# D-Robotics/hobot_stereonet

Measured on AMD Instinct MI355X. Metric: stereo pairs/s at 1280x720 D=192 (ms/frame alongside), higher is better.
Workload: dtype f16 (refinement-tower MFMA operands fp16 — 3x3 weights rounded per kernel so that every kernel's tap sum survives —, LeakyReLU applied after the fp16 rounding; low-resolution branch on 22-bit hi/lo split fp16 operands, 3 fp16 MFMAs per product in every 32-channel layer — profiles/r04_lowres_ablation

## Files before the change

### hobot_stereonet_amd/csrc/sn_dbg_hooks.hpp

```cpp
#pragma once

namespace {

void host_to_slots(const float* src, int nimg, int H, int W, std::vector<_Float16>& dst) {
  const size_t plane = (size_t)H * W;
  dst.assign((size_t)nimg * 8 * plane * 8, (_Float16)0.f);
  for (int img = 0; img < nimg; ++img)
    for (int c = 0; c < kC; ++c)
      for (size_t i = 0; i < plane; ++i) {
        const float v = src[((size_t)img * kC + c) * plane + i];
        const _Float16 hi = (_Float16)v;
        const size_t base = (((size_t)img * 4 + (c >> 3)) * 2) * plane;
        dst[(base + i) * 8 + (c & 7)] = hi;
        dst[(base + plane + i) * 8 + (c & 7)] = (_Float16)((v - (float)hi) * kSplitScale);
      }
}
void host_from_slots(const std::vector<_Float16>& src, int nimg, int H, int W, float* dst) {
  const size_t plane = (size_t)H * W;
  for (int img = 0; img < nimg; ++img)
    for (int c = 0; c < kC; ++c)
      for (size_t i = 0; i < plane; ++i) {
        const size_t base = (((size_t)img * 4 + (c >> 3)) * 2) * plane;
        dst[((size_t)img * kC + c) * plane + i] =
            (float)src[(base + i) * 8 + (c & 7)] + (float)src[(base + plane + i) * 8 + (c & 7)] * kSplitInv;
      }
}

template <class V>
hipError_t to_dev(void* dev, const V& v) {
  return hipMemcpy(dev, v.data(), v.size() * sizeof(v[0]), hipMemcpyHostToDevice);
}
template <class V>
hipError_t from_dev(V& v, const void* dev) {
  return hipMemcpy(v.data(), dev, v.size() * sizeof(v[0]), hipMemcpyDeviceToHost);
}

struct PaddedSlots {
  SlotGeom g;
  int H, W;
  size_t nplanes, lead;
  std::vector<_Float16> v;
  PaddedSlots(const SlotGeom& g_, int H_, int W_, size_t nplanes_, size_t lead_ = 0)
      : g(g_), H(H_), W(W_), nplanes(nplanes_), lead(lead_), v((nplanes_ + 2 * lead_) * g_.PH * g_.PW * 8, (_Float16)0.f) {}
  size_t row(size_t plane, int y) const { return (((plane + lead) * g.PH + y + g.py) * g.PW + g.px) * 8; }
  void put(const std::vector<_Float16>& plain) {
    for (size_t p = 0; p < nplanes; ++p)
      for (int y = 0; y < H; ++y) memcpy(&v[row(p, y)], &plain[((p * H + y) * W) * 8], (size_t)W * 16);
  }
  void get(std::vector<_Float16>& plain) const {
    for (size_t p = 0; p < nplanes; ++p)
      for (int y = 0; y < H; ++y) memcpy(&plain[((p * H + y) * W) * 8], &v[row(p, y)], (size_t)W * 16);
  }
  bool outside_is_zero() const {
    const size_t phw = (size_t)g.PH * g.PW;
    for (size_t i = 0; i < v.size(); ++i) {
      const size_t sl = i / 8, p = sl / phw, y = (sl % phw) / g.PW, x = sl % g.PW;
      const bool inside = p >= lead && p < lead + nplanes && y >= (size_t)g.py && y < (size_t)H + g.py && x >= (size_t)g.px &&
                          x < (size_t)W + g.px;
      if (!inside && (float)v[i] != 0.f) return false;
    }
    return true;
  }
};

struct RefHost {
  RefGeom g;
  int n, h, w;
  size_t lo_slots;
  std::vector<_Float16> v;
  RefHost(const RefGeom& g_, int n_, int h_, int w_, bool split, bool slack)
      : g(g_), n(n_), h(h_), w(w_), lo_slots(ref16_slots(g_, n_) + (slack ? ref_slack(g_) : 0)), v((split ? 2 : 1) * lo_slots * 8) {}
  size_t slots() const { return v.size() / 8; }
  size_t at(int i, int c, int y, int x) const {
    return ((((size_t)i * 4 + (c >> 3)) * g.Hs + y + kRefPad) * g.Ws + x + kRefPad) * 8 + (c & 7);
  }
  void pack(const float* src, bool split) {
    v.assign(v.size(), (_Float16)0.f);
    for (int i = 0; i < n; ++i)
      for (int c = 0; c < kC; ++c)
        for (int y = 0; y < h; ++y)
          for (int x = 0; x < w; ++x) {
            const float f = src[(((size_t)i * kC + c) * h + y) * w + x];
            const _Float16 hi = (_Float16)f;
            v[at(i, c, y, x)] = hi;
            if (split) v[lo_slots * 8 + at(i, c, y, x)] = (_Float16)((f - (float)hi) * kSplitScale);
          }
  }
  void unpack(float* dst, bool split) const {
    for (int i = 0; i < n; ++i)
      for (int c = 0; c < kC; ++c)
        for (int y = 0; y < h; ++y)
          for (int x = 0; x < w; ++x) {
            float f = (float)v[at(i, c, y, x)];
            if (split) f += (float)v[lo_slots * 8 + at(i, c, y, x)] * kSplitInv;
            dst[(((size_t)i * kC + c) * h + y) * w + x] = f;
          }
  }
  bool border_is_zero(int parts) const {
    for (int part = 0; part < parts; ++part)
      for (int plane = 0; plane < 4 * n; ++plane)
        for (int y = 0; y < g.Hs; ++y)
          for (int x = 0; x < g.Ws; ++x) {
            if (y >= kRefPad && y < kRefPad + h && x >= kRefPad && x < kRefPad + w) continue;
            for (int e = 0; e < 8; ++e)
              if ((float)v[part * lo_slots * 8 + (((size_t)plane * g.Hs + y) * g.Ws + x) * 8 + e] != 0.f) return false;
          }
    return true;
  }
};

hipError_t alloc_ref16(DevScope& ds, const RefGeom& g, size_t tensor_and_slack_slots, uint4** base) {
  uint4* raw = nullptr;
  const hipError_t e = alloc_ref16(g, tensor_and_slack_slots, &raw, base);
  ds.track(raw);
  return e;
}

}

extern "C" {

int sn_dbg_conv2d(sn_handle* h, const float* in, int cin, int h_px, int w, const float* wt, const float* bias,
                  int k, int stride, int dil, int lrelu, const float* residual, float* out) {
  DevScope ds;
  if (!h || !in || !wt || !bias || !out || cin <= 0 || cin > kC) return SN_ERR_ARG;
  if (!((k == 3 && stride == 1) || (k == 5 && stride == 2 && dil == 1))) return SN_ERR_ARG;
  int rc = check_device(h);
  if (rc) return rc;
  const int taps = k * k;
  const int Ho = stride == 1 ? h_px : h_px / 2, Wo = stride == 1 ? w : w / 2;
  if (stride == 2 && ((h_px & 1) || (w & 1))) return SN_ERR_ARG;
  const bool x3 = (lrelu & 2) != 0, slots = (lrelu & 4) != 0;
  const bool tower32 = (lrelu & 8) != 0;
  const bool dma = (lrelu & 16) != 0;
  lrelu &= 1;
  if (x3 != slots || (x3 && !(cin == kC && dil == 1))) return SN_ERR_ARG;
  if (dma && !(slots && (k == 3 || !residual))) return SN_ERR_ARG;
  ConvLayer L;
  rc = upload_conv2d(h, HostLayer{wt, bias, kC, cin, taps}, slots ? 8 : (k == 5 || cin <= 4) ? 4 : 8, &L);
  if (!rc && slots)
    rc = upload_x3(h, kC, [&](int co, int c, int tap) { return wt[((size_t)co * kC + c) * taps + tap]; }, &L, taps);
  ds.adopt(L);
  if (rc) return rc;
  hipStream_t st = h->stream;
  if (slots) {
    std::vector<_Float16> hin, hres, hout((size_t)8 * Ho * Wo * 8);
    host_to_slots(in, 1, h_px, w, hin);
    if (residual) host_to_slots(residual, 1, Ho, Wo, hres);
    if (dma) {
      const FeatPad fp = feat_pad(h_px, w);
      PaddedSlots pin(k == 3 ? SlotGeom{fp.PH, fp.PW, 1, 1} : down_in_geom(Ho, Wo), h_px, w, 8);
      PaddedSlots pout(k == 3 ? pin.g : SlotGeom{Ho + 5, Wo + 7, 2, 3}, Ho, Wo, 8);
      pin.put(hin);
      if (residual) pout.put(hres);
      uint4 *pdin = nullptr, *pdout = nullptr;
      HIP_TRY(h, ds.alloc(&pdin, pin.v.size() / 8));
      HIP_TRY(h, ds.alloc(&pdout, pout.v.size() / 8));
      HIP_TRY(h, to_dev(pdin, pin.v));
      HIP_TRY(h, to_dev(pdout, pout.v));
      HIP_TRY(h, hipDeviceSynchronize());
      if (k == 5)
        HIP_TRY(h, launch_down_dma(st, L, pdin, 1, Ho, Wo, pdout, pout.g, lrelu != 0, h->num_cu));
      else if (residual)
        HIP_TRY(h, (launch_feat_dma<true, true>(st, L, pdin, fp, 1, pdout, pdout, lrelu != 0, h->num_cu)));
      else
        HIP_TRY(h, (launch_feat_dma<true, false>(st, L, pdin, fp, 1, pdout, nullptr, lrelu != 0, h->num_cu)));
      HIP_TRY(h, hipStreamSynchronize(st));
      HIP_TRY(h, from_dev(pout.v, pdout));
      pout.get(hout);
      if (!pout.outside_is_zero()) {
        set_err(h, k == 3 ? "k_feat_x3s_dma wrote outside the image" : "k_down_x3s_dma wrote outside the image");
        return SN_ERR_DEVICE;
      }
    } else {
      uint4 *din = nullptr, *dout = nullptr;
      HIP_TRY(h, ds.alloc(&din, hin.size() / 8));
      HIP_TRY(h, ds.alloc(&dout, hout.size() / 8));
      HIP_TRY(h, to_dev(din, hin));
      if (residual) HIP_TRY(h, to_dev(dout, hres));
      const float* dres = residual ? reinterpret_cast<const float*>(dout) : nullptr;
      SlotIn ls{din, 0, h_px, w};
      HIP_TRY(h, k == 5 ? (launch_conv_x3s<5, 2, 32, 4, 32, 32, 1, true, SlotIn>(st, L, ls, 1, Ho, Wo, reinterpret_cast<float*>(dout), dres, lrelu != 0, h->num_cu))
                        : (launch_conv_x3s<3, 1, 32, 8, 16, 16, 2, true, SlotIn>(st, L, ls, 1, Ho, Wo, reinterpret_cast<float*>(dout), dres, lrelu != 0, h->num_cu)));
      HIP_TRY(h, hipStreamSynchronize(st));
      HIP_TRY(h, from_dev(hout, dout));
    }
    host_from_slots(hout, 1, Ho, Wo, out);
    return SN_OK;
  }
  float *din = nullptr, *dout = nullptr;
  const size_t nin = (size_t)cin * h_px * w, nout = (size_t)kC * Ho * Wo;
  HIP_TRY(h, ds.alloc(&din, nin));
  HIP_TRY(h, ds.alloc(&dout, nout));
  HIP_TRY(h, hipMemcpy(din, in, nin * 4, hipMemcpyHostToDevice));
  const float* dres = nullptr;
  if (residual) {
    HIP_TRY(h, hipMemcpy(dout, residual, nout * 4, hipMemcpyHostToDevice));
    dres = dout;
  }
  LoadF32 ld{din, cin, h_px, w};
  hipError_t e;
  if (k == 5) {
    e = (Ho * Wo <= 64 * 128) ? launch_conv<5, 2, 1, 4, 4, 32>(st, L, ld, 1, Ho, Wo, dout, dres, lrelu != 0)
                              : launch_conv<5, 2, 1, 4, 8, 64>(st, L, ld, 1, Ho, Wo, dout, dres, lrelu != 0);
  } else if (cin <= 4) {
    if (dil != 1) return SN_ERR_ARG;
    e = (Ho * Wo <= 64 * 128) ? launch_conv<3, 1, 1, 4, 4, 32>(st, L, ld, 1, Ho, Wo, dout, dres, lrelu != 0)
                              : launch_conv<3, 1, 1, 4, 8, 64>(st, L, ld, 1, Ho, Wo, dout, dres, lrelu != 0);
  } else {
    if (tower32 && ((w & 3) != 0 || cin != kC)) return SN_ERR_ARG;
    e = conv3x3(st, L, din, 1, h_px, w, dil, dout, dres, lrelu != 0, tower32 ? h->num_cu : 0);
  }
  HIP_TRY(h, e);
  HIP_TRY(h, hipStreamSynchronize(st));
  HIP_TRY(h, hipMemcpy(out, dout, nout * 4, hipMemcpyDeviceToHost));
  return SN_OK;
}

int sn_dbg_down0(sn_handle* h, const int8_t* in6, int h_px, int w, const float* wt, const float* bias, int tc,
                 float* out) {
  DevScope ds;
  if (!h || !in6 || !wt || !bias || !out || h_px <= 0 || w <= 0 || tc != 32) return SN_ERR_ARG;
  int rc = check_device(h);
  if (rc) return rc;
  const int Hp = (h_px + 15) / 16 * 16, Wp = (w + 15) / 16 * 16, Ho = Hp / 2, Wo = Wp / 2;
  Down0F16 L;
  rc = upload_down0_f16(h, HostLayer{wt, bias, kC, 3, 25}, &L);
  ds.adopt(L);
  if (rc) return rc;
  int8_t* din = nullptr;
  float *dout = nullptr, *dbias = nullptr;
  const size_t nin = (size_t)6 * h_px * w, nout = (size_t)2 * kC * Ho * Wo;
  HIP_TRY(h, ds.alloc(&din, nin));
  HIP_TRY(h, ds.alloc(&dout, nout));
  HIP_TRY(h, ds.alloc(&dbias, kC));
  HIP_TRY(h, hipMemcpy(din, in6, nin, hipMemcpyHostToDevice));
  HIP_TRY(h, hipMemcpy(dbias, bias, kC * 4, hipMemcpyHostToDevice));
  HIP_TRY(h, launch_down0_f16(h->stream, L, dbias, din, h_px, w, 2, Ho, Wo, dout, h->num_cu));
  HIP_TRY(h, hipStreamSynchronize(h->stream));
  std::vector<_Float16> hs(nout * 2);
  HIP_TRY(h, from_dev(hs, dout));
  host_from_slots(hs, 2, Ho, Wo, out);
  return SN_OK;
}

int sn_dbg_round_kernels_f16(const float* w, int nkernels, float* out) {
  if (!w || !out || nkernels < 0) return SN_ERR_ARG;
  for (int k = 0; k < nkernels; ++k) {
    _Float16 q[9];
    round_kernel_sum_preserving(w + (size_t)k * 9, q);
    for (int t = 0; t < 9; ++t) out[(size_t)k * 9 + t] = (float)q[t];
  }
  return SN_OK;
}

int sn_dbg_compose_down01(const float* w0, const float* b0, const float* w1, const float* b1, float* weff, float* beff) {
  if (!w0 || !b0 || !w1 || !b1 || !weff || !beff) return SN_ERR_ARG;
  std::vector<double> we, be;
  compose_down01(w0, b0, w1, b1, we, be);
  for (size_t i = 0; i < we.size(); ++i) weff[i] = (float)we[i];
  for (size_t i = 0; i < be.size(); ++i) beff[i] = (float)be[i];
  return SN_OK;
}

int sn_dbg_down01(sn_handle* h, const int8_t* in6, int h_px, int w, const float* w0, const float* b0, const float* w1,
                  const float* b1, float* out) {
  DevScope ds;
  if (!h || !in6 || !w0 || !b0 || !w1 || !b1 || !out || h_px <= 0 || w <= 0) return SN_ERR_ARG;
  int rc = check_device(h);
  if (rc) return rc;
  const int Hp = (h_px + 15) / 16 * 16, Wp = (w + 15) / 16 * 16, Ho = Hp / 4, Wo = Wp / 4;
  Down01W L;
  rc = upload_down01(h, HostLayer{w0, b0, kC, 3, 25}, HostLayer{w1, b1, kC, kC, 25}, &L);
  ds.adopt(L);
  if (rc) return rc;
  int8_t* din = nullptr;
  uint4* dout = nullptr;
  const size_t nin = (size_t)6 * h_px * w, nout = (size_t)2 * kC * Ho * Wo;
  HIP_TRY(h, ds.alloc(&din, nin));
  HIP_TRY(h, ds.alloc(&dout, nout / 4));
  HIP_TRY(h, hipMemcpy(din, in6, nin, hipMemcpyHostToDevice));
  HIP_TRY(h, launch_down01(h->stream, L, din, h_px, w, 2, Ho, Wo, dout, SlotGeom{Ho, Wo, 0, 0}, h->num_cu));
  HIP_TRY(h, hipStreamSynchronize(h->stream));
  std::vector<_Float16> hs(nout * 2);
  HIP_TRY(h, from_dev(hs, dout));
  host_from_slots(hs, 2, Ho, Wo, out);
  return SN_OK;
}

int sn_dbg_refin(sn_handle* h, const float* disp_low, const int8_t* in6, int h_px, int w, int dmax, const float* wt,
                 const float* bias, int split, float* out) {
  DevScope ds;
  if (!h || !disp_low || !in6 || !wt || !bias || !out || h_px <= 0 || w <= 0 || dmax <= 0) return SN_ERR_ARG;
  int rc = check_device(h);
  if (rc) return rc;
  const int Hp = (h_px + 15) / 16 * 16, Wp = (w + 15) / 16 * 16, hl = Hp / 16, wl = Wp / 16;
  RefHost t(make_ref_geom(Hp, Wp), 1, Hp, Wp, true, true);
  Down0F16 L;
  rc = upload_refin_f16(h, HostLayer{wt, bias, kC, 4, 9}, &L);
  ds.adopt(L);
  if (rc) return rc;
  float *ddl = nullptr, *dbias = nullptr;
  int8_t* din = nullptr;
  uint4* dout = nullptr;
  HIP_TRY(h, ds.alloc(&ddl, (size_t)hl * wl));
  HIP_TRY(h, ds.alloc(&dbias, kC));
  HIP_TRY(h, ds.alloc(&din, (size_t)6 * h_px * w));
  HIP_TRY(h, ds.alloc(&dout, t.slots()));
  HIP_TRY(h, hipMemcpy(ddl, disp_low, (size_t)hl * wl * 4, hipMemcpyHostToDevice));
  HIP_TRY(h, hipMemcpy(dbias, bias, kC * 4, hipMemcpyHostToDevice));
  HIP_TRY(h, hipMemcpy(din, in6, (size_t)6 * h_px * w, hipMemcpyHostToDevice));
  HIP_TRY(h, memset_now(dout, 0, t.slots() * 16));
  HIP_TRY(h, launch_refin_f16(h->stream, L, dbias, ddl, din, false, hl, wl, h_px, w, 1.0f / (float)dmax,
                              UpScale{1.0f / 16.0f, 16.0f}, t.g, 1, dout, split != 0, t.lo_slots * 16, h->num_cu));
  HIP_TRY(h, hipStreamSynchronize(h->stream));
  HIP_TRY(h, from_dev(t.v, dout));
  t.unpack(out, split != 0);
  if (!t.border_is_zero(1)) {
    set_err(h, "ref.in wrote into the zero border");
    return SN_ERR_DEVICE;
  }
  return SN_OK;
}

int sn_dbg_conv3d(sn_handle* h, const float* in, int d, int h_px, int w, const float* wt, const float* bias,
                  int lrelu, float* out) {
  DevScope ds;
  if (!h || !in || !wt || !bias || !out || d <= 0) return SN_ERR_ARG;
  int rc = check_device(h);
  if (rc) return rc;
  const bool x3 = (lrelu & 2) != 0, slots = (lrelu & 4) != 0, dma = (lrelu & 8) != 0;
  lrelu &= 1;
  if (slots != x3 || (dma && !slots)) return SN_ERR_ARG;
  ConvLayer L;
  rc = upload_conv3d(h, HostLayer{wt, bias, kC, kC, 27}, &L);
  if (!rc && x3)
    rc = upload_x3(h, 96, [&](int co, int c, int tap) { return wt[(((size_t)co * kC + (c & 31)) * 3 + (c >> 5)) * 9 + tap]; }, &L);
  ds.adopt(L);
  if (rc) return rc;
  const size_t plane = (size_t)h_px * w, n = (size_t)kC * d * plane;
  std::vector<float> tmp(n);
  for (int ci = 0; ci < kC; ++ci)
    for (int z = 0; z < d; ++z)
      memcpy(&tmp[((size_t)z * kC + ci) * plane], &in[((size_t)ci * d + z) * plane], plane * 4);
  float *din = nullptr, *dout = nullptr;
  HIP_TRY(h, ds.alloc(&din, n));
  HIP_TRY(h, ds.alloc(&dout, n));
  if (slots) {
    std::vector<_Float16> hs, ho(n * 2);
    host_to_slots(tmp.data(), d, h_px, w, hs);
    if (dma) {
      const VolPad g = vol_pad(d, h_px, w);
      PaddedSlots pin(SlotGeom{g.PH, g.PW, 1, 1}, h_px, w, (size_t)d * 8, 8), pout = pin;
      pin.put(hs);
      uint4 *pdin = nullptr, *pdout = nullptr;
      HIP_TRY(h, ds.alloc(&pdin, pin.v.size() / 8));
      HIP_TRY(h, ds.alloc(&pdout, pout.v.size() / 8));
      HIP_TRY(h, to_dev(pdin, pin.v));
      HIP_TRY(h, memset_now(pdout, 0, pout.v.size() * 2));
      HIP_TRY(h, launch_agg_dma<true>(h->stream, L, pdin, g, 1, pdout, lrelu != 0, h->num_cu));
      HIP_TRY(h, hipStreamSynchronize(h->stream));
      HIP_TRY(h, from_dev(pout.v, pdout));
      pout.get(ho);
      if (!pout.outside_is_zero()) {
        set_err(h, "k_agg_x3s_dma wrote outside the image");
        return SN_ERR_DEVICE;
      }
    } else {
      HIP_TRY(h, to_dev(din, hs));
      SlotIn ls{reinterpret_cast<const uint4*>(din), d, h_px, w};
      HIP_TRY(h, (launch_conv_x3s<3, 1, 96, 8, 16, 16, 1, true, SlotIn>(h->stream, L, ls, d, h_px, w, dout, nullptr, lrelu != 0, h->num_cu)));
      HIP_TRY(h, hipStreamSynchronize(h->stream));
      HIP_TRY(h, from_dev(ho, dout));
    }
    host_from_slots(ho, d, h_px, w, tmp.data());
  } else {
    HIP_TRY(h, to_dev(din, tmp));
    LoadVol3D lv{din, d, h_px, w};
    HIP_TRY(h, (launch_conv<3, 1, 1, 8, 4, 32>(h->stream, L, lv, d, h_px, w, dout, nullptr, lrelu != 0)));
    HIP_TRY(h, hipStreamSynchronize(h->stream));
    HIP_TRY(h, from_dev(tmp, dout));
  }
  for (int co = 0; co < kC; ++co)
    for (int z = 0; z < d; ++z)
      memcpy(&out[((size_t)co * d + z) * plane], &tmp[((size_t)z * kC + co) * plane], plane * 4);
  return SN_OK;
}

int sn_dbg_ref_conv_f16(sn_handle* h, const float* in, int h_px, int w, const float* wt, const float* bias, int dil,
                        int lrelu, const float* residual, float* out) {
  DevScope ds;
  if (!h || !in || !wt || !bias || !out || h_px <= 0 || w <= 0) return SN_ERR_ARG;
  if (dil != 1 && dil != 2 && dil != 4 && dil != 8) return SN_ERR_ARG;
  int rc = check_device(h);
  if (rc) return rc;
  RefHost t(make_ref_geom(h_px, w), 1, h_px, w, false, false);
  RefLayerF16 L;
  rc = upload_ref_f16(h, HostLayer{wt, bias, kC, kC, 9}, switches_at_create().w_round_sum_preserving, &L);
  ds.adopt(L);
  if (rc) return rc;
  uint4 *din = nullptr, *dout = nullptr;
  HIP_TRY(h, ds.alloc(&din, t.slots()));
  HIP_TRY(h, ds.alloc(&dout, t.slots()));
  t.pack(in, false);
  HIP_TRY(h, to_dev(din, t.v));
  if (residual) {
    t.pack(residual, false);
    HIP_TRY(h, to_dev(dout, t.v));
  } else {
    HIP_TRY(h, memset_now(dout, 0, t.slots() * 16));
  }
  unsigned* ctr = h->ws.tile_ctr;
  if (!ctr) {
    set_err(h, "sn_dbg_ref_conv_f16 needs an engine created in an fp16 mode");
    return SN_ERR_ARG;
  }
  HIP_TRY(h, hipMemsetAsync(ctr, 0, kTileCtrBytes, h->stream));
  HIP_TRY(h, ref_conv_f16(h->stream, L, t.g, h->num_cu, dil, din, dout, residual ? dout : nullptr, 1, (lrelu & 1) != 0, ctr,
                          (lrelu & 2) ? 64 : (lrelu & 4) ? 32 : 0));
  HIP_TRY(h, hipStreamSynchronize(h->stream));
  HIP_TRY(h, from_dev(t.v, dout));
  t.unpack(out, false);
  if (!t.border_is_zero(1)) {
    set_err(h, "fp16 conv wrote into the zero border");
    return SN_ERR_DEVICE;
  }
  return SN_OK;
}

int sn_dbg_ref_conv_f16x3(sn_handle* h, const float* in, int h_px, int w, const float* wt, const float* bias, int dil,
                          int lrelu, const float* residual, float* out) {
  DevScope ds;
  if (!h || !in || !wt || !bias || !out || h_px <= 0 || w <= 0) return SN_ERR_ARG;
  if (dil != 1 && dil != 2 && dil != 4 && dil != 8) return SN_ERR_ARG;
  int rc = check_device(h);
  if (rc) return rc;
  RefHost t(make_ref_geom(h_px, w), 1, h_px, w, true, true);
  RefLayerF16 L;
  rc = upload_ref_f16x3(h, HostLayer{wt, bias, kC, kC, 9}, &L);
  ds.adopt(L);
  if (rc) return rc;
  uint4 *din = nullptr, *dout = nullptr;
  HIP_TRY(h, ds.alloc(&din, t.slots()));
  HIP_TRY(h, ds.alloc(&dout, t.slots()));
  t.pack(in, true);
  HIP_TRY(h, to_dev(din, t.v));
  if (residual) {
    t.pack(residual, true);
    HIP_TRY(h, to_dev(dout, t.v));
  } else {
    HIP_TRY(h, memset_now(dout, 0, t.slots() * 16));
  }
  HIP_TRY(h, ref_conv_f16x3(h->stream, L, t.g, h->num_cu, dil, din, dout, residual ? dout : nullptr, t.lo_slots, 1, lrelu != 0));
  HIP_TRY(h, hipStreamSynchronize(h->stream));
  HIP_TRY(h, from_dev(t.v, dout));
  t.unpack(out, true);
  if (!t.border_is_zero(2)) {
    set_err(h, "f16x3 conv wrote into the zero border");
    return SN_ERR_DEVICE;
  }
  return SN_OK;
}

int sn_dbg_ref_block_f16x3(sn_handle* h, const float* in, int h_px, int w, const float* w1, const float* b1, const float* w2,
                           const float* b2, int dil, int form, float* out) {
  DevScope ds;
  if (!h || !in || !w1 || !b1 || !w2 || !b2 || !out || h_px <= 0 || w <= 0) return SN_ERR_ARG;
  if (dil != 1 && dil != 2 && dil != 4 && dil != 8) return SN_ERR_ARG;
  if (form != 0 && form != 1) return SN_ERR_ARG;
  if (form == 1 && !stream_x3_supports(dil)) return SN_ERR_ARG;
  int rc = check_device(h);
  if (rc) return rc;
  RefHost t(make_ref_geom(h_px, w), 1, h_px, w, true, true);
  RefLayerF16 L1, L2;
  rc = upload_ref_f16x3(h, HostLayer{w1, b1, kC, kC, 9}, &L1);
  if (!rc) rc = upload_ref_f16x3(h, HostLayer{w2, b2, kC, kC, 9}, &L2);
  ds.adopt(L1);
  ds.adopt(L2);
  if (rc) return rc;
  uint4 *cur = nullptr, *oth = nullptr;
  HIP_TRY(h, alloc_ref16(ds, t.g, t.slots(), &cur));
  HIP_TRY(h, alloc_ref16(ds, t.g, t.slots(), &oth));
  t.pack(in, true);
  HIP_TRY(h, to_dev(cur, t.v));
  HIP_TRY(h, ref_block_f16x3(h->stream, L1, L2, t.g, h->num_cu, dil, &cur, &oth, t.lo_slots, 1, form == 1));
  HIP_TRY(h, hipStreamSynchronize(h->stream));
  HIP_TRY(h, from_dev(t.v, cur));
  t.unpack(out, true);
  if (!t.border_is_zero(2)) {
    set_err(h, "f16x3 residual block wrote into the zero border");
    return SN_ERR_DEVICE;
  }
  return SN_OK;
}

int sn_dbg_ref_block_f16(sn_handle* h, const float* in, int h_px, int w, const float* w1, const float* b1,
                         const float* w2, const float* b2, int dil, float* out) {
  DevScope ds;
  if (!h || !in || !w1 || !b1 || !w2 || !b2 || !out || h_px <= 0 || w <= 0) return SN_ERR_ARG;
  const int form = dil >> 8;
  if (form != 0 && form != 2) return SN_ERR_ARG;
  const int fuse_mode = form == 2 ? 4 : 0;
  dil &= 0xff;
  if (dil != 1 && dil != 2 && dil != 4 && dil != 8) return SN_ERR_ARG;
  if (fuse_mode == 4 && !stream_block_supports(dil)) return SN_ERR_ARG;
  int rc = check_device(h);
  if (rc) return rc;
  RefHost t(make_ref_geom(h_px, w), 1, h_px, w, false, false);
  const bool sp = switches_at_create().w_round_sum_preserving;
  RefLayerF16 L1, L2;
  rc = upload_ref_f16(h, HostLayer{w1, b1, kC, kC, 9}, sp, &L1);
  if (!rc) rc = upload_ref_f16(h, HostLayer{w2, b2, kC, kC, 9}, sp, &L2);
  ds.adopt(L1);
  ds.adopt(L2);
  if (rc) return rc;
  uint4 *cur = nullptr, *oth = nullptr;
  HIP_TRY(h, alloc_ref16(ds, t.g, t.slots() + ref_slack(t.g), &cur));
  HIP_TRY(h, alloc_ref16(ds, t.g, t.slots() + ref_slack(t.g), &oth));
  t.pack(in, false);
  HIP_TRY(h, to_dev(cur, t.v));
  if (!h->ws.tile_ctr) {
    set_err(h, "sn_dbg_ref_block_f16 needs an engine created in an fp16 mode");
    return SN_ERR_ARG;
  }
  HIP_TRY(h, hipMemsetAsync(h->ws.tile_ctr, 0, kTileCtrBytes, h->stream));
  HIP_TRY(h, ref_block_f16(h->stream, L1, L2, t.g, h->num_cu, dil, &cur, &oth, 1, h->ws.tile_ctr, fuse_mode, h->dump));
  HIP_TRY(h, hipStreamSynchronize(h->stream));
  HIP_TRY(h, from_dev(t.v, cur));
  t.unpack(out, false);
  if (!t.border_is_zero(1)) {
    set_err(h, "fp16 residual block wrote into the zero border");
    return SN_ERR_DEVICE;
  }
  return SN_OK;
}

int sn_dbg_ref_tail_f16(sn_handle* h, int n, const float* in, int hk, int wk, const float* w1, const float* b1, const float* w2,
                        const float* b2, const float* head_w, float head_b, const float* low, int ups, float dnorm, int h_out,
                        int w_out, int form, float* out_disp, int32_t* out_raw) {
  DevScope ds;
  if (!h || !in || !w1 || !b1 || !w2 || !b2 || !head_w || !low || !out_disp || !out_raw) return SN_ERR_ARG;
  if (n <= 0 || hk <= 0 || wk <= 0 || h_out <= 0 || w_out <= 0 || h_out > hk || w_out > wk || (ups != 16 && ups != 2) ||
      hk % ups || wk % ups || (form != 0 && form != 1) || !(dnorm > 0.f))
    return SN_ERR_ARG;
  if (h->precision != SN_PREC_F16 && h->precision != SN_PREC_AUTO) {
    set_err(h, "sn_dbg_ref_tail_f16 needs an engine created with SN_PREC_F16 or SN_PREC_AUTO");
    return SN_ERR_ARG;
  }
  int rc = check_device(h);
  if (rc) return rc;
  const RefGeom g = make_ref_geom(hk, wk);
  if ((ref16_slots(g, n) + ref_slack(g) + ref_front(g)) * 16 >= ((size_t)1 << 32)) return SN_ERR_ARG;
  RefHost t(g, n, hk, wk, false, false);
  t.pack(in, false);
  const bool sp = switches_at_create().w_round_sum_preserving;
  RefLayerF16 L1, L2;
  HeadLayer hd;
  rc = upload_ref_f16(h, HostLayer{w1, b1, kC, kC, 9}, sp, &L1);
  if (!rc) rc = upload_ref_f16(h, HostLayer{w2, b2, kC, kC, 9}, sp, &L2);
  if (!rc) rc = upload_head(h, HostLayer{head_w, &head_b, 1, kC, 9}, &hd);
  ds.adopt(L1);
  ds.adopt(L2);
  ds.adopt(hd);
  if (rc) return rc;
  uint4 *da = nullptr, *db = nullptr;
  HIP_TRY(h, alloc_ref16(ds, g, t.slots() + ref_slack(g), &da));
  HIP_TRY(h, alloc_ref16(ds, g, t.slots() + ref_slack(g), &db));
  HIP_TRY(h, to_dev(da, t.v));
  const int sh = hk / ups, sw = wk / ups;
  const size_t nlow = (size_t)n * sh * sw, nout = (size_t)n * h_out * w_out;
  float *dlow = nullptr, *dd = nullptr;
  int32_t* dr = nullptr;
  HIP_TRY(h, ds.alloc(&dlow, nlow));
  HIP_TRY(h, ds.alloc(&dd, nout));
  HIP_TRY(h, ds.alloc(&dr, nout));
  HIP_TRY(h, hipMemcpy(dlow, low, nlow * 4, hipMemcpyHostToDevice));
  HIP_TRY(h, memset_now(dd, 0xff, nout * 4));
  HIP_TRY(h, memset_now(dr, 0xff, nout * 4));
  const float inv_q = (float)(1.0 / (kWireFactor * (double)kOutScale));
  const UpScale us{1.0f / (float)ups, (float)ups};
  const HeadArgs ha{hd.w, dlow, dd, dr, hd.bias, dnorm, inv_q, sh, sw, h_out, w_out, us};
  if (form == 1) {
    HIP_TRY(h, ref_block_stream_tail(h->stream, L1, L2, g, h->num_cu, da, n, h->dump, ha));
  } else {
    HIP_TRY(h, ref_block_stream(h->stream, L1, L2, g, h->num_cu, 1, da, db, n, h->dump));
    HIP_TRY(h, launch_head_final_f16(h->stream, false, db, 0, g, n, ha));
  }
  HIP_TRY(h, hipStreamSynchronize(h->stream));
  HIP_TRY(h, hipMemcpy(out_disp, dd, nout * 4, hipMemcpyDeviceToHost));
  HIP_TRY(h, hipMemcpy(out_raw, dr, nout * 4, hipMemcpyDeviceToHost));
  return SN_OK;
}

int sn_dbg_jpeg_dct(sn_handle* h, const uint8_t* nv12, int w, int h_px, int pitch, float* out) {
  DevScope ds;
  if (!h || !nv12 || !out || !jpg_size_ok(w, h_px) || pitch < w) return SN_ERR_ARG;
  int rc = check_device(h);
  if (rc) return rc;
  const size_t span = (size_t)(h_px + h_px / 2 - 1) * pitch + w;
  const size_t blocks = (size_t)((w + 15) / 16) * jpg_mcu_rows(h_px) * 6;
  JpgPlan plan;
  jpg_make_plan(w, h_px, 50, 0, &plan);
  uint8_t* din = nullptr;
  int16_t* dcoef = nullptr;
  float* ddct = nullptr;
  HIP_TRY(h, ds.alloc(&din, span));
  HIP_TRY(h, ds.alloc(&dcoef, blocks * 64));
  HIP_TRY(h, ds.alloc(&ddct, blocks * 64));
  HIP_TRY(h, hipMemcpy(din, nv12, span, hipMemcpyHostToDevice));
  if ((rc = jpeg_launch(h, h->stream, plan, 1, din, pitch, 0, 0, dcoef, nullptr, nullptr, nullptr, 0, nullptr, ddct))) return rc;
  HIP_TRY(h, hipStreamSynchronize(h->stream));
  HIP_TRY(h, hipMemcpy(out, ddct, blocks * 64 * 4, hipMemcpyDeviceToHost));
  return SN_OK;
}

__global__ __launch_bounds__(256) void k_copy_limited(uint4* __restrict__ dst, const uint4* __restrict__ src, size_t n16) {
  for (size_t i = (size_t)blockIdx.x * 256 + threadIdx.x; i < n16; i += (size_t)gridDim.x * 256) dst[i] = src[i];
}

int sn_dbg_copy_limited(void* dst, const void* src, size_t bytes, int workgroups, void* stream) {
  if (!dst || !src || (bytes & 15) || workgroups <= 0 || workgroups > 65535 || ((uintptr_t)dst & 15) || ((uintptr_t)src & 15)) return SN_ERR_ARG;
  hipLaunchKernelGGL(k_copy_limited, dim3((unsigned)workgroups), dim3(256), 0, static_cast<hipStream_t>(stream),
                     static_cast<uint4*>(dst), static_cast<const uint4*>(src), bytes / 16);
  return hipGetLastError() == hipSuccess ? SN_OK : SN_ERR_DEVICE;
}

int sn_dbg_read(sn_handle* h, const char* what, float* dst, size_t cap, size_t* n) {
  if (!h || !what || !n) return SN_ERR_ARG;
  int rc = check_device(h);
  if (rc) return rc;
  const size_t hw = (size_t)h->hl * h->wl;
  const float* src = nullptr;
  size_t cnt = 0;
  if (!strcmp(what, "stream_prio")) {
    *n = 1;
    if (dst && cap >= 1) dst[0] = h->stream_prio ? 1.f : 0.f;
    return (dst && cap < 1) ? SN_ERR_ARG : SN_OK;
  }
  if (!strcmp(what, "feat_l")) { src = h->ws.feat; cnt = kC * hw; }
  else if (!strcmp(what, "feat_r")) { src = h->ws.feat + kC * hw; cnt = kC * hw; }
  else if (!strcmp(what, "cost")) { src = h->ws.cost; cnt = h->Dl * hw; }
  else if (!strcmp(what, "disp_low")) { src = h->ws.disp_low; cnt = hw; }
  else if (!strcmp(what, "conf_low")) { src = h->ws.conf_low; cnt = hw; }
  else if (!strcmp(what, "tile_ctr") && h->ws.tile_ctr) { src = reinterpret_cast<const float*>(h->ws.tile_ctr); cnt = kTileCtrBytes / 4 * h->ws.n_chunks; }
  else if (!strcmp(what, "refine_x") && h->precision == SN_PREC_FP32) { src = h->ws.ref[0]; cnt = (size_t)kC * h->Hp * h->Wp; }
  else if (!strncmp(what, "level", 5) && what[5] >= '1' && what[5] < '0' + h->levels && what[6] == 0) {
    const int k = what[5] - '0';
    src = h->ws.lvl_disp[k];
    cnt = (size_t)h->tw[k].Hk * h->tw[k].Wk;
  }
  else return SN_ERR_ARG;
  *n = cnt;
  if (!dst) return SN_OK;
  if (cap < cnt) return SN_ERR_ARG;
  HIP_TRY(h, hipStreamSynchronize(h->stream));
  HIP_TRY(h, hipMemcpy(dst, src, cnt * 4, hipMemcpyDeviceToHost));
  return SN_OK;
}

}
```

### hobot_stereonet_amd/csrc/sn_engine.hpp

```cpp
#pragma once

namespace {

using namespace sn;

constexpr int kNDown = 4, kNFeatRes = 6, kNAgg = 4, kNRefRes = 6;
constexpr int kRefDil[kNRefRes] = {1, 2, 4, 8, 1, 1};
constexpr float kOutScale = 2.60443857769133e-6f;
constexpr double kWireFactor = 16.0 * 12.0;
constexpr double kAutoEnvelopeSingle = 1.0, kAutoEnvelopeMulti = 2.9;
constexpr double kAutoResidualCap = 1e30;
constexpr int kMaxPieceEvents = 64;
constexpr int kMaxTowerStreams = 2;

#define HIP_TRY(h, expr)                                                              \
  do {                                                                                \
    hipError_t e_ = (expr);                                                           \
    if (e_ != hipSuccess) {                                                           \
      set_err(h, std::string(#expr) + ": " + hipGetErrorString(e_));                  \
      return SN_ERR_DEVICE;                                                           \
    }                                                                                 \
  } while (0)

inline hipError_t memset_now(void* p, int v, size_t bytes) {
  hipError_t e = hipMemset(p, v, bytes);
  if (e != hipSuccess) return e;
  return hipStreamSynchronize(nullptr);
}

struct GrowBuf {
  void* p = nullptr;
  size_t cap = 0;
  bool pinned = false;
  hipError_t reserve(size_t bytes) {
    if (bytes <= cap) return hipSuccess;
    release();
    const hipError_t e = pinned ? hipHostMalloc(&p, bytes, hipHostMallocDefault) : hipMalloc(&p, bytes);
    if (e == hipSuccess) cap = bytes;
    else p = nullptr;
    return e;
  }
  void release() {
    if (p) (void)(pinned ? hipHostFree(p) : hipFree(p));
    p = nullptr;
    cap = 0;
  }
};

template <class Slots>
struct Lane : Slots {
  std::mutex mu;
  hipStream_t stream = nullptr;
  hipEvent_t ev = nullptr;
  GrowBuf buf[Slots::kCount];
  void destroy() {
    if (stream) (void)hipStreamSynchronize(stream);
    if (ev) {
      (void)hipEventSynchronize(ev);
      (void)hipEventDestroy(ev);
    }
    if (stream) (void)hipStreamDestroy(stream);
    for (GrowBuf& b : buf) b.release();
    stream = nullptr, ev = nullptr;
  }
};

struct ConvLayer {
  uint4* wx3 = nullptr;
  float* wpk = nullptr;
  float* bias = nullptr;
  int cin = 0, cin_pad = 0, taps = 0;
};

struct Down0F16 {
  uint4* wfrag = nullptr;
};

struct Down01W {
  uint4* wfrag = nullptr;
  float* bias = nullptr;
};

struct RefLayerF16 {
  uint4* wfrag = nullptr;
  float* bias = nullptr;
};

struct HeadLayer {
  float* w = nullptr;
  float bias = 0.f;
  float* wsplit = nullptr;
  float biassplit = 0.f, unscale = 1.f;
  uint4* pfrag = nullptr;
};

constexpr int kMaxLevels = 4, kMultiLevels = 4;
constexpr int kStatWords = 8;
constexpr size_t kStatU64 = (size_t)kStatWords * kStatWordStride;
constexpr int kTileCtrStride = 8 * 16;
constexpr size_t kTileCtrBytes = (size_t)2 * 6 * kTileCtrStride * sizeof(unsigned);

struct Workspace {
  int nb = 0, rb = 0, pb = 0;
  int rb_x3 = 0;
  int tower_cu = 0;
  int rbk_x3[4] = {};
  unsigned long long* stats = nullptr;
  unsigned long long* stats_host = nullptr;
  int8_t* in6 = nullptr;
  float* down[3] = {nullptr, nullptr, nullptr};
  float* low[3] = {nullptr, nullptr, nullptr};
  float* feat = nullptr;
  float* vol[2] = {nullptr, nullptr};
  uint4* volp[2] = {nullptr, nullptr};
  uint4* lowp[2] = {nullptr, nullptr};
  uint4* downp[3] = {nullptr, nullptr, nullptr};
  float* cost = nullptr;
  float* disp_low = nullptr;
  float* conf_low = nullptr;
  int ns = 1;
  float* ref[2 * kMaxTowerStreams] = {};
  uint4* ref16[2 * kMaxTowerStreams] = {};
  uint4* ref16_raw[2 * kMaxTowerStreams] = {};
  int rbk[kMaxLevels] = {};
  float* ref_lv[kMaxLevels][2] = {};
  uint4* ref16_lv[kMaxLevels][2] = {};
  uint4* ref16_lv_raw[kMaxLevels][2] = {};
  float* pyr[kMaxLevels] = {};
  float* lvl_disp[kMaxLevels] = {};
  int n_chunks = 0;
  unsigned* tile_ctr = nullptr;
  float* out_disp = nullptr;
  int32_t* out_raw = nullptr;
  uint8_t* nv12 = nullptr;
};

struct Tower {
  ConvLayer rin, rres[kNRefRes][2];
  Down0F16 refin;
  RefLayerF16 rres16[kNRefRes][2];
  RefLayerF16 rres16x3[kNRefRes][2];
  HeadLayer rout;
  RefGeom rg{};
  int Hk = 0, Wk = 0;
};

struct Slot {
  hipStream_t stream = nullptr;
  hipEvent_t ev0 = nullptr, ev1 = nullptr;
  Workspace ws;
  int8_t* pin_in = nullptr;
  int32_t* pin_raw = nullptr;
  float* pin_disp = nullptr;
  int32_t* user_raw = nullptr;
  float* user_disp = nullptr;
  uint64_t ticket = 0;
  hipGraphExec_t gexec[2][4][4] = {};
  int uses[2][4][4] = {};
  int mode_run = 0;
};

struct RangeCount {
  unsigned long long level[4] = {}, low = 0;
  bool any() const { return (level[0] | level[1] | level[2] | level[3] | low) != 0; }
};

struct AutoCtl {
  sn_auto_state st{};
  bool calibrated = false;
  bool pending = false;
  int pending_mode = 0, pending_n = 0;
  double selfcheck_epe = -1.0, selfcheck_res = -1.0;
  double last_level[4] = {}, last_res = 0.0;
  RangeCount last_range;
  int last_mode = 0;
  uint64_t calls = 0, pairs = 0, reruns = 0;
};

}

struct sn_handle {
  int device = 0;
  int W = 0, H = 0, D = 0, Wp = 0, Hp = 0, wl = 0, hl = 0, Dl = 0;
  int max_batch = 1, precision = SN_PREC_F16, task_num = 4, refine_chunk = 1, piece = 16;
  AutoCtl actl;
  std::mutex mu_cal;
  float* chk[2] = {nullptr, nullptr};
  hipEvent_t ev_stats = nullptr;
  int refine_chunk_x3 = 1;
  hipStream_t stream = nullptr;
  hipStream_t s_low = nullptr, s_tow[kMaxTowerStreams] = {};
  hipEvent_t ev_fork = nullptr, ev_join = nullptr, ev_tow_join[kMaxTowerStreams] = {}, ev_piece[kMaxPieceEvents] = {};
  bool overlap = true;
  int tower_streams = kMaxTowerStreams;
#if SN_DIAGNOSTICS
  unsigned ablate_x = 0;
#else
  static constexpr unsigned ablate_x = 0;
#endif
  bool tail_fuse = true;
  int fuse_mode = 4;
  unsigned* dump = nullptr;
  bool use_graphs = true;
  bool stream_prio = false;
  ConvLayer down[kNDown], fres[kNFeatRes][2], fout, agg[kNAgg];
  Down0F16 down0;
  Down01W down01;
  bool fold_down01 = false;
  HeadLayer aout;
  int levels = 1;
  Tower tw[kMaxLevels];
  int num_cu = 256;
  Workspace ws;
  std::vector<Slot> slots;
  std::mutex mu;
  std::condition_variable cv;
  uint64_t next_ticket = 1;
  bool profiling = false;
  hipEvent_t ev[8] = {};
  hipEvent_t ev_dom[2 * 6] = {};
  int dom_pairs = 0;
  float stage_ms[SN_STAGE_COUNT] = {};
  mutable std::string err;
  mutable std::mutex err_mu;
  struct PointCloudSlots {
    enum { kScratch = 0, kRaw, kNv12, kPoints, kCounts, kPinRaw, kPinNv12, kCount };
  };
  struct PointCloud : Lane<PointCloudSlots> {
    PointCloud() { buf[kPinRaw].pinned = buf[kPinNv12].pinned = true; }
  } pc;
  struct FilterSlots {
    enum { kScratch = 0, kRaw, kDisp, kMask, kCounts, kCount };
  };
  using Filter = Lane<FilterSlots>;
  Filter flt;
  struct SmoothSlots {
    enum { kScratch = 0, kRaw, kGuide, kOut, kDisp, kMask, kCounts, kCount };
  };
  using Smooth = Lane<SmoothSlots>;
  Smooth smo;
  struct JpegSlots {
    enum { kCoef = 0, kBytes, kLens, kIn, kOut, kSizes, kCount };
  };
  struct Jpeg : Lane<JpegSlots> {
    sn::JpgPlan plan;
  } jpg;
  struct InferStaging {
    enum { kIn = 0, kMirror, kLeft, kRight, kDisp, kRightOut, kMask, kKept, kConf, kCount };
    GrowBuf buf[kCount];
  } stage;
  std::atomic<int> temporal_live{0};
  std::atomic<int> rectify_live{0};
};

struct sn_temporal_slots {
  enum { kRaw = 0, kGuide, kDisp, kMask, kCounts, kCount };
};
struct sn_temporal : Lane<sn_temporal_slots> {
  sn_handle* h = nullptr;
  int streams = 0;
  sn_temporal_params p{};
  long long q = 0;
  void* state = nullptr;
  std::vector<uint8_t> fresh;
};

struct sn_rectify_slots {
  enum { kLeft = 0, kRight, kSbs, kTensor, kCount };
};
struct sn_rectify : Lane<sn_rectify_slots> {
  sn_handle* h = nullptr;
  sn_stereo_calib c{};
  uint32_t valid[2] = {0, 0};
  int32_t* map = nullptr;
};

namespace {

void set_err(const sn_handle* h, const std::string& s) {
  if (h) {
    std::lock_guard<std::mutex> lk(h->err_mu);
    h->err = s;
  }
}
void set_err(std::nullptr_t, const std::string&) {}

template <class T>
hipError_t dalloc(T** p, size_t count) {
  return hipMalloc(reinterpret_cast<void**>(p), count * sizeof(T) + 256);
}

struct DevScope {
  std::vector<void*> ptrs;
  void track(const void* p) {
    void* q = const_cast<void*>(p);
    if (q && std::find(ptrs.begin(), ptrs.end(), q) == ptrs.end()) ptrs.push_back(q);
  }
  template <class T>
  hipError_t alloc(T** p, size_t count) {
    const hipError_t e = dalloc(p, count);
    track(*p);
    return e;
  }
  void adopt(const ConvLayer& l) { track(l.wx3); track(l.wpk); track(l.bias); }
  void adopt(const Down0F16& l) { track(l.wfrag); }
  void adopt(const Down01W& l) { track(l.wfrag); track(l.bias); }
  void adopt(const RefLayerF16& l) { track(l.wfrag); track(l.bias); }
  void adopt(const HeadLayer& l) { track(l.w); track(l.pfrag); if (l.wsplit != l.w) track(l.wsplit); }
  ~DevScope() {
    for (void* q : ptrs) (void)hipFree(q);
  }
};

int check_device(sn_handle* h) {
  HIP_TRY(h, hipSetDevice(h->device));
  return SN_OK;
}

}
```

### hobot_stereonet_amd/csrc/sn_forward.hpp

```cpp
#pragma once

namespace {

inline int piece_pairs(const sn_handle* h, int nb, int rb) {
  int pb = h->piece > 0 ? h->piece : 16;
  if (pb > nb) pb = nb;
  if (pb < rb) pb = rb;
  return pb;
}
inline int level_chunk_pairs(int rb, int pb, int lv) {
  const long r = (long)rb << (2 * lv);
  return lv == 0 ? rb : (r < pb ? (int)r : pb);
}

int alloc_ws(sn_handle* h, Workspace* ws, int nb, int rb, int ns, int rb_x3 = 0) {
  const bool is_auto = h->precision == SN_PREC_AUTO;
  if (rb_x3 <= 0 || rb_x3 > rb) rb_x3 = rb;
  ws->nb = nb;
  ws->rb = rb;
  ws->rb_x3 = rb_x3;
  ws->ns = (ns > 1 && nb > rb) ? (ns < kMaxTowerStreams ? ns : kMaxTowerStreams) : 1;
  if (h->levels > 1) ws->ns = 1;
  ws->pb = piece_pairs(h, nb, rb);
  const int pb = ws->pb;
  const size_t HW = (size_t)h->H * h->W, HWp = (size_t)h->Hp * h->Wp, hw = (size_t)h->hl * h->wl;
  HIP_TRY(h, dalloc(&ws->in6, (size_t)nb * 6 * HW));
  bool padded_down = h->precision != SN_PREC_FP32 && switches().down_dma;
  size_t downp_bytes[3] = {0, 0, 0};
  for (int k = h->fold_down01 ? 1 : 0; k < 3 && padded_down; ++k) {
    const SlotGeom g = down_in_geom(h->Hp >> (k + 2), h->Wp >> (k + 2));
    downp_bytes[k] = (size_t)2 * pb * 8 * g.PH * g.PW * sizeof(uint4);
    padded_down = downp_bytes[k] < ((size_t)1 << 32);
  }
  const int k_first = h->fold_down01 ? 1 : 0;
  for (int k = k_first; k < 3 && !padded_down; ++k)
    HIP_TRY(h, dalloc(&ws->down[k], (size_t)2 * pb * kC * (HWp >> (2 * (k + 1)))));
  for (int k = 0; k < 3; ++k) HIP_TRY(h, dalloc(&ws->low[k], (size_t)2 * pb * kC * hw));
  HIP_TRY(h, dalloc(&ws->feat, (size_t)2 * pb * kC * hw));
  for (int k = 0; k < 2; ++k) HIP_TRY(h, dalloc(&ws->vol[k], (size_t)pb * h->Dl * kC * hw));
  for (int k = k_first; k < 3 && padded_down; ++k) {
    HIP_TRY(h, hipMalloc(reinterpret_cast<void**>(&ws->downp[k]), downp_bytes[k]));
    HIP_TRY(h, memset_now(ws->downp[k], 0, downp_bytes[k]));
  }
  if (padded_down && switches().feat_dma) {
    const FeatPad g = feat_pad(h->hl, h->wl);
    const size_t bytes = (size_t)2 * pb * g.img_slots() * sizeof(uint4);
    for (int k = 0; k < 2 && bytes < ((size_t)1 << 32); ++k) {
      HIP_TRY(h, hipMalloc(reinterpret_cast<void**>(&ws->lowp[k]), bytes));
      HIP_TRY(h, memset_now(ws->lowp[k], 0, bytes));
    }
  }
  if (h->precision != SN_PREC_FP32 && switches().agg_dma) {
    const VolPad g = vol_pad(h->Dl, h->hl, h->wl);
    const size_t bytes = g.planes(pb) * g.plane_slots() * sizeof(uint4);
    for (int k = 0; k < 2 && bytes < ((size_t)1 << 32); ++k) {
      HIP_TRY(h, hipMalloc(reinterpret_cast<void**>(&ws->volp[k]), bytes));
      HIP_TRY(h, memset_now(ws->volp[k], 0, bytes));
    }
  }
  HIP_TRY(h, dalloc(&ws->cost, (size_t)nb * h->Dl * hw));
  HIP_TRY(h, dalloc(&ws->disp_low, (size_t)nb * hw));
  HIP_TRY(h, dalloc(&ws->conf_low, (size_t)nb * hw));
  HIP_TRY(h, memset_now(ws->conf_low, 0, (size_t)nb * hw * sizeof(float)));
  auto tensor_slots = [&](const RefGeom& rg, int pairs, int pairs_x3) {
    const size_t one = ref16_slots(rg, pairs) + ref_slack(rg), lo = ref16_slots(rg, pairs_x3) + ref_slack(rg);
    return h->precision == SN_PREC_F16X3 ? 2 * one : (is_auto ? one + lo : one);
  };
  if (h->precision == SN_PREC_FP32) {
    for (int k = 0; k < 2 * ws->ns; ++k) HIP_TRY(h, dalloc(&ws->ref[k], (size_t)rb * kC * HWp));
  } else {
    for (int k = 0; k < 2 * ws->ns; ++k)
      HIP_TRY(h, alloc_ref16(h->tw[0].rg, tensor_slots(h->tw[0].rg, rb, rb_x3), &ws->ref16_raw[k], &ws->ref16[k]));
    ws->n_chunks = (nb + rb_x3 - 1) / rb_x3 + (nb + pb - 1) / pb + 2;
    for (int lv = 1; lv < h->levels; ++lv) {
      const int rbk = level_chunk_pairs(rb_x3, pb, lv);
      ws->n_chunks += ((nb + pb - 1) / pb + 2) * ((pb + rbk - 1) / rbk + 1);
    }
    HIP_TRY(h, hipExtMallocWithFlags(reinterpret_cast<void**>(&ws->tile_ctr), kTileCtrBytes * ws->n_chunks, hipDeviceMallocFinegrained));
  }
  ws->rbk[0] = rb;
  ws->rbk_x3[0] = rb_x3;
  for (int lv = 1; lv < h->levels; ++lv) {
    const Tower& T = h->tw[lv];
    const size_t HWk = (size_t)T.Hk * T.Wk;
    ws->rbk[lv] = level_chunk_pairs(rb, pb, lv);
    ws->rbk_x3[lv] = level_chunk_pairs(rb_x3, pb, lv);
    for (int k = 0; k < 2; ++k) {
      if (h->precision == SN_PREC_FP32) {
        HIP_TRY(h, dalloc(&ws->ref_lv[lv][k], (size_t)ws->rbk[lv] * kC * HWk));
      } else {
        HIP_TRY(h, alloc_ref16(T.rg, tensor_slots(T.rg, ws->rbk[lv], ws->rbk_x3[lv]), &ws->ref16_lv_raw[lv][k], &ws->ref16_lv[lv][k]));
      }
    }
    HIP_TRY(h, dalloc(&ws->pyr[lv], (size_t)pb * 3 * HWk));
    HIP_TRY(h, dalloc(&ws->lvl_disp[lv], (size_t)pb * HWk));
  }
  HIP_TRY(h, dalloc(&ws->out_disp, (size_t)nb * HW));
  HIP_TRY(h, dalloc(&ws->out_raw, (size_t)nb * HW));
  HIP_TRY(h, dalloc(&ws->nv12, (size_t)HW * 3));
  HIP_TRY(h, dalloc(&ws->stats, kStatU64));
  HIP_TRY(h, memset_now(ws->stats, 0, kStatU64 * sizeof(unsigned long long)));
  HIP_TRY(h, hipHostMalloc(reinterpret_cast<void**>(&ws->stats_host), kStatU64 * sizeof(unsigned long long), hipHostMallocDefault));
  memset(ws->stats_host, 0, kStatU64 * sizeof(unsigned long long));
  return SN_OK;
}

void free_ws(Workspace* ws) {
  hipFree(ws->in6);
  hipFree(ws->tile_ctr);
  for (auto p : ws->down) hipFree(p);
  for (auto p : ws->low) hipFree(p);
  hipFree(ws->feat);
  for (auto p : ws->vol) hipFree(p);
  for (auto p : ws->volp) hipFree(p);
  for (auto p : ws->downp) hipFree(p);
  for (auto p : ws->lowp) hipFree(p);
  hipFree(ws->cost);
  hipFree(ws->disp_low);
  hipFree(ws->conf_low);
  for (auto p : ws->ref) hipFree(p);
  for (auto p : ws->ref16_raw) hipFree(p);
  for (auto& lv : ws->ref_lv)
    for (auto p : lv) hipFree(p);
  for (auto& lv : ws->ref16_lv_raw)
    for (auto p : lv) hipFree(p);
  for (auto p : ws->pyr) hipFree(p);
  for (auto p : ws->lvl_disp) hipFree(p);
  hipFree(ws->out_disp);
  hipFree(ws->out_raw);
  hipFree(ws->nv12);
  hipFree(ws->stats);
  if (ws->stats_host) hipHostFree(ws->stats_host);
  *ws = Workspace();
}

int launch_softargmin(sn_handle* h, Workspace& ws, hipStream_t st, const float* v, bool folded, int p0, int m, bool want_cost,
                      bool want_conf) {
  const int hl = h->hl, wl = h->wl, Dl = h->Dl, npix = m * hl * wl;
  float* const disp_low = ws.disp_low + (size_t)p0 * hl * wl;
  float* const cost_out = want_cost ? ws.cost + (size_t)p0 * Dl * hl * wl : nullptr;
  float* const conf_low = want_conf ? ws.conf_low + (size_t)p0 * hl * wl : nullptr;
  unsigned long long* const nf = ws.stats + kStatNonfiniteLow;
  const dim3 grid((npix + 63) / 64);
  if (folded) {
    const auto kern = want_conf ? k_softargmin_p<16, true> : k_softargmin_p<16, false>;
    hipLaunchKernelGGL(kern, grid, dim3(64 * Dl), 0, st, v, h->aout.bias, Dl, hl, wl, npix, disp_low, cost_out, conf_low, nf);
  } else {
    const auto kern = want_conf ? k_head_softargmin<16, true> : k_head_softargmin<16, false>;
    hipLaunchKernelGGL(kern, grid, dim3(64 * kSamWaves), 0, st, v, h->aout.w, h->aout.bias, Dl, hl, wl, npix, disp_low, cost_out,
                       conf_low, nf);
  }
  HIP_TRY(h, hipGetLastError());
  return SN_OK;
}

inline const uint4* as_slots(const float* p) { return reinterpret_cast<const uint4*>(p); }

int lowres_down_slots(sn_handle* h, Workspace& ws, hipStream_t st, const int8_t* in, int ni) {
  const int Hp = h->Hp, Wp = h->Wp, ncu = h->num_cu;
  const int k_first = h->fold_down01 ? 1 : 0;
  if (ws.downp[1] != nullptr) {
    SlotGeom gin[3];
    for (int i = 0; i < 3; ++i) gin[i] = down_in_geom(Hp >> (i + 2), Wp >> (i + 2));
    if (h->fold_down01)
      HIP_TRY(h, launch_down01(st, h->down01, in, h->H, h->W, ni, Hp / 4, Wp / 4, ws.downp[1], gin[1], ncu));
    else
      HIP_TRY(h, launch_down0_f16(st, h->down0, h->down[0].bias, in, h->H, h->W, ni, Hp / 2, Wp / 2,
                                  reinterpret_cast<float*>(ws.downp[0]), ncu, &gin[0]));
    for (int i = k_first; i < 3; ++i) {
      const int Ho = Hp >> (i + 2), Wo = Wp >> (i + 2);
      const SlotGeom plain{Ho, Wo, 0, 0};
      const FeatPad fp = feat_pad(h->hl, h->wl);
      const SlotGeom bordered{fp.PH, fp.PW, 1, 1};
      void* const last = ws.lowp[0] ? (void*)ws.lowp[0] : (void*)ws.low[0];
      HIP_TRY(h, launch_down_dma(st, h->down[i + 1], ws.downp[i], ni, Ho, Wo, i < 2 ? (void*)ws.downp[i + 1] : last,
                                 i < 2 ? gin[i + 1] : (ws.lowp[0] ? bordered : plain), false, ncu));
    }
    return SN_OK;
  }
  if (h->fold_down01)
    HIP_TRY(h, launch_down01(st, h->down01, in, h->H, h->W, ni, Hp / 4, Wp / 4, reinterpret_cast<uint4*>(ws.down[1]),
                             SlotGeom{Hp / 4, Wp / 4, 0, 0}, ncu));
  else
    HIP_TRY(h, launch_down0_f16(st, h->down0, h->down[0].bias, in, h->H, h->W, ni, Hp / 2, Wp / 2, ws.down[0], ncu));
  float* const src[3] = {ws.down[0], ws.down[1], ws.down[2]};
  float* const dst[3] = {ws.down[1], ws.down[2], ws.low[0]};
  for (int i = k_first; i < 3; ++i) {
    const int Hi = Hp >> (i + 1), Wi = Wp >> (i + 1);
    if ((h->ablate_x >> (kAblDown + i)) & 1u) HIP_TRY(h, zero_lo_slots(st, src[i], ni, (size_t)Hi * Wi));
    SlotIn ld{as_slots(src[i]), 0, Hi, Wi};
    HIP_TRY(h, (launch_conv_x3s<5, 2, 32, 4, 32, 32, 1, true, SlotIn>(st, h->down[i + 1], ld, ni, Hi / 2, Wi / 2, dst[i],
                                                                     nullptr, false, ncu)));
  }
  return SN_OK;
}

int lowres_features_slots(sn_handle* h, Workspace& ws, hipStream_t st, int ni) {
  const int hl = h->hl, wl = h->wl, ncu = h->num_cu;
  if (ws.lowp[0] != nullptr && ws.downp[1] != nullptr) {
    const FeatPad fp = feat_pad(hl, wl);
    uint4 *x = ws.lowp[0], *t = ws.lowp[1];
    for (int i = 0; i < kNFeatRes; ++i) {
      HIP_TRY(h, (launch_feat_dma<true, false>(st, h->fres[i][0], x, fp, ni, t, nullptr, true, ncu)));
      HIP_TRY(h, (launch_feat_dma<true, true>(st, h->fres[i][1], t, fp, ni, x, x, true, ncu)));
    }
    HIP_TRY(h, (launch_feat_dma<false, false>(st, h->fout, x, fp, ni, ws.feat, nullptr, false, ncu)));
    return SN_OK;
  }
  float *const x = ws.low[0], *const t = ws.low[1];
  const SlotIn lx{as_slots(x), 0, hl, wl}, lt{as_slots(t), 0, hl, wl};
  for (int i = 0; i < kNFeatRes; ++i) {
    if ((h->ablate_x >> (kAblFeat + 2 * i)) & 1u) HIP_TRY(h, zero_lo_slots(st, x, ni, (size_t)hl * wl));
    HIP_TRY(h, (launch_conv_x3s<3, 1, 32, 8, 16, 16, 2, true, SlotIn>(st, h->fres[i][0], lx, ni, hl, wl, t, nullptr, true, ncu)));
    if ((h->ablate_x >> (kAblFeat + 2 * i + 1)) & 1u) HIP_TRY(h, zero_lo_slots(st, t, ni, (size_t)hl * wl));
    HIP_TRY(h, (launch_conv_x3s<3, 1, 32, 8, 16, 16, 2, true, SlotIn>(st, h->fres[i][1], lt, ni, hl, wl, x, x, true, ncu)));
  }
  if ((h->ablate_x >> (kAblFeat + 12)) & 1u) HIP_TRY(h, zero_lo_slots(st, x, ni, (size_t)hl * wl));
  HIP_TRY(h, (launch_conv_x3s<3, 1, 32, 8, 16, 16, 1, false, SlotIn>(st, h->fout, lx, ni, hl, wl, ws.feat, nullptr, false, ncu)));
  return SN_OK;
}

int lowres_aggregate_slots(sn_handle* h, Workspace& ws, hipStream_t st, int m, bool* folded) {
  const int hl = h->hl, wl = h->wl, Dl = h->Dl, ncu = h->num_cu;
  const long total = (long)m * Dl * 4 * hl * wl;
  *folded = false;
  if (ws.volp[0] != nullptr) {
    const VolPad g = vol_pad(Dl, hl, wl);
    hipLaunchKernelGGL(k_cost_slots_pad, dim3((unsigned)((total + 255) / 256)), dim3(256), 0, st, ws.feat, ws.volp[1], g, m);
    for (int i = 0; i + 1 < kNAgg; ++i)
      HIP_TRY(h, launch_agg_dma<true>(st, h->agg[i], ws.volp[(i + 1) & 1], g, m, ws.volp[i & 1], true, ncu));
    const int i = kNAgg - 1;
    *folded = switches().head_fold && h->aout.pfrag;
    if (*folded)
      HIP_TRY(h, (launch_agg_dma<false, true>(st, h->agg[i], ws.volp[(i + 1) & 1], g, m, ws.vol[i & 1], true, ncu, h->aout.pfrag)));
    else
      HIP_TRY(h, launch_agg_dma<false>(st, h->agg[i], ws.volp[(i + 1) & 1], g, m, ws.vol[i & 1], true, ncu));
    return SN_OK;
  }
  hipLaunchKernelGGL(k_cost_slots, dim3((unsigned)((total + 255) / 256)), dim3(256), 0, st, ws.feat,
                     reinterpret_cast<uint4*>(ws.vol[1]), Dl, hl, wl, m);
  for (int i = 0; i < kNAgg; ++i) {
    float* const src = ws.vol[(i + 1) & 1];
    if ((h->ablate_x >> (kAblAgg + i)) & 1u) HIP_TRY(h, zero_lo_slots(st, src, m * Dl, (size_t)hl * wl));
    SlotIn lv{as_slots(src), Dl, hl, wl};
    if (i + 1 < kNAgg)
      HIP_TRY(h, (launch_conv_x3s<3, 1, 96, 8, 16, 16, 1, true, SlotIn>(st, h->agg[i], lv, m * Dl, hl, wl, ws.vol[i & 1], nullptr, true, ncu)));
    else
      HIP_TRY(h, (launch_conv_x3s<3, 1, 96, 8, 16, 16, 1, false, SlotIn>(st, h->agg[i], lv, m * Dl, hl, wl, ws.vol[i & 1], nullptr, true, ncu)));
  }
  return SN_OK;
}

int lowres(sn_handle* h, Workspace& ws, hipStream_t st, int p0, int m, const int8_t* in6, bool want_cost, bool want_conf,
           bool prof) {
  const int Hp = h->Hp, Wp = h->Wp, hl = h->hl, wl = h->wl, Dl = h->Dl;
  const size_t HW = (size_t)h->H * h->W;
  const int8_t* in = in6 + (size_t)p0 * 6 * HW;
  bool folded = false;
  if (h->precision != SN_PREC_FP32) {
    int rc;
    if ((rc = lowres_down_slots(h, ws, st, in, 2 * m))) return rc;
    if ((rc = lowres_features_slots(h, ws, st, 2 * m))) return rc;
    if (prof) HIP_TRY(h, hipEventRecord(h->ev[1], st));
    if ((rc = lowres_aggregate_slots(h, ws, st, m, &folded))) return rc;
    return launch_softargmin(h, ws, st, ws.vol[(kNAgg - 1) & 1], folded, p0, m, want_cost, want_conf);
  }
  {
    LoadI8Eye ld{in, h->H, h->W};
    const int Ho = Hp / 2, Wo = Wp / 2;
    if (Ho * Wo <= 64 * 128)
      HIP_TRY(h, (launch_conv<5, 2, 1, 4, 4, 32>(st, h->down[0], ld, 2 * m, Ho, Wo, ws.down[0], nullptr, false)));
    else
      HIP_TRY(h, (launch_conv<5, 2, 1, 4, 8, 64>(st, h->down[0], ld, 2 * m, Ho, Wo, ws.down[0], nullptr, false)));
  }
  HIP_TRY(h, conv5x5s2(st, h->down[1], ws.down[0], 2 * m, Hp / 2, Wp / 2, ws.down[1]));
  HIP_TRY(h, conv5x5s2(st, h->down[2], ws.down[1], 2 * m, Hp / 4, Wp / 4, ws.down[2]));
  HIP_TRY(h, conv5x5s2(st, h->down[3], ws.down[2], 2 * m, Hp / 8, Wp / 8, ws.low[0]));
  float* x = ws.low[0];
  float* t = ws.low[1];
  for (int i = 0; i < kNFeatRes; ++i) {
    HIP_TRY(h, conv3x3(st, h->fres[i][0], x, 2 * m, hl, wl, 1, t, nullptr, true));
    HIP_TRY(h, conv3x3(st, h->fres[i][1], t, 2 * m, hl, wl, 1, x, x, true));
  }
  HIP_TRY(h, conv3x3(st, h->fout, x, 2 * m, hl, wl, 1, ws.feat, nullptr, false));
  if (prof) HIP_TRY(h, hipEventRecord(h->ev[1], st));

  LoadCostVol ld{ws.feat, Dl, hl, wl};
  HIP_TRY(h, (launch_conv<3, 1, 1, 8, 4, 32>(st, h->agg[0], ld, m * Dl, hl, wl, ws.vol[0], nullptr, true)));
  for (int i = 1; i < kNAgg; ++i) {
    LoadVol3D lv{ws.vol[(i - 1) & 1], Dl, hl, wl};
    HIP_TRY(h, (launch_conv<3, 1, 1, 8, 4, 32>(st, h->agg[i], lv, m * Dl, hl, wl, ws.vol[i & 1], nullptr, true)));
  }
  return launch_softargmin(h, ws, st, ws.vol[(kNAgg - 1) & 1], folded, p0, m, want_cost, want_conf);
}

inline int first_piece(const sn_handle* h, const Workspace& ws, int n) {
  const int forced = switches().first_piece;
  int m = ws.pb;
  if (h->precision == SN_PREC_FP32) m = ws.rb * ws.ns > 2 ? ws.rb * ws.ns : 2;
  if (forced > 0) m = forced;
  if (m > ws.pb) m = ws.pb;
  return m < n ? m : n;
}

struct RefineCall {
  const Tower* T;
  float* const* ref;
  uint4* const* ref16;
  const float* src;
  int sh, sw;
  UpScale ups;
  const void* img_src;
  bool pyr;
  int H, W;
  float dnorm;
  float* od;
  int32_t* orw;
  unsigned* chunk_ctr;
  int c;
  int cap;
  bool pe;
  int mode;
  unsigned long long* stat;
};

int refine_level(sn_handle* h, Workspace& ws, hipStream_t st, const RefineCall& a) {
  const Tower& T = *a.T;
  const int ncu = h->num_cu, c = a.c;
  const int tcu = ws.tower_cu > 0 ? ws.tower_cu : ncu;
  const int Hk = T.Hk, Wk = T.Wk;
  const bool pe = a.pe;
  const float inv_q = (float)(1.0 / (kWireFactor * (double)kOutScale));
  if (a.mode == SN_PREC_FP32) {
    LoadRefineIn ld{a.src, reinterpret_cast<const int8_t*>(a.img_src), a.sh, a.sw, a.H, a.W, Hk, Wk, 1.0f / a.dnorm, a.ups,
                    a.pyr ? reinterpret_cast<const float*>(a.img_src) : nullptr};
    if (Hk * Wk <= 64 * 128)
      HIP_TRY(h, (launch_conv<3, 1, 1, 4, 4, 32>(st, T.rin, ld, c, Hk, Wk, a.ref[0], nullptr, true)));
    else
      HIP_TRY(h, (launch_conv<3, 1, 1, 4, 8, 64>(st, T.rin, ld, c, Hk, Wk, a.ref[0], nullptr, true)));
    if (pe) HIP_TRY(h, hipEventRecord(h->ev[4], st));
    for (int i = 0; i < kNRefRes; ++i) {
      HIP_TRY(h, conv3x3(st, T.rres[i][0], a.ref[0], c, Hk, Wk, kRefDil[i], a.ref[1], nullptr, true, ncu));
      HIP_TRY(h, conv3x3(st, T.rres[i][1], a.ref[1], c, Hk, Wk, kRefDil[i], a.ref[0], a.ref[0], true, ncu));
    }
    if (pe) HIP_TRY(h, hipEventRecord(h->ev[5], st));
    const HeadArgs ha{T.rout.w, a.src, a.od, a.orw, T.rout.bias, a.dnorm, inv_q, a.sh, a.sw, a.H, a.W, a.ups, a.stat};
    if (switches().head_mfma32) {
      constexpr int TH = 14;
      using HT = HeadTile<TH>;
      const int tiles_x = (a.W + HT::TWO - 1) / HT::TWO, tiles_y = (a.H + TH - 1) / TH;
      hipLaunchKernelGGL(k_head_final_mfma32<TH>, dim3((unsigned)(tiles_x * tiles_y * c)), dim3(256), HT::LDS_BYTES, st, a.ref[0],
                         Hk, Wk, tiles_x, tiles_y, ha);
    } else {
      dim3 grid((a.W + 63) / 64, (a.H + 3) / 4, c);
      hipLaunchKernelGGL(k_head_final, grid, dim3(256), 0, st, a.ref[0], Hk, Wk, ha);
    }
  } else {
    uint4 *x16 = a.ref16[0], *t16 = a.ref16[1];
    if (pe) h->dom_pairs = 0;
    const bool rev_env = switches().rev;
    RefGeom g = T.rg;
    int launch_no = 0;
    auto flip = [&]() { g.rev = rev_env ? (launch_no++ & 1) : 0; };
    flip();
    const bool x3 = a.mode == SN_PREC_F16X3;
    const size_t lo_slots = ref16_slots(g, a.cap) + ref_slack(g);
    HIP_TRY(h, launch_refin_f16(st, T.refin, T.rin.bias, a.src, a.img_src, a.pyr, a.sh, a.sw, a.H, a.W, 1.0f / a.dnorm, a.ups, g,
                                c, x16, x3, lo_slots * 16, ncu));
    if (pe) HIP_TRY(h, hipEventRecord(h->ev[4], st));
    flip();
    const HeadArgs ha{T.rout.wsplit, a.src, a.od, a.orw, T.rout.biassplit, a.dnorm * T.rout.unscale, inv_q, a.sh, a.sw,
                      a.H, a.W, a.ups, a.stat};
    const bool last_streamed = h->fuse_mode == 4 && stream_block_supports(kRefDil[kNRefRes - 1]);
    const bool tail = !x3 && last_streamed && h->tail_fuse && kRefDil[kNRefRes - 1] == 1 && a.ups.rs <= 0.5f;
    for (int i = 0; i < kNRefRes; ++i) {
      if (x3) {
        const bool dom = pe && stream_x3_supports(kRefDil[i]) && h->dom_pairs < 6;
        if (dom) HIP_TRY(h, hipEventRecord(h->ev_dom[2 * h->dom_pairs], st));
        HIP_TRY(h, ref_block_f16x3(st, T.rres16x3[i][0], T.rres16x3[i][1], g, tcu, kRefDil[i], &x16, &t16, lo_slots, c));
        if (dom) HIP_TRY(h, hipEventRecord(h->ev_dom[2 * h->dom_pairs++ + 1], st));
      } else if (tail && i == kNRefRes - 1) {
        if (pe) HIP_TRY(h, hipEventRecord(h->ev[5], st));
        HIP_TRY(h, ref_block_stream_tail(st, T.rres16[i][0], T.rres16[i][1], g, tcu, x16, c, h->dump, ha));
      } else {
        const bool dom = pe && h->fuse_mode == 4 && stream_block_supports(kRefDil[i]) && h->dom_pairs < 6;
        if (dom) HIP_TRY(h, hipEventRecord(h->ev_dom[2 * h->dom_pairs], st));
        HIP_TRY(h, ref_block_f16(st, T.rres16[i][0], T.rres16[i][1], g, tcu, kRefDil[i], &x16, &t16, c,
                                 a.chunk_ctr + 2 * i * kTileCtrStride, h->fuse_mode, h->dump, rev_env));
        if (dom) HIP_TRY(h, hipEventRecord(h->ev_dom[2 * h->dom_pairs++ + 1], st));
      }
    }
    if (!tail) {
      if (pe) HIP_TRY(h, hipEventRecord(h->ev[5], st));
      HIP_TRY(h, launch_head_final_f16(st, x3, x16, lo_slots, g, c, ha));
    }
  }
  HIP_TRY(h, hipGetLastError());
  return SN_OK;
}

inline int chunk_pairs(const sn_handle* h, const Workspace& ws, int mode, int lv = 0) {
  return (h->precision == SN_PREC_AUTO && mode == SN_PREC_F16X3) ? ws.rbk_x3[lv] : ws.rbk[lv];
}

inline int take_ctr_block(sn_handle* h, Workspace& ws, int* ctr_block, unsigned** out) {
  *out = nullptr;
  if (!ws.tile_ctr) return SN_OK;
  if (*ctr_block >= ws.n_chunks) {
    set_err(h, "internal: tile-queue pool exhausted");
    return SN_ERR_DEVICE;
  }
  *out = ws.tile_ctr + (size_t)(*ctr_block)++ * (kTileCtrBytes / sizeof(unsigned));
  return SN_OK;
}

int refine_coarse(sn_handle* h, Workspace& ws, hipStream_t st, int p0, int m, const int8_t* in6, int* ctr_block, int mode) {
  const size_t HW = (size_t)h->H * h->W;
  const int8_t* in_piece = in6 + (size_t)p0 * 6 * HW;
  for (int lv = 1; lv < h->levels; ++lv) {
    const Tower& T = h->tw[lv];
    const long total = (long)m * 3 * T.Hk * T.Wk;
    const dim3 grid((unsigned)((total + 255) / 256));
    if (lv == 1)
      hipLaunchKernelGGL(k_img_pool2<true>, grid, dim3(256), 0, st, (const void*)in_piece, h->H, h->W, T.Hk, T.Wk,
                         ws.pyr[lv], total);
    else
      hipLaunchKernelGGL(k_img_pool2<false>, grid, dim3(256), 0, st, (const void*)ws.pyr[lv - 1], 0, 0, T.Hk, T.Wk,
                         ws.pyr[lv], total);
  }
  HIP_TRY(h, hipGetLastError());
  const float* src = ws.disp_low + (size_t)p0 * h->hl * h->wl;
  int sh = h->hl, sw = h->wl;
  for (int lv = h->levels - 1; lv >= 1; --lv) {
    const Tower& T = h->tw[lv];
    const size_t HWk = (size_t)T.Hk * T.Wk;
    const float dnorm = (float)h->D / (float)(1 << lv);
    const int rbk = chunk_pairs(h, ws, mode, lv);
    for (int q = 0; q < m; q += rbk) {
      const int c = (m - q) < rbk ? (m - q) : rbk;
      RefineCall a{};
      int rc = take_ctr_block(h, ws, ctr_block, &a.chunk_ctr);
      if (rc) return rc;
      a.T = &T;
      a.ref = ws.ref_lv[lv], a.ref16 = ws.ref16_lv[lv];
      a.src = src + (size_t)q * sh * sw, a.sh = sh, a.sw = sw, a.ups = UpScale{0.5f, 2.0f};
      a.img_src = ws.pyr[lv] + (size_t)q * 3 * HWk, a.pyr = true;
      a.H = T.Hk, a.W = T.Wk, a.dnorm = dnorm;
      a.od = ws.lvl_disp[lv] + (size_t)q * HWk;
      a.c = c, a.cap = ws.rbk[lv], a.mode = mode;
      a.stat = ws.stats + (size_t)lv * kStatWordStride;
      if ((rc = refine_level(h, ws, st, a))) return rc;
    }
    src = ws.lvl_disp[lv];
    sh = T.Hk;
    sw = T.Wk;
  }
  return SN_OK;
}

int refine_chunk(sn_handle* h, Workspace& ws, hipStream_t st, int sidx, int* ctr_block, int p0, int q0, int c,
                 const int8_t* in6, float* out_disp, int32_t* out_raw, bool pe, int mode) {
  const int hl = h->hl, wl = h->wl;
  const size_t HW = (size_t)h->H * h->W;
  RefineCall a{};
  if (const int rc = take_ctr_block(h, ws, ctr_block, &a.chunk_ctr)) return rc;
  a.T = &h->tw[0];
  a.ref = &ws.ref[2 * sidx], a.ref16 = &ws.ref16[2 * sidx];
  if (h->levels > 1) {
    a.sh = h->tw[1].Hk, a.sw = h->tw[1].Wk;
    a.src = ws.lvl_disp[1] + (size_t)(q0 - p0) * a.sh * a.sw;
    a.ups = UpScale{0.5f, 2.0f};
  } else {
    a.sh = hl, a.sw = wl;
    a.src = ws.disp_low + (size_t)q0 * hl * wl;
    a.ups = UpScale{1.0f / 16.0f, 16.0f};
  }
  a.img_src = in6 + (size_t)q0 * 6 * HW, a.pyr = false;
  a.H = h->H, a.W = h->W, a.dnorm = (float)h->D;
  a.od = out_disp ? out_disp + (size_t)q0 * HW : nullptr;
  a.orw = out_raw ? out_raw + (size_t)q0 * HW : nullptr;
  a.c = c, a.cap = ws.rb, a.pe = pe, a.mode = mode, a.stat = ws.stats;
  return refine_level(h, ws, st, a);
}

int forward(sn_handle* h, Workspace& ws, hipStream_t st, int n, const int8_t* in6, float* out_disp,
            int32_t* out_raw, bool want_cost, int mode = 0, bool want_conf = false) {
  if (mode == 0) mode = h->precision == SN_PREC_AUTO ? h->actl.st.mode : h->precision;
  const int rb = chunk_pairs(h, ws, mode);
  const bool prof = h->profiling && (&ws == &h->ws);
  const bool piped = !prof && (&ws == &h->ws) && h->overlap && n > rb;
  int rc;
  int ctr_block = 0;
  bool need_queues = ws.tile_ctr != nullptr && mode == SN_PREC_F16;
  if (need_queues && h->fuse_mode == 4) {
    need_queues = false;
    for (int i = 0; i < kNRefRes; ++i) need_queues = need_queues || !stream_block_supports(kRefDil[i]);
  }
  if (need_queues) HIP_TRY(h, hipMemsetAsync(ws.tile_ctr, 0, kTileCtrBytes * ws.n_chunks, st));
  HIP_TRY(h, hipMemsetAsync(ws.stats, 0, kMaxLevels * kStatWordStride * sizeof(unsigned long long), st));
  auto finish = [&]() -> int {
    HIP_TRY(h, hipMemcpyAsync(ws.stats_host, ws.stats, (size_t)h->levels * kStatWordStride * sizeof(unsigned long long),
                              hipMemcpyDeviceToHost, st));
    return SN_OK;
  };
  if (!piped) {
    if (prof) HIP_TRY(h, hipEventRecord(h->ev[0], st));
    for (int p0 = 0, m = 0; p0 < n; p0 += m) {
      m = (n - p0) < ws.pb ? (n - p0) : ws.pb;
      if ((rc = lowres(h, ws, st, p0, m, in6, want_cost, want_conf, prof && p0 == 0))) return rc;
      if (prof && p0 == 0) HIP_TRY(h, hipEventRecord(h->ev[2], st));
      if (h->levels > 1 && (rc = refine_coarse(h, ws, st, p0, m, in6, &ctr_block, mode))) return rc;
      for (int q0 = p0; q0 < p0 + m; q0 += rb) {
        const int c = (p0 + m - q0) < rb ? (p0 + m - q0) : rb;
        if ((rc = refine_chunk(h, ws, st, 0, &ctr_block, p0, q0, c, in6, out_disp, out_raw, prof && q0 == 0, mode))) return rc;
      }
    }
    if (prof) HIP_TRY(h, hipEventRecord(h->ev[3], st));
    return finish();
  }
  const int ns = ws.ns;
  HIP_TRY(h, hipEventRecord(h->ev_fork, st));
  HIP_TRY(h, hipStreamWaitEvent(h->s_low, h->ev_fork, 0));
  for (int s = 0; s < ns; ++s) HIP_TRY(h, hipStreamWaitEvent(h->s_tow[s], h->ev_fork, 0));
  int k = 0, chunk = 0;
  for (int p0 = 0, m = 0; p0 < n; p0 += m, ++k) {
    m = p0 == 0 ? first_piece(h, ws, n) : ((n - p0) < ws.pb ? (n - p0) : ws.pb);
    if ((rc = lowres(h, ws, h->s_low, p0, m, in6, want_cost, want_conf, false))) return rc;
    hipEvent_t e = h->ev_piece[k % kMaxPieceEvents];
    HIP_TRY(h, hipEventRecord(e, h->s_low));
    bool waited[kMaxTowerStreams] = {};
    if (h->levels > 1) {
      HIP_TRY(h, hipStreamWaitEvent(h->s_tow[0], e, 0));
      waited[0] = true;
      if ((rc = refine_coarse(h, ws, h->s_tow[0], p0, m, in6, &ctr_block, mode))) return rc;
    }
    for (int q0 = p0; q0 < p0 + m; q0 += rb, ++chunk) {
      const int c = (p0 + m - q0) < rb ? (p0 + m - q0) : rb;
      const int s = chunk % ns;
      if (!waited[s]) {
        HIP_TRY(h, hipStreamWaitEvent(h->s_tow[s], e, 0));
        waited[s] = true;
      }
      if ((rc = refine_chunk(h, ws, h->s_tow[s], s, &ctr_block, p0, q0, c, in6, out_disp, out_raw, false, mode))) return rc;
    }
  }
  HIP_TRY(h, hipEventRecord(h->ev_join, h->s_low));
  HIP_TRY(h, hipStreamWaitEvent(st, h->ev_join, 0));
  for (int s = 0; s < ns; ++s) {
    HIP_TRY(h, hipEventRecord(h->ev_tow_join[s], h->s_tow[s]));
    HIP_TRY(h, hipStreamWaitEvent(st, h->ev_tow_join[s], 0));
  }
  return finish();
}

int collect_profile(sn_handle* h) {
  if (!h->profiling) return SN_OK;
  HIP_TRY(h, hipEventSynchronize(h->ev[3]));
  float ms = 0.f;
  HIP_TRY(h, hipEventElapsedTime(&ms, h->ev[0], h->ev[1]));
  h->stage_ms[SN_STAGE_FEATURES] = ms;
  HIP_TRY(h, hipEventElapsedTime(&ms, h->ev[1], h->ev[2]));
  h->stage_ms[SN_STAGE_AGGREGATE] = ms;
  HIP_TRY(h, hipEventElapsedTime(&ms, h->ev[2], h->ev[3]));
  h->stage_ms[SN_STAGE_REFINE] = ms;
  HIP_TRY(h, hipEventElapsedTime(&ms, h->ev[4], h->ev[5]));
  h->stage_ms[SN_STAGE_REFINE_CONV] = ms;
  HIP_TRY(h, hipEventElapsedTime(&ms, h->ev[0], h->ev[3]));
  h->stage_ms[SN_STAGE_TOTAL] = ms;
  if (h->dom_pairs > 0) {
    float sum = 0.f;
    for (int i = 0; i < h->dom_pairs; ++i) {
      HIP_TRY(h, hipEventElapsedTime(&ms, h->ev_dom[2 * i], h->ev_dom[2 * i + 1]));
      sum += ms;
    }
    h->stage_ms[SN_STAGE_DOMINANT] = sum;
  } else {
    h->stage_ms[SN_STAGE_DOMINANT] = h->stage_ms[SN_STAGE_REFINE_CONV];
  }
  return SN_OK;
}

__global__ __launch_bounds__(256) void k_abs_diff_sum(const float* __restrict__ a, const float* __restrict__ b, size_t n,
                                                      unsigned long long* __restrict__ out) {
  float sum = 0.f;
  for (size_t i = (size_t)blockIdx.x * 256 + threadIdx.x; i < n; i += (size_t)gridDim.x * 256) sum += fabsf(a[i] - b[i]);
  refine_stat_commit_block(out, sum);
}

inline unsigned long long stat_word(const Workspace& ws, int word, int at = 0) {
  unsigned long long sum = 0;
  for (int s = 0; s < kStatSlots; ++s) sum += ws.stats_host[(size_t)word * kStatWordStride + (size_t)s * kStatLine + at];
  return sum;
}
void read_stats(const sn_handle* h, const Workspace& ws, int n, double* level_px, double* residual_px, RangeCount* range) {
  double res = 0.0;
  *range = RangeCount{};
  for (int lv = 0; lv < kMaxLevels; ++lv) {
    level_px[lv] = 0.0;
    if (lv >= h->levels || n <= 0) continue;
    const double px = lv == 0 ? (double)h->H * h->W : (double)h->tw[lv].Hk * h->tw[lv].Wk;
    level_px[lv] = (double)stat_word(ws, lv) / (double)kStatScale / (px * n);
    res += level_px[lv] * (double)(1 << lv);
    range->level[lv] = stat_word(ws, lv, kStatNonfinite);
  }
  if (n > 0) range->low = stat_word(ws, 0, kStatNonfiniteLow);
  *residual_px = range->any() ? (double)INFINITY : res;
}
int range_result(sn_handle* h, const RangeCount& r) {
  if (!r.any()) return SN_OK;
  char msg[256];
  snprintf(msg, sizeof msg, "activations left the range of fp16 (65504): non-finite pixels per level %llu/%llu/%llu/%llu, low-resolution "
           "%llu; the maps are not valid — use SN_PREC_FP32 for this model", r.level[0], r.level[1], r.level[2], r.level[3], r.low);
  set_err(h, msg);
  return SN_ERR_RANGE;
}

void count_call(sn_handle* h, int n) {
  std::lock_guard<std::mutex> lk(h->mu);
  ++h->actl.calls;
  h->actl.pairs += (uint64_t)n;
}

int fold_stats(sn_handle* h, const double* level_px, double residual_px, const RangeCount& range, int n, int mode,
               bool observe = true) {
  std::lock_guard<std::mutex> lk(h->mu);
  AutoCtl& a = h->actl;
  for (int lv = 0; lv < kMaxLevels; ++lv) a.last_level[lv] = level_px[lv];
  a.last_res = residual_px;
  a.last_range = range;
  a.last_mode = mode;
  if (!observe) {
    ++a.reruns;
    return a.st.mode;
  }
  if (h->precision != SN_PREC_AUTO) {
    const double r = residual_px <= kAutoResidualCap ? residual_px : kAutoResidualCap;
    a.st.running_px = a.st.running_px < 0.0 ? r : 0.75 * a.st.running_px + 0.25 * r;
    return h->precision;
  }
  const int before = a.st.mode;
  const int after = sn_auto_observe(&a.st, residual_px);
  if (before == SN_PREC_F16X3 && after == SN_PREC_F16) a.calibrated = false;
  return after;
}

int auto_selfcheck(sn_handle* h, Workspace& ws, hipStream_t st, const int8_t* in6_pair) {
  std::lock_guard<std::mutex> cal(h->mu_cal);
  {
    std::lock_guard<std::mutex> lk(h->mu);
    if (h->actl.calibrated) return SN_OK;
  }
  const bool prof = h->profiling;
  h->profiling = false;
  double lvl[kMaxLevels], res = 0.0;
  RangeCount range_x3, range;
  int rc = forward(h, ws, st, 1, in6_pair, h->chk[1], nullptr, false, SN_PREC_F16X3);
  if (!rc && hipStreamSynchronize(st) == hipSuccess) read_stats(h, ws, 1, lvl, &res, &range_x3);
  if (!rc) rc = forward(h, ws, st, 1, in6_pair, h->chk[0], nullptr, false, SN_PREC_F16);
  h->profiling = prof;
  if (rc) return rc;
  const size_t HW = (size_t)h->H * h->W;
  HIP_TRY(h, hipMemsetAsync(ws.stats + 4 * kStatWordStride, 0, kStatWordStride * sizeof(unsigned long long), st));
  hipLaunchKernelGGL(k_abs_diff_sum, dim3(512), dim3(256), 0, st, h->chk[0], h->chk[1], HW, ws.stats + 4 * kStatWordStride);
  HIP_TRY(h, hipGetLastError());
  HIP_TRY(h, hipMemcpyAsync(ws.stats_host, ws.stats, kStatU64 * sizeof(unsigned long long), hipMemcpyDeviceToHost, st));
  HIP_TRY(h, hipStreamSynchronize(st));
  read_stats(h, ws, 1, lvl, &res, &range);
  if (range.any() || range_x3.any() || stat_word(ws, 4, kStatNonfinite) != 0) return SN_OK;
  const double epe = (double)stat_word(ws, 4) / (double)kStatScale / (double)HW;
  std::lock_guard<std::mutex> lk(h->mu);
  AutoCtl& a = h->actl;
  a.selfcheck_epe = epe;
  a.selfcheck_res = res;
  a.st.epe_per_px = res > 1e-6 ? epe / res : 0.0;
  a.calibrated = true;
  return SN_OK;
}

int fold_pending(sn_handle* h, bool wait) {
  AutoCtl& a = h->actl;
  {
    std::lock_guard<std::mutex> lk(h->mu);
    if (!a.pending) return SN_OK;
  }
  if (wait) {
    HIP_TRY(h, hipEventSynchronize(h->ev_stats));
  } else if (hipEventQuery(h->ev_stats) != hipSuccess) {
    (void)hipGetLastError();
    return SN_OK;
  }
  int n, mode;
  {
    std::lock_guard<std::mutex> lk(h->mu);
    if (!a.pending) return SN_OK;
    a.pending = false;
    n = a.pending_n;
    mode = a.pending_mode;
  }
  double lvl[kMaxLevels], res = 0.0;
  RangeCount range;
  read_stats(h, h->ws, n, lvl, &res, &range);
  fold_stats(h, lvl, res, range, n, mode);
  return SN_OK;
}

template <class Rerun>
int settle(sn_handle* h, Workspace& ws, hipStream_t st, int n, const int8_t* in6, int mode, bool check, bool count,
           Rerun rerun, RangeCount* range) {
  double lvl[kMaxLevels], res = 0.0;
  int rc;
  read_stats(h, ws, n, lvl, &res, range);
  if (check && !range->any() && (rc = auto_selfcheck(h, ws, st, in6))) return rc;
  if (count) count_call(h, n);
  const int next = fold_stats(h, lvl, res, *range, n, mode);
  if (h->precision == SN_PREC_AUTO && mode == SN_PREC_F16 && next == SN_PREC_F16X3) {
    if ((rc = rerun())) return rc;
    read_stats(h, ws, n, lvl, &res, range);
    fold_stats(h, lvl, res, *range, n, SN_PREC_F16X3, false);
  }
  return SN_OK;
}

template <class Post>
int run_forward(sn_handle* h, hipStream_t st, int n, const int8_t* din, float* ddisp, int32_t* draw, bool want_cost,
                bool blocking, Post post, bool want_conf = false) {
  const bool is_auto = h->precision == SN_PREC_AUTO;
  AutoCtl& a = h->actl;
  int rc = fold_pending(h, blocking);
  if (rc) return rc;
  int mode, calibrated;
  {
    std::lock_guard<std::mutex> lk(h->mu);
    mode = is_auto ? a.st.mode : h->precision;
    calibrated = a.calibrated;
  }
  const bool check = is_auto && mode == SN_PREC_F16 && !calibrated;
  if ((rc = forward(h, h->ws, st, n, din, ddisp, draw, want_cost, mode, want_conf))) return rc;
  if ((rc = post())) return rc;
  count_call(h, n);
  if (!blocking && !check) {
    HIP_TRY(h, hipEventRecord(h->ev_stats, st));
    std::lock_guard<std::mutex> lk(h->mu);
    a.pending = true;
    a.pending_n = n;
    a.pending_mode = mode;
    return SN_OK;
  }
  HIP_TRY(h, hipStreamSynchronize(st));
  RangeCount range;
  auto rerun = [&]() -> int {
    int r = forward(h, h->ws, st, n, din, ddisp, draw, want_cost, SN_PREC_F16X3, want_conf);
    if (!r) r = post();
    if (r) return r;
    HIP_TRY(h, hipStreamSynchronize(st));
    return SN_OK;
  };
  if ((rc = settle(h, h->ws, st, n, din, mode, check, false, rerun, &range))) return rc;
  if ((rc = collect_profile(h))) return rc;
  return blocking ? range_result(h, range) : SN_OK;
}

}
```

### hobot_stereonet_amd/csrc/sn_switches.hpp

```cpp
#pragma once

#include <cctype>
#include <climits>
#include <cstdlib>
#include <cstring>
#include <string>

#include "../../include/stereonet_hip.h"

#ifndef SN_DIAGNOSTICS
#define SN_DIAGNOSTICS 0
#endif

namespace sn {

constexpr int kSwitchUnset = INT_MIN;

enum { kAblDown = 0, kAblFeat = 3, kAblAgg = 16, kAblCount = 20 };

struct Switches {
  bool down01 = true;
  bool agg_dma = true;
  bool feat_dma = true;
  bool down_dma = true;
  bool head_fold = true;
  int f32_grid = 0;
  bool f32_tower = true;
  int stream_wgs = 0;
  int stream_dil = 8;
  int fuse = 4;
  bool x3_stream = true;
  int x3_nwr = 4;
  int first_piece = 0;
  bool head_mfma32 = true;
  bool rev = true;
  bool async_share = true;

  bool w_round_sum_preserving = true;
  int precision = SN_PREC_AUTO;
  int tower_streams = kSwitchUnset;
  int stream_priority = kSwitchUnset;
  bool no_overlap = false;
  bool no_graph = false;
  bool tail_fuse = true;
  int mgpu_gather = 0;
  bool mgpu_allow_dup = false;
  unsigned ablate_w = 0;
  unsigned ablate_x = 0;
};

namespace switch_parse {
inline bool on_unless_zero(const char* name) {
  const char* e = getenv(name);
  return !(e != nullptr && atoi(e) == 0);
}
inline bool present(const char* name) { return getenv(name) != nullptr; }
inline int int_or(const char* name, int dflt) {
  const char* e = getenv(name);
  return e ? atoi(e) : dflt;
}
inline bool equals(const char* name, const char* value) {
  const char* e = getenv(name);
  return e && strcmp(e, value) == 0;
}

#if !SN_DIAGNOSTICS
inline unsigned ablate_mask(const char*) { return 0u; }
#else
inline unsigned ablate_mask(const char* var) {
  const char* e = getenv(var);
  if (!e || !*e) return 0u;
  if (!strcmp(e, "all")) return (1u << kAblCount) - 1u;
  unsigned m = 0;
  std::string str(e);
  size_t pos = 0;
  while (pos <= str.size()) {
    size_t c = str.find(',', pos);
    if (c == std::string::npos) c = str.size();
    const std::string t = str.substr(pos, c - pos);
    int idx = -1;
    if (t.rfind("down", 0) == 0 && t.size() == 5 && t[4] >= '1' && t[4] <= '3') idx = kAblDown + (t[4] - '1');
    else if (t.rfind("agg", 0) == 0 && t.size() == 4 && t[3] >= '0' && t[3] <= '3') idx = kAblAgg + (t[3] - '0');
    else if (t.size() >= 2 && t[0] == 'f' && atoi(t.c_str() + 1) >= 0 && atoi(t.c_str() + 1) <= 12 && isdigit((unsigned char)t[1])) idx = kAblFeat + atoi(t.c_str() + 1);
    if (idx >= 0) m |= 1u << idx;
    pos = c + 1;
  }
  return m;
}
#endif
}

inline void read_switches(Switches* s, bool process_scope) {
  using namespace switch_parse;
  if (process_scope) {
    const bool plain = ablate_mask("SN_ABLATE_X") != 0;
    s->down01 = on_unless_zero("SN_DOWN01");
    s->agg_dma = on_unless_zero("SN_AGG_DMA") && !plain;
    s->feat_dma = on_unless_zero("SN_FEAT_DMA") && !plain;
    s->down_dma = on_unless_zero("SN_DOWN_DMA") && !plain;
    s->head_fold = on_unless_zero("SN_HEAD_FOLD");
    s->f32_grid = int_or("SN_F32_GRID", 0);
    s->f32_tower = on_unless_zero("SN_F32_TOWER");
    s->stream_wgs = int_or("SN_STREAM_WGS", 0);
    s->stream_dil = int_or("SN_STREAM_DIL", 8);
    s->fuse = int_or("SN_FUSE", 4);
    s->x3_stream = on_unless_zero("SN_X3_STREAM");
    s->x3_nwr = int_or("SN_X3_NWR", 4);
    s->first_piece = int_or("SN_FIRST_PIECE", 0);
    s->head_mfma32 = on_unless_zero("SN_HEAD_MFMA32");
    s->rev = on_unless_zero("SN_REV");
    s->async_share = on_unless_zero("SN_ASYNC_SHARE");
    return;
  }
  s->w_round_sum_preserving = !equals("SN_W_ROUND", "rne");
  s->precision = equals("SN_PRECISION", "f16") ? SN_PREC_F16 : equals("SN_PRECISION", "f16x3") ? SN_PREC_F16X3
                 : equals("SN_PRECISION", "fp32") ? SN_PREC_FP32 : SN_PREC_AUTO;
  s->tower_streams = int_or("SN_TOWER_STREAMS", kSwitchUnset);
  s->stream_priority = equals("SN_STREAM_PRIORITY", "") ? kSwitchUnset : int_or("SN_STREAM_PRIORITY", kSwitchUnset);
  s->no_overlap = present("SN_NO_OVERLAP");
  s->no_graph = present("SN_NO_GRAPH");
  s->tail_fuse = on_unless_zero("SN_TAIL_FUSE");
  s->mgpu_gather = equals("SN_MGPU_GATHER", "peer") ? 1 : equals("SN_MGPU_GATHER", "rccl") ? 2 : 0;
  s->mgpu_allow_dup = int_or("SN_MGPU_ALLOW_DUP", 0) == 1;
  s->ablate_w = ablate_mask("SN_ABLATE_W");
  s->ablate_x = ablate_mask("SN_ABLATE_X");
}

inline const Switches& switches() {
  static const Switches latched = [] {
    Switches s;
    read_switches(&s, true);
    return s;
  }();
  return latched;
}
inline Switches switches_at_create() {
  Switches s = switches();
  read_switches(&s, false);
  return s;
}

}
```

### hobot_stereonet_amd/csrc/stereonet_hip.hip

```cpp
#include <hip/hip_runtime.h>

#include <algorithm>

#include <atomic>
#include <chrono>
#include <cmath>
#include <condition_variable>
#include <cstdio>
#include <cstdlib>
#include <cstring>
#include <memory>
#include <mutex>
#include <string>
#include <unordered_map>
#include <vector>

#include "../../include/stereonet_hip.h"
#include "sn_internal.h"
#include "sn_switches.hpp"
#include "sn_kernels.hpp"
#include "sn_pointcloud.hpp"
#include "sn_lrcheck.hpp"
#include "sn_dispfilter.hpp"
#include "sn_confidence.hpp"
#include "sn_smooth.hpp"
#include "sn_temporal.hpp"
#include "sn_rectify.hpp"
#include "sn_jpeg.hpp"
#include "sn_engine.hpp"
#include "sn_weights.hpp"
#include "sn_launch.hpp"
#include "sn_forward.hpp"
#include "sn_postproc.hpp"
#include "sn_dbg_hooks.hpp"

extern "C" {

const char* sn_strerror(int code) {
  switch (code) {
    case SN_OK: return "ok";
    case SN_ERR_ARG: return "invalid argument";
    case SN_ERR_FILE: return "model file missing or unreadable";
    case SN_ERR_FORMAT: return "model file is not an SN-K4 SNW1 weight file";
    case SN_ERR_DEVICE: return "HIP device error (a gfx950 GPU is required; there is no CPU path)";
    case SN_ERR_NOMEM: return "out of memory";
    case SN_ERR_BUSY: return "no free task slot";
    case SN_ERR_TICKET: return "unknown ticket";
    case SN_ERR_RANGE: return "activations left the range of fp16 (65504): the maps are not valid; use SN_PREC_FP32 for this model";
    default: return "unknown error";
  }
}

static thread_local std::string g_create_err;
static int create_fail(int code, const char* what) {
  const hipError_t e = hipGetLastError();
  g_create_err = std::string(what) + (e != hipSuccess ? std::string(": ") + hipGetErrorString(e) : std::string());
  return code;
}

const char* sn_last_error(const sn_handle* h) {
  if (!h) return g_create_err.c_str();
  thread_local std::string copy;
  std::lock_guard<std::mutex> lk(h->err_mu);
  copy = h->err;
  return copy.c_str();
}

int sn_create(const char* model_file, const sn_config* cfg, sn_handle** out) {
  return sn_create_prio(model_file, cfg, -1, out);
}

int sn_create_prio(const char* model_file, const sn_config* cfg, int stream_prio, sn_handle** out) {
  if (!model_file || !out) return SN_ERR_ARG;
  *out = nullptr;
  FILE* f = fopen(model_file, "rb");
  if (!f) return SN_ERR_FILE;
  SnwHeader hd;
  if (fread(&hd, 1, sizeof hd, f) != sizeof hd || memcmp(hd.magic, "SNW1", 4) != 0) {
    fclose(f);
    return SN_ERR_FORMAT;
  }
  const uint32_t dil_ok[6] = {1, 2, 4, 8, 1, 1};
  if (hd.version != 1 || hd.channels != kC || hd.n_down != kNDown || hd.n_fres != kNFeatRes ||
      hd.n_agg != kNAgg || hd.n_rres != kNRefRes || memcmp(hd.dil, dil_ok, sizeof dil_ok) != 0 ||
      (hd.reserved != 0 && hd.reserved != 1 && hd.reserved != (uint64_t)kMultiLevels)) {
    fclose(f);
    return SN_ERR_FORMAT;
  }
  const int levels = hd.reserved > 1 ? (int)hd.reserved : 1;
  if (hd.n_params != param_count(levels)) {
    fclose(f);
    return SN_ERR_FORMAT;
  }
  std::vector<float> blob(hd.n_params);
  const size_t got = fread(blob.data(), sizeof(float), blob.size(), f);
  fclose(f);
  if (got != blob.size()) return SN_ERR_FORMAT;

  const Switches sw = switches_at_create();
  sn_config c{};
  if (cfg) c = *cfg; else c.device = -1;
  const int W = c.width > 0 ? c.width : (int)hd.width;
  const int H = c.height > 0 ? c.height : (int)hd.height;
  const int D = c.dmax > 0 ? c.dmax : (int)hd.dmax;
  if (W <= 0 || H <= 0 || D < 16 || D % 16 || D > 256) return SN_ERR_ARG;
  if (c.precision == SN_PREC_DEFAULT) {
    c.precision = sw.precision;
  }
  if (c.precision != SN_PREC_FP32 && c.precision != SN_PREC_F16 && c.precision != SN_PREC_F16X3 && c.precision != SN_PREC_AUTO)
    return SN_ERR_ARG;

  int ndev = 0;
  g_create_err.clear();
  if (hipGetDeviceCount(&ndev) != hipSuccess || ndev <= 0) return create_fail(SN_ERR_DEVICE, "hipGetDeviceCount");
  int dev = c.device;
  if (dev < 0 && hipGetDevice(&dev) != hipSuccess) return create_fail(SN_ERR_DEVICE, "hipGetDevice");
  if (dev >= ndev) return SN_ERR_ARG;
  hipDeviceProp_t prop;
  if (hipGetDeviceProperties(&prop, dev) != hipSuccess) return create_fail(SN_ERR_DEVICE, "hipGetDeviceProperties");
  if (strncmp(prop.gcnArchName, "gfx950", 6) != 0) {
    fprintf(stderr, "stereonet_hip: device %d is %s, this library is built for gfx950 only\n", dev,
            prop.gcnArchName);
    return SN_ERR_DEVICE;
  }

  sn_handle* h = new sn_handle();
  h->device = dev;
  h->W = W;
  h->H = H;
  h->D = D;
  h->Wp = (W + 15) / 16 * 16;
  h->Hp = (H + 15) / 16 * 16;
  h->wl = h->Wp / 16;
  h->hl = h->Hp / 16;
  h->Dl = D / 16;
  h->max_batch = c.max_batch > 0 ? c.max_batch : 1;
  h->precision = c.precision;
  h->task_num = c.task_num > 0 ? c.task_num : 4;
  h->refine_chunk = c.refine_chunk;
  h->piece = c.piece > 0 ? c.piece : 16;
  h->levels = levels;
  sn_auto_init(&h->actl.st, levels);
  if (c.precision != SN_PREC_AUTO) h->actl.st.mode = c.precision;
  h->actl.last_mode = h->actl.st.mode;
  for (int k = 0; k < levels; ++k) {
    h->tw[k].Hk = h->Hp >> k;
    h->tw[k].Wk = h->Wp >> k;
    h->tw[k].rg = make_ref_geom(h->tw[k].Hk, h->tw[k].Wk);
  }
  {
    h->tower_streams = sw.tower_streams != kSwitchUnset ? sw.tower_streams : (h->precision == SN_PREC_FP32 ? 2 : 1);
    if (h->tower_streams < 1) h->tower_streams = 1;
    if (h->tower_streams > kMaxTowerStreams) h->tower_streams = kMaxTowerStreams;
  }
  const bool want_f16 = c.precision == SN_PREC_F16 || c.precision == SN_PREC_AUTO;
  const bool want_x3 = c.precision == SN_PREC_F16X3 || c.precision == SN_PREC_AUTO;
  {
    const double tensor_mb = 4.0 * h->tw[0].rg.Hs * h->tw[0].rg.Ws * 16.0 / 1048576.0 * 2.0;
    int r = (int)(256.0 / (2.0 * tensor_mb * h->tower_streams) + 0.5);
    if (stream_x3_supports(8)) {
      const int by_px = (int)(5.5e6 / ((double)h->Hp * h->Wp) + 0.5);
      if (by_px > r) r = by_px;
    }
    h->refine_chunk_x3 = r < 1 ? 1 : (r > 8 ? 8 : r);
  }
  if (h->refine_chunk <= 0) {
    const double tensor_mb = 4.0 * h->tw[0].rg.Hs * h->tw[0].rg.Ws * 16.0 / 1048576.0 * (c.precision == SN_PREC_F16X3 ? 2.0 : c.precision == SN_PREC_FP32 ? 2.0 : 1.0);
    int rc_auto = (int)(256.0 / (2.0 * tensor_mb * h->tower_streams) + 0.5);
    if ((want_f16 && sw.fuse == 4 && stream_block_supports(8)) || (c.precision == SN_PREC_F16X3 && stream_x3_supports(8))) {
      const int by_px = (int)(5.5e6 / ((double)h->Hp * h->Wp) + 0.5);
      if (by_px > rc_auto) rc_auto = by_px;
    }
    h->refine_chunk = rc_auto < 1 ? 1 : (rc_auto > 8 ? 8 : rc_auto);
  }
  h->num_cu = prop.multiProcessorCount > 0 ? prop.multiProcessorCount : 256;
  if (h->refine_chunk > h->max_batch) h->refine_chunk = h->max_batch;
  if (h->refine_chunk_x3 > h->refine_chunk) h->refine_chunk_x3 = h->refine_chunk;

  {
    const int pb = piece_pairs(h, h->max_batch, h->refine_chunk);
    const double low_elems = 2.0 * pb * kC * (h->Hp / 2.0) * (h->Wp / 2.0);
    const double vol_elems = (double)pb * h->Dl * kC * h->hl * h->wl;
    double ref_bytes = 0;
    for (int lv = 0; lv < h->levels; ++lv) {
      const RefGeom& rg = h->tw[lv].rg;
      const double b = ((double)level_chunk_pairs(h->refine_chunk, pb, lv) * 4.0 * rg.Hs * rg.Ws + (double)ref_slack(rg) + (double)ref_front(rg)) * 16.0;
      if (b > ref_bytes) ref_bytes = b;
    }
    if (low_elems >= 4.0e9 || ref_bytes >= 4.0e9 || vol_elems >= 4.0e9) {
      delete h;
      return SN_ERR_ARG;
    }
  }
  int rc = check_device(h);
  auto fail = [&](int code) {
    create_fail(code, h->err.empty() ? "engine set-up" : h->err.c_str());
    sn_destroy(h);
    return code;
  };
  if (rc) return fail(rc);
  if (hipStreamCreateWithFlags(&h->stream, hipStreamNonBlocking) != hipSuccess) return fail(SN_ERR_DEVICE);
  for (auto& e : h->ev)
    if (hipEventCreate(&e) != hipSuccess) return fail(SN_ERR_DEVICE);
  for (auto& e : h->ev_dom)
    if (hipEventCreate(&e) != hipSuccess) return fail(SN_ERR_DEVICE);
  if (hipEventCreateWithFlags(&h->ev_stats, hipEventDisableTiming) != hipSuccess) return fail(SN_ERR_DEVICE);
  if (c.precision == SN_PREC_AUTO)
    for (auto& p : h->chk)
      if (dalloc(&p, (size_t)H * W) != hipSuccess) return fail(SN_ERR_NOMEM);
  int prio = 0;
  {
    int least = 0, greatest = 0;
    const bool want = sw.stream_priority != kSwitchUnset ? sw.stream_priority == 1 : stream_prio == 1;
    if (want && hipDeviceGetStreamPriorityRange(&least, &greatest) == hipSuccess) prio = greatest;
  }
  h->stream_prio = prio != 0;
  auto mk_stream = [&](hipStream_t* st) {
    return prio != 0 ? hipStreamCreateWithPriority(st, hipStreamNonBlocking, prio) : hipStreamCreateWithFlags(st, hipStreamNonBlocking);
  };
  if (mk_stream(&h->s_low) != hipSuccess ||
      hipEventCreateWithFlags(&h->ev_fork, hipEventDisableTiming) != hipSuccess ||
      hipEventCreateWithFlags(&h->ev_join, hipEventDisableTiming) != hipSuccess)
    return fail(SN_ERR_DEVICE);
  for (int i = 0; i < kMaxTowerStreams; ++i)
    if (mk_stream(&h->s_tow[i]) != hipSuccess ||
        hipEventCreateWithFlags(&h->ev_tow_join[i], hipEventDisableTiming) != hipSuccess)
      return fail(SN_ERR_DEVICE);
  for (auto& e : h->ev_piece)
    if (hipEventCreateWithFlags(&e, hipEventDisableTiming) != hipSuccess) return fail(SN_ERR_DEVICE);
  h->overlap = !sw.no_overlap;
  h->use_graphs = !sw.no_graph;
  h->fuse_mode = sw.fuse;
  h->tail_fuse = sw.tail_fuse;
  if (hipMalloc(reinterpret_cast<void**>(&h->dump), 4096) != hipSuccess) return fail(SN_ERR_NOMEM);

  BlobWalker bw{blob.data()};
  const bool low_x3 = h->precision != SN_PREC_FP32;
  const unsigned abl_w = sw.ablate_w;
#if SN_DIAGNOSTICS
  h->ablate_x = sw.ablate_x;
#endif
  int feat_idx = 0;
  h->fold_down01 = low_x3 && sw.down01;
  HostLayer hl_down0{};
  for (int i = 0; i < kNDown; ++i) {
    const HostLayer hl_ = bw.next(kC, i == 0 ? 3 : kC, 25);
    if ((rc = upload_conv2d(h, hl_, 4, &h->down[i]))) return fail(rc);
    if (low_x3 && i == 0 && (rc = upload_down0_f16(h, hl_, &h->down0))) return fail(rc);
    if (i == 0) hl_down0 = hl_;
    if (h->fold_down01 && i == 1 && (rc = upload_down01(h, hl_down0, hl_, &h->down01))) return fail(rc);
    if (low_x3 && i > 0 &&
        (rc = upload_x3(h, kC, [&](int co, int c, int tap) { return hl_.w[((size_t)co * kC + c) * 25 + tap]; },
                        &h->down[i], 25, (abl_w >> (kAblDown + i - 1)) & 1u)))
      return fail(rc);
  }
  auto up2d = [&](ConvLayer* L) -> int {
    const HostLayer hl_ = bw.next(kC, kC, 9);
    int r = upload_conv2d(h, hl_, 8, L);
    if (r || !low_x3) return r;
    const bool z = (abl_w >> (kAblFeat + feat_idx)) & 1u;
    ++feat_idx;
    return upload_x3(h, kC, [&](int co, int c, int tap) { return hl_.w[((size_t)co * kC + c) * 9 + tap]; }, L, 9, z);
  };
  for (int i = 0; i < kNFeatRes; ++i)
    for (int j = 0; j < 2; ++j)
      if ((rc = up2d(&h->fres[i][j]))) return fail(rc);
  if ((rc = up2d(&h->fout))) return fail(rc);
  for (int i = 0; i < kNAgg; ++i) {
    const HostLayer hl_ = bw.next(kC, kC, 27);
    if ((rc = upload_conv3d(h, hl_, &h->agg[i]))) return fail(rc);
    if (low_x3 && (rc = upload_x3(h, 96, [&](int co, int c, int tap) {
          return hl_.w[(((size_t)co * kC + (c & 31)) * 3 + (c >> 5)) * 9 + tap];
        }, &h->agg[i], 9, (abl_w >> (kAblAgg + i)) & 1u)))
      return fail(rc);
  }
  {
    const HostLayer hl_ = bw.next(1, kC, 27);
    if ((rc = upload_head(h, hl_, &h->aout))) return fail(rc);
    if (low_x3 && (rc = upload_agg_head_frag(h, hl_, &h->aout))) return fail(rc);
  }
  for (int lv = 0; lv < h->levels; ++lv) {
    Tower& T = h->tw[lv];
    {
      const HostLayer hl_ = bw.next(kC, 4, 9);
      if ((rc = upload_conv2d(h, hl_, 4, &T.rin))) return fail(rc);
      if (h->precision != SN_PREC_FP32 && (rc = upload_refin_f16(h, hl_, &T.refin))) return fail(rc);
    }
    for (int i = 0; i < kNRefRes; ++i)
      for (int j = 0; j < 2; ++j) {
        const HostLayer hl_ = bw.next(kC, kC, 9);
        if (h->precision == SN_PREC_FP32 && (rc = upload_conv2d(h, hl_, 8, &T.rres[i][j]))) return fail(rc);
        if (want_x3 && (rc = upload_ref_f16x3(h, hl_, &T.rres16x3[i][j]))) return fail(rc);
        if (want_f16 && (rc = upload_ref_f16(h, hl_, sw.w_round_sum_preserving, &T.rres16[i][j]))) return fail(rc);
      }
    if ((rc = upload_head_split(h, bw.next(1, kC, 9), &T.rout))) return fail(rc);
  }
  if (bw.off != blob.size()) return fail(SN_ERR_FORMAT);

  if ((rc = alloc_ws(h, &h->ws, h->max_batch, h->refine_chunk, h->tower_streams, h->refine_chunk_x3)))
    return fail(rc == SN_ERR_DEVICE ? SN_ERR_NOMEM : rc);
  *out = h;
  return SN_OK;
}

int sn_destroy(sn_handle* h) {
  if (!h) return SN_ERR_ARG;
  if (h->temporal_live.load() > 0) {
    set_err(h, "sn_destroy: the handle still has temporal filters (sn_temporal_destroy them first)");
    return SN_ERR_BUSY;
  }
  if (h->rectify_live.load() > 0) {
    set_err(h, "sn_destroy: the handle still has rectifiers (sn_rectify_destroy them first)");
    return SN_ERR_BUSY;
  }
  hipSetDevice(h->device);
  hipDeviceSynchronize();
  auto free_conv = [](ConvLayer& l) {
    hipFree(l.wx3);
    hipFree(l.wpk);
    hipFree(l.bias);
  };
  for (auto& l : h->down) free_conv(l);
  hipFree(h->down0.wfrag);
  hipFree(h->down01.wfrag);
  hipFree(h->down01.bias);
  for (auto& b : h->fres)
    for (auto& l : b) free_conv(l);
  free_conv(h->fout);
  for (auto& l : h->agg) free_conv(l);
  for (auto& T : h->tw) {
    hipFree(T.refin.wfrag);
    free_conv(T.rin);
    for (auto& b : T.rres)
      for (auto& l : b) free_conv(l);
    for (auto& b : T.rres16)
      for (auto& l : b) {
        hipFree(l.wfrag);
        hipFree(l.bias);
      }
    for (auto& b : T.rres16x3)
      for (auto& l : b) {
        hipFree(l.wfrag);
        hipFree(l.bias);
      }
    if (T.rout.wsplit != T.rout.w) hipFree(T.rout.wsplit);
    hipFree(T.rout.w);
  }
  hipFree(h->dump);
  h->pc.destroy();
  h->flt.destroy();
  h->smo.destroy();
  h->jpg.destroy();
  for (GrowBuf& b : h->stage.buf) b.release();
  hipFree(h->aout.w);
  hipFree(h->aout.pfrag);
  for (auto p : h->chk) hipFree(p);
  if (h->ev_stats) hipEventDestroy(h->ev_stats);
  free_ws(&h->ws);
  for (auto& s : h->slots) {
    free_ws(&s.ws);
    if (s.pin_in) hipHostFree(s.pin_in);
    if (s.pin_raw) hipHostFree(s.pin_raw);
    if (s.pin_disp) hipHostFree(s.pin_disp);
    for (auto& gk : s.gexec)
      for (auto& gm : gk)
        for (auto& g : gm)
          if (g) hipGraphExecDestroy(g);
    if (s.ev0) hipEventDestroy(s.ev0);
    if (s.ev1) hipEventDestroy(s.ev1);
    if (s.stream) hipStreamDestroy(s.stream);
  }
  for (auto& e : h->ev)
    if (e) hipEventDestroy(e);
  for (auto& e : h->ev_dom)
    if (e) hipEventDestroy(e);
  for (auto& e : h->ev_piece)
    if (e) hipEventDestroy(e);
  if (h->ev_fork) hipEventDestroy(h->ev_fork);
  if (h->ev_join) hipEventDestroy(h->ev_join);
  if (h->s_low) hipStreamDestroy(h->s_low);
  for (auto& st : h->s_tow)
    if (st) hipStreamDestroy(st);
  for (auto& e : h->ev_tow_join)
    if (e) hipEventDestroy(e);
  if (h->stream) hipStreamDestroy(h->stream);
  delete h;
  return SN_OK;
}

int sn_get_io_info(const sn_handle* h, sn_io_info* info) {
  if (!h || !info) return SN_ERR_ARG;
  memset(info, 0, sizeof *info);
  info->width = h->W;
  info->height = h->H;
  info->dmax = h->D;
  info->in_channels = 6;
  info->max_batch = h->max_batch;
  info->precision = h->precision;
  info->task_num = h->task_num;
  info->device = h->device;
  info->out_scale = kOutScale;
  info->in_bytes = (size_t)6 * h->H * h->W;
  info->out_bytes = (size_t)4 * h->H * h->W;
  double mac = 0;
  const double wp = h->Wp, hp = h->Hp, wl = h->wl, hl = h->hl, dl = h->Dl;
  for (int k = 1; k <= kNDown; ++k) mac += 2.0 * (wp * hp / (double)(1 << (2 * k))) * kC * (k == 1 ? 3 : kC) * 25;
  mac += 2.0 * (2 * kNFeatRes + 1) * wl * hl * kC * kC * 9;
  mac += kNAgg * dl * hl * wl * kC * kC * 27 + dl * hl * wl * kC * 27;
  for (int k = 0; k < h->levels; ++k)
    mac += (wp * hp / (double)(1 << (2 * k))) * (4.0 * kC * 9 + 2.0 * kNRefRes * kC * kC * 9 + kC * 9);
  info->flops_per_pair = 2.0 * mac;
  info->refine_levels = h->levels;
  info->precision_selected = h->precision == SN_PREC_AUTO ? h->actl.st.mode : h->precision;
  info->refine_chunk = chunk_pairs(h, h->ws, info->precision_selected);
  info->piece = h->ws.pb;
  info->tower_streams = h->ws.ns;
  return SN_OK;
}

int sn_abi_version(void) { return SN_ABI_VERSION; }

double sn_auto_envelope_px(int refine_levels) { return refine_levels > 1 ? kAutoEnvelopeMulti : kAutoEnvelopeSingle; }

int sn_auto_init(sn_auto_state* s, int refine_levels) {
  if (!s) return SN_ERR_ARG;
  s->mode = SN_PREC_F16;
  s->calm = 0;
  s->envelope_px = sn_auto_envelope_px(refine_levels);
  s->epe_per_px = 0.0;
  s->running_px = -1.0;
  s->switches = 0;
  return SN_OK;
}

double sn_auto_limit_px(const sn_auto_state* s) {
  if (!s) return 0.0;
  if (!(s->epe_per_px > 0.0)) return s->envelope_px;
  const double own = SN_AUTO_BUDGET_PX / s->epe_per_px;
  return own < s->envelope_px ? own : s->envelope_px;
}

int sn_auto_observe(sn_auto_state* s, double residual_px) {
  if (!s) return SN_ERR_ARG;
  if (!(residual_px >= 0.0) || residual_px > kAutoResidualCap) residual_px = kAutoResidualCap;
  s->running_px = s->running_px < 0.0 ? residual_px : 0.75 * s->running_px + 0.25 * residual_px;
  const double lim = sn_auto_limit_px(s);
  if (s->mode == SN_PREC_F16) {
    if (residual_px > lim) {
      s->mode = SN_PREC_F16X3;
      s->calm = 0;
      ++s->switches;
    }
  } else {
    if (residual_px < SN_AUTO_REENTRY * lim) {
      if (++s->calm >= SN_AUTO_CALM_CALLS) {
        s->mode = SN_PREC_F16;
        s->calm = 0;
        ++s->switches;
      }
    } else {
      s->calm = 0;
    }
  }
  return s->mode;
}

int sn_get_refine_stats(sn_handle* h, sn_refine_stats* out) {
  if (!h || !out) return SN_ERR_ARG;
  int rc = check_device(h);
  if (rc) return rc;
  if ((rc = fold_pending(h, true))) return rc;
  std::lock_guard<std::mutex> lk(h->mu);
  const AutoCtl& a = h->actl;
  memset(out, 0, sizeof *out);
  out->levels = h->levels;
  out->precision = h->precision;
  out->precision_selected = h->precision == SN_PREC_AUTO ? a.st.mode : h->precision;
  out->precision_last = a.last_mode;
  out->calls = a.calls;
  out->pairs = a.pairs;
  out->switches = a.st.switches;
  out->reruns = a.reruns;
  for (int lv = 0; lv < kMaxLevels; ++lv) out->level_px[lv] = a.last_level[lv];
  out->residual_px = a.last_res;
  out->running_px = a.st.running_px < 0.0 ? 0.0 : a.st.running_px;
  out->envelope_px = a.st.envelope_px;
  out->limit_px = sn_auto_limit_px(&a.st);
  out->selfcheck_epe_px = a.selfcheck_epe;
  out->selfcheck_residual_px = a.selfcheck_res;
  for (int lv = 0; lv < kMaxLevels; ++lv) out->nonfinite_px[lv] = a.last_range.level[lv];
  out->nonfinite_low_px = a.last_range.low;
  return SN_OK;
}

int sn_infer_batch(sn_handle* h, int n, const int8_t* in, int32_t* out_i32, float* out_disp, int mem,
                   void* stream) {
  if (!h) return SN_ERR_ARG;
  if (!in || (!out_i32 && !out_disp) || n <= 0 || n > h->max_batch) {
    set_err(h, "sn_infer_batch: bad arguments");
    return SN_ERR_ARG;
  }
  Call c;
  const int rc = enter(h, "sn_infer_batch", mem, stream, &h->stream, &c);
  if (rc) return rc;
  hipStream_t st = c.st;
  const size_t HW = (size_t)h->H * h->W;
  const int8_t* din = in;
  int32_t* draw = out_i32;
  float* ddisp = out_disp;
  if (c.host) {
    HIP_TRY(h, hipMemcpyAsync(h->ws.in6, in, (size_t)n * 6 * HW, hipMemcpyHostToDevice, st));
    din = h->ws.in6;
    draw = out_i32 ? h->ws.out_raw : nullptr;
    ddisp = out_disp ? h->ws.out_disp : nullptr;
  }
  auto post = [&]() -> int {
    if (c.host) {
      if (out_i32) HIP_TRY(h, hipMemcpyAsync(out_i32, draw, (size_t)n * HW * 4, hipMemcpyDeviceToHost, st));
      if (out_disp) HIP_TRY(h, hipMemcpyAsync(out_disp, ddisp, (size_t)n * HW * 4, hipMemcpyDeviceToHost, st));
    }
    return SN_OK;
  };
  return run_forward(h, st, n, din, ddisp, draw, n == 1, c.blocking, post);
}

int sn_infer_i8(sn_handle* h, const int8_t* in, int32_t* out_i32, float* out_disp, int mem, void* stream) {
  return sn_infer_batch(h, 1, in, out_i32, out_disp, mem, stream);
}

int sn_preprocess_nv12(sn_handle* h, const uint8_t* left, const uint8_t* right, int w, int h_px,
                       int8_t* out6, int mem, void* stream) {
  if (!h) return SN_ERR_ARG;
  if (!left || !right || !out6 || w <= 0 || h_px <= 0 || (w & 3) || (h_px & 1) ||
      (size_t)w * h_px > (size_t)h->W * h->H) {
    set_err(h, "sn_preprocess_nv12: bad arguments");
    return SN_ERR_ARG;
  }
  Call c;
  const int rc = enter(h, "sn_preprocess_nv12", mem, stream, &h->stream, &c);
  if (rc) return rc;
  hipStream_t st = c.st;
  const size_t eye = (size_t)w * h_px * 3 / 2;
  const uint8_t *dl = left, *dr = right;
  int8_t* dout = out6;
  if (c.host) {
    HIP_TRY(h, hipMemcpyAsync(h->ws.nv12, left, eye, hipMemcpyHostToDevice, st));
    HIP_TRY(h, hipMemcpyAsync(h->ws.nv12 + eye, right, eye, hipMemcpyHostToDevice, st));
    dl = h->ws.nv12;
    dr = h->ws.nv12 + eye;
    dout = h->ws.in6;
  } else if (((uintptr_t)left | (uintptr_t)right | (uintptr_t)out6) & 3) {
    return SN_ERR_ARG;
  }
  launch_pre_nv12(st, dl, dr, w, w, h_px, dout);
  HIP_TRY(h, hipGetLastError());
  if (c.host) HIP_TRY(h, hipMemcpyAsync(out6, dout, (size_t)6 * w * h_px, hipMemcpyDeviceToHost, st));
  if (c.blocking) HIP_TRY(h, hipStreamSynchronize(st));
  return SN_OK;
}

int sn_infer_sbs_nv12(sn_handle* h, const uint8_t* sbs, int w2, int h_px, int32_t* out_i32, float* out_disp,
                      int8_t* out_tensor, int mem, void* stream) {
  if (!h) return SN_ERR_ARG;
  if (!sbs || (!out_i32 && !out_disp) || !sbs_frame_ok(h, w2, h_px)) {
    set_err(h, "sn_infer_sbs_nv12: image size does not match the model input");
    return SN_ERR_ARG;
  }
  Call c;
  const int rc = enter(h, "sn_infer_sbs_nv12", mem, stream, &h->stream, &c);
  if (rc) return rc;
  hipStream_t st = c.st;
  const size_t HW = (size_t)h->H * h->W;
  const uint8_t* dsrc = sbs;
  if (c.host) {
    HIP_TRY(h, hipMemcpyAsync(h->ws.nv12, sbs, HW * 3, hipMemcpyHostToDevice, st));
    dsrc = h->ws.nv12;
  } else if ((uintptr_t)sbs & 3) {
    return SN_ERR_ARG;
  }
  int8_t* din = (!c.host && out_tensor) ? out_tensor : h->ws.in6;
  launch_pre_nv12(st, dsrc, dsrc + w2 / 2, w2, w2 / 2, h_px, din);
  HIP_TRY(h, hipGetLastError());
  int32_t* draw = out_i32;
  float* ddisp = out_disp;
  if (c.host) {
    draw = out_i32 ? h->ws.out_raw : nullptr;
    ddisp = out_disp ? h->ws.out_disp : nullptr;
  }
  auto post = [&]() -> int {
    if (c.host) {
      if (out_i32) HIP_TRY(h, hipMemcpyAsync(out_i32, draw, HW * 4, hipMemcpyDeviceToHost, st));
      if (out_disp) HIP_TRY(h, hipMemcpyAsync(out_disp, ddisp, HW * 4, hipMemcpyDeviceToHost, st));
      if (out_tensor) HIP_TRY(h, hipMemcpyAsync(out_tensor, din, HW * 6, hipMemcpyDeviceToHost, st));
    }
    return SN_OK;
  };
  return run_forward(h, st, 1, din, ddisp, draw, true, c.blocking, post);
}

int sn_preprocess_sbs_nv12_batch(sn_handle* h, int n, const uint8_t* sbs, int w2, int h_px, int8_t* out6, int mem,
                                 void* stream) {
  if (!h) return SN_ERR_ARG;
  if (!sbs || !out6 || n <= 0 || !sbs_frame_ok(h, w2, h_px) || (mem == SN_MEM_HOST && n > h->max_batch)) {
    set_err(h, "sn_preprocess_sbs_nv12_batch: bad arguments");
    return SN_ERR_ARG;
  }
  if (mem == SN_MEM_DEVICE && (((uintptr_t)sbs | (uintptr_t)out6) & 3)) return SN_ERR_ARG;
  Call c;
  int rc = enter(h, "sn_preprocess_sbs_nv12_batch", mem, stream, &h->stream, &c);
  if (rc) return rc;
  const size_t HW = (size_t)h->H * h->W;
  if ((rc = sbs_to_tensors(h, c.st, n, sbs, w2, h_px, c.host, c.host ? h->ws.in6 : out6))) return rc;
  if (c.host) HIP_TRY(h, hipMemcpyAsync(out6, h->ws.in6, (size_t)n * 6 * HW, hipMemcpyDeviceToHost, c.st));
  if (c.blocking) HIP_TRY(h, hipStreamSynchronize(c.st));
  return SN_OK;
}

static int ensure_slots(sn_handle* h) {
  if (!h->slots.empty()) return SN_OK;
  const size_t HW = (size_t)h->H * h->W;
  h->slots.resize(h->task_num);
  for (auto& s : h->slots) {
    HIP_TRY(h, hipStreamCreateWithFlags(&s.stream, hipStreamNonBlocking));
    HIP_TRY(h, hipEventCreate(&s.ev0));
    HIP_TRY(h, hipEventCreate(&s.ev1));
    int rc = alloc_ws(h, &s.ws, 1, 1, 1, 1);
    if (rc) return rc;
    HIP_TRY(h, hipHostMalloc(reinterpret_cast<void**>(&s.pin_in), 6 * HW, hipHostMallocDefault));
    HIP_TRY(h, hipHostMalloc(reinterpret_cast<void**>(&s.pin_raw), 4 * HW, hipHostMallocDefault));
    HIP_TRY(h, hipHostMalloc(reinterpret_cast<void**>(&s.pin_disp), 4 * HW, hipHostMallocDefault));
  }
  return SN_OK;
}

struct SlotGuard {
  sn_handle* h;
  Slot* s;
  bool take_mu;
  bool armed = true;
  ~SlotGuard() {
    if (!armed) return;
    if (take_mu) h->mu.lock();
    s->ticket = 0;
    if (take_mu) h->mu.unlock();
    h->cv.notify_one();
  }
};

static int submit_common(sn_handle* h, const void* in, int kind, int32_t* out_i32, float* out_disp, int timeout_ms,
                         uint64_t* ticket) {
  if (!h || !in || (!out_i32 && !out_disp) || !ticket) return SN_ERR_ARG;
  std::unique_lock<std::mutex> lk(h->mu);
  int rc = check_device(h);
  if (rc) return rc;
  if ((rc = ensure_slots(h))) return rc;
  Slot* s = nullptr;
  auto find_free = [&]() {
    for (auto& c : h->slots)
      if (c.ticket == 0) {
        s = &c;
        return true;
      }
    return false;
  };
  if (timeout_ms < 0) {
    h->cv.wait(lk, find_free);
  } else if (!h->cv.wait_for(lk, std::chrono::milliseconds(timeout_ms), find_free)) {
    return SN_ERR_BUSY;
  }
  const size_t HW = (size_t)h->H * h->W;
  s->ticket = h->next_ticket++;
  s->user_raw = out_i32;
  s->user_disp = out_disp;
  SlotGuard guard{h, s, false};
  memcpy(s->pin_in, in, (kind == 1 ? 3 : 6) * HW);
  const int mask = (out_i32 ? 1 : 0) | (out_disp ? 2 : 0);
  const int mode = h->precision == SN_PREC_AUTO ? h->actl.st.mode : h->precision;
  int others = 0;
  for (auto& c : h->slots)
    if (&c != s && c.ticket != 0) ++others;
  const int shared = (others > 0 && switches().async_share) ? 1 : 0;
  s->ws.tower_cu = shared ? h->num_cu * 7 / 8 : 0;
  const int mi = (mode == SN_PREC_F16X3 ? 0 : 2) + shared;
  s->mode_run = mode;
  auto enqueue = [&]() -> int {
    if (kind == 1) {
      HIP_TRY(h, hipMemcpyAsync(s->ws.nv12, s->pin_in, 3 * HW, hipMemcpyHostToDevice, s->stream));
      launch_pre_nv12(s->stream, s->ws.nv12, s->ws.nv12 + h->W, 2 * h->W, h->W, h->H, s->ws.in6);
      HIP_TRY(h, hipGetLastError());
    } else {
      HIP_TRY(h, hipMemcpyAsync(s->ws.in6, s->pin_in, 6 * HW, hipMemcpyHostToDevice, s->stream));
    }
    const bool prof = h->profiling;
    h->profiling = false;
    const int r = forward(h, s->ws, s->stream, 1, s->ws.in6, out_disp ? s->ws.out_disp : nullptr,
                          out_i32 ? s->ws.out_raw : nullptr, false, mode);
    h->profiling = prof;
    if (r) return r;
    if (out_i32) HIP_TRY(h, hipMemcpyAsync(s->pin_raw, s->ws.out_raw, 4 * HW, hipMemcpyDeviceToHost, s->stream));
    if (out_disp) HIP_TRY(h, hipMemcpyAsync(s->pin_disp, s->ws.out_disp, 4 * HW, hipMemcpyDeviceToHost, s->stream));
    return SN_OK;
  };
  if (h->use_graphs && !s->gexec[kind][mask][mi] && s->uses[kind][mask][mi] >= 1) {
    hipGraph_t graph = nullptr;
    if (hipStreamBeginCapture(s->stream, hipStreamCaptureModeThreadLocal) == hipSuccess) {
      const int r = enqueue();
      const hipError_t e = hipStreamEndCapture(s->stream, &graph);
      if (r == SN_OK && e == hipSuccess && graph &&
          hipGraphInstantiate(&s->gexec[kind][mask][mi], graph, nullptr, nullptr, 0) != hipSuccess)
        s->gexec[kind][mask][mi] = nullptr;
      if (graph) hipGraphDestroy(graph);
    }
    if (!s->gexec[kind][mask][mi]) {
      (void)hipGetLastError();
      h->use_graphs = false;
    }
  }
  HIP_TRY(h, hipEventRecord(s->ev0, s->stream));
  if (s->gexec[kind][mask][mi]) {
    HIP_TRY(h, hipGraphLaunch(s->gexec[kind][mask][mi], s->stream));
  } else {
    rc = enqueue();
    if (rc) return rc;
    ++s->uses[kind][mask][mi];
  }
  HIP_TRY(h, hipEventRecord(s->ev1, s->stream));
  guard.armed = false;
  *ticket = s->ticket;
  return SN_OK;
}

int sn_submit(sn_handle* h, const int8_t* in, int32_t* out_i32, float* out_disp, int timeout_ms,
              uint64_t* ticket) {
  return submit_common(h, in, 0, out_i32, out_disp, timeout_ms, ticket);
}

int sn_submit_nv12(sn_handle* h, const uint8_t* sbs, int w2, int h_px, int32_t* out_i32, float* out_disp,
                   int timeout_ms, uint64_t* ticket) {
  if (!h) return SN_ERR_ARG;
  if (!sbs_frame_ok(h, w2, h_px)) {
    set_err(h, "sn_submit_nv12: image size does not match the model input");
    return SN_ERR_ARG;
  }
  return submit_common(h, sbs, 1, out_i32, out_disp, timeout_ms, ticket);
}

int sn_wait(sn_handle* h, uint64_t ticket, float* infer_ms) {
  if (!h || ticket == 0) return SN_ERR_ARG;
  Slot* s = nullptr;
  {
    std::lock_guard<std::mutex> lk(h->mu);
    for (auto& c : h->slots)
      if (c.ticket == ticket) s = &c;
  }
  if (!s) return SN_ERR_TICKET;
  SlotGuard guard{h, s, true};
  hipSetDevice(h->device);
  HIP_TRY(h, hipEventSynchronize(s->ev1));
  const size_t HW = (size_t)h->H * h->W;
  auto rerun = [&]() -> int {
    const int r = forward(h, s->ws, s->stream, 1, s->ws.in6, s->user_disp ? s->ws.out_disp : nullptr,
                          s->user_raw ? s->ws.out_raw : nullptr, false, SN_PREC_F16X3);
    if (r) return r;
    if (s->user_raw) HIP_TRY(h, hipMemcpyAsync(s->pin_raw, s->ws.out_raw, 4 * HW, hipMemcpyDeviceToHost, s->stream));
    if (s->user_disp) HIP_TRY(h, hipMemcpyAsync(s->pin_disp, s->ws.out_disp, 4 * HW, hipMemcpyDeviceToHost, s->stream));
    HIP_TRY(h, hipEventRecord(s->ev1, s->stream));
    HIP_TRY(h, hipEventSynchronize(s->ev1));
    return SN_OK;
  };
  const bool check = h->precision == SN_PREC_AUTO && s->mode_run == SN_PREC_F16;
  RangeCount range;
  if (const int rc = settle(h, s->ws, s->stream, 1, s->ws.in6, s->mode_run, check, true, rerun, &range)) return rc;
  float ms = 0.f;
  if (infer_ms) HIP_TRY(h, hipEventElapsedTime(&ms, s->ev0, s->ev1));
  if (infer_ms) *infer_ms = ms;
  if (s->user_raw) memcpy(s->user_raw, s->pin_raw, 4 * HW);
  if (s->user_disp) memcpy(s->user_disp, s->pin_disp, 4 * HW);
  return range_result(h, range);
}

int sn_synchronize(sn_handle* h) {
  if (!h) return SN_ERR_ARG;
  int rc = check_device(h);
  if (rc) return rc;
  HIP_TRY(h, hipStreamSynchronize(h->stream));
  for (auto& s : h->slots) HIP_TRY(h, hipStreamSynchronize(s.stream));
  return SN_OK;
}

int sn_set_profiling(sn_handle* h, int enable) {
  if (!h) return SN_ERR_ARG;
  h->profiling = enable != 0;
  return SN_OK;
}

int sn_get_stage_ms(sn_handle* h, float* ms, int count) {
  if (!h || !ms || count <= 0) return SN_ERR_ARG;
  for (int i = 0; i < count && i < SN_STAGE_COUNT; ++i) ms[i] = h->stage_ms[i];
  return SN_OK;
}

int sn_get_dominant_kernel(sn_handle* h, char* name, size_t cap, int* launches, double* flops, double* bytes) {
  if (!h) return SN_ERR_ARG;
  const int cur = h->precision == SN_PREC_AUTO ? h->actl.st.mode : h->precision;
  const bool f16 = cur == SN_PREC_F16;
  const double px = (double)h->Hp * h->Wp * chunk_pairs(h, h->ws, cur);
  if (f16 && h->fuse_mode == 4) {
    int n = 0;
    for (int i = 0; i < kNRefRes; ++i) {
      const bool last = i == kNRefRes - 1;
      if (stream_block_supports(kRefDil[i]) && !(last && h->tail_fuse)) ++n;
    }
    if (n > 0) {
      if (name && cap)
        snprintf(name, cap, "%s", "k_ref_block_stream_f16<DIL> (fused residual block: two 3x3 C->C convs + residual, fp16 MFMA 32x32x16)");
      if (launches) *launches = n;
      if (flops) *flops = 2.0 * (2.0 * px * kC * kC * 9);
      if (bytes) *bytes = px * kC * 2.0 * 2.0;
      return SN_OK;
    }
  }
  if (cur == SN_PREC_F16X3) {
    int n = 0;
    for (int i = 0; i < kNRefRes; ++i)
      if (stream_x3_supports(kRefDil[i])) ++n;
    if (n > 0) {
      if (name && cap)
        snprintf(name, cap, "%s", "k_ref_block_stream_x3<DIL> (fused residual block: two 3x3 C->C convs + residual, 3 fp16 MFMAs 32x32x16 "
                                  "per product on hi/lo split operands; the FLOPs counted are the model's, not the three products')");
      if (launches) *launches = n;
      if (flops) *flops = 2.0 * (2.0 * px * kC * kC * 9);
      if (bytes) *bytes = px * kC * 4.0 * 2.0;
      return SN_OK;
    }
  }
  if (name && cap)
    snprintf(name, cap, "%s",
             cur == SN_PREC_F16     ? "k_ref_conv_f16<DIL> (refinement 3x3 C->C, fp16 MFMA 32x32x16)"
             : cur == SN_PREC_F16X3 ? "k_ref_conv_f16x3<DIL> (refinement 3x3 C->C, 3x fp16 MFMA on hi/lo split operands)"
                                             : "k_ref_conv_f32<DIL> (refinement 3x3 C->C, weights-stationary, fp32 MFMA 32x32x2)");
  const int n_plain = kNRefRes, n_res = kNRefRes;
  if (launches) *launches = n_plain + n_res;
  if (flops) *flops = 2.0 * px * kC * kC * 9;
  if (bytes) *bytes = px * kC * (f16 ? 2.0 : 4.0) * (2.0 * n_plain + 3.0 * n_res) / (double)(n_plain + n_res);
  return SN_OK;
}

}
```

### include/stereonet_hip.h

```cpp
#ifndef STEREONET_HIP_H_
#define STEREONET_HIP_H_

#include <stddef.h>
#include <stdint.h>

#ifdef __cplusplus
extern "C" {
#endif

typedef struct sn_handle sn_handle;

#define SN_ABI_VERSION 4
int sn_abi_version(void);

enum {
  SN_OK = 0,
  SN_ERR_ARG = -1,
  SN_ERR_FILE = -2,
  SN_ERR_FORMAT = -3,
  SN_ERR_DEVICE = -4,
  SN_ERR_NOMEM = -5,
  SN_ERR_BUSY = -6,
  SN_ERR_TICKET = -7,
  SN_ERR_RANGE = -8
};

enum { SN_MEM_HOST = 0, SN_MEM_DEVICE = 1 };

enum {
  SN_PREC_DEFAULT = 0,
  SN_PREC_F16X3 = 1,
  SN_PREC_F16 = 2,
  SN_PREC_FP32 = 3,
  SN_PREC_AUTO = 4
};

typedef struct sn_config {
  int device;
  int max_batch;
  int width;
  int height;
  int dmax;
  int precision;
  int task_num;
  int refine_chunk;
  int piece;
} sn_config;

typedef struct sn_io_info {
  int width, height, dmax;
  int in_channels;
  int max_batch, precision, task_num, device;
  float out_scale;
  size_t in_bytes;
  size_t out_bytes;
  double flops_per_pair;
  int refine_chunk;
  int piece;
  int tower_streams;
  int refine_levels;
  int precision_selected;
} sn_io_info;

int sn_create(const char *model_file, const sn_config *cfg, sn_handle **out);
int sn_destroy(sn_handle *h);
int sn_get_io_info(const sn_handle *h, sn_io_info *info);
const char *sn_strerror(int code);
const char *sn_last_error(const sn_handle *h);

typedef struct sn_refine_stats {
  int levels;
  int precision;
  int precision_selected;
  int precision_last;
  uint64_t calls, pairs;
  uint64_t switches;
  uint64_t reruns;
  double level_px[4];
  double residual_px;
  double running_px;
  double envelope_px;
  double limit_px;
  double selfcheck_epe_px;
  double selfcheck_residual_px;
  uint64_t nonfinite_px[4];
  uint64_t nonfinite_low_px;
} sn_refine_stats;
int sn_get_refine_stats(sn_handle *h, sn_refine_stats *out);

#define SN_AUTO_BUDGET_PX 0.85e-3
#define SN_AUTO_REENTRY 0.8
#define SN_AUTO_CALM_CALLS 8
typedef struct sn_auto_state {
  int mode;
  int calm;
  double envelope_px;
  double epe_per_px;
  double running_px;
  uint64_t switches;
} sn_auto_state;
double sn_auto_envelope_px(int refine_levels);
int sn_auto_init(sn_auto_state *s, int refine_levels);
double sn_auto_limit_px(const sn_auto_state *s);
int sn_auto_observe(sn_auto_state *s, double residual_px);

int sn_infer_i8(sn_handle *h, const int8_t *in_nchw6, int32_t *out_i32, float *out_disp,
                int mem, void *stream);
int sn_infer_batch(sn_handle *h, int n, const int8_t *in_nchw6, int32_t *out_i32, float *out_disp,
                   int mem, void *stream);

int sn_preprocess_nv12(sn_handle *h, const uint8_t *left_nv12, const uint8_t *right_nv12,
                       int w, int h_px, int8_t *out_nchw6, int mem, void *stream);
int sn_infer_sbs_nv12(sn_handle *h, const uint8_t *sbs_nv12, int w2, int h_px, int32_t *out_i32,
                      float *out_disp, int8_t *out_tensor, int mem, void *stream);

int sn_preprocess_sbs_nv12_batch(sn_handle *h, int n, const uint8_t *sbs_nv12, int w2, int h_px, int8_t *out_nchw6,
                                 int mem, void *stream);

int sn_submit(sn_handle *h, const int8_t *in_nchw6_host, int32_t *out_i32_host, float *out_disp_host,
              int timeout_ms, uint64_t *ticket);
int sn_submit_nv12(sn_handle *h, const uint8_t *sbs_nv12_host, int w2, int h_px, int32_t *out_i32_host,
                   float *out_disp_host, int timeout_ms, uint64_t *ticket);
int sn_wait(sn_handle *h, uint64_t ticket, float *infer_ms);
int sn_synchronize(sn_handle *h);

typedef struct sn_mgpu sn_mgpu;
int sn_mgpu_shard(int n, int ndev, int k, int *first, int *count);
int sn_mgpu_create(const char *model_file, const sn_config *cfg, const int *devices, int ndev, sn_mgpu **out);
int sn_mgpu_destroy(sn_mgpu *m);
int sn_mgpu_get_info(const sn_mgpu *m, int *ndev, int *per_device_batch, int *gather_kind );
int sn_mgpu_get_handle(sn_mgpu *m, int k, sn_handle **h);
int sn_mgpu_infer_batch(sn_mgpu *m, int n, const int8_t *in_nchw6_host, int32_t *out_i32_host, float *out_disp_host);
int sn_mgpu_infer_batch_device(sn_mgpu *m, int n, const int8_t *const *in_per_device, int32_t *out_i32_root,
                               float *out_disp_root);
int sn_mgpu_submit_device(sn_mgpu *m, int n, const int8_t *const *in_per_device, int32_t *out_i32_root,
                          float *out_disp_root, uint64_t *ticket);
int sn_mgpu_wait(sn_mgpu *m, uint64_t ticket);
const char *sn_mgpu_last_error(const sn_mgpu *m);
#define SN_MGPU_SLOTS 2
typedef struct sn_mgpu_ring {
  uint64_t next;
  uint64_t slot_ticket[SN_MGPU_SLOTS];
} sn_mgpu_ring;
int sn_mgpu_ring_init(sn_mgpu_ring *r);
int sn_mgpu_ring_submit(sn_mgpu_ring *r, uint64_t *ticket, int *slot);
int sn_mgpu_ring_wait(sn_mgpu_ring *r, uint64_t ticket, int *slot);

enum {
  SN_STAGE_FEATURES = 0,
  SN_STAGE_AGGREGATE = 1,
  SN_STAGE_REFINE = 2,
  SN_STAGE_REFINE_CONV = 3,
  SN_STAGE_TOTAL = 4,
  SN_STAGE_DOMINANT = 5,
  SN_STAGE_COUNT = 6
};
int sn_set_profiling(sn_handle *h, int enable);
int sn_get_stage_ms(sn_handle *h, float *ms, int count);
int sn_get_dominant_kernel(sn_handle *h, char *name, size_t name_cap, int *launches,
                           double *flops_per_launch, double *bytes_per_launch);

int sn_dbg_conv2d(sn_handle *h, const float *in, int cin, int h_px, int w, const float *wt,
                  const float *bias, int k, int stride, int dil, int lrelu, const float *residual,
                  float *out);
int sn_dbg_down0(sn_handle *h, const int8_t *in6, int h_px, int w, const float *wt, const float *bias, int tc,
                 float *out);
int sn_dbg_round_kernels_f16(const float *w, int nkernels, float *out);
int sn_dbg_compose_down01(const float *w0, const float *b0, const float *w1, const float *b1, float *weff,
                          float *beff);
int sn_dbg_down01(sn_handle *h, const int8_t *in6, int h_px, int w, const float *w0, const float *b0,
                  const float *w1, const float *b1, float *out);
int sn_dbg_refin(sn_handle *h, const float *disp_low, const int8_t *in6, int h_px, int w, int dmax,
                 const float *wt, const float *bias, int split, float *out);
int sn_dbg_conv3d(sn_handle *h, const float *in, int d, int h_px, int w, const float *wt,
                  const float *bias, int lrelu, float *out);
int sn_dbg_ref_conv_f16(sn_handle *h, const float *in, int h_px, int w, const float *wt, const float *bias,
                        int dil, int lrelu, const float *residual, float *out);
int sn_dbg_ref_conv_f16x3(sn_handle *h, const float *in, int h_px, int w, const float *wt, const float *bias,
                          int dil, int lrelu, const float *residual, float *out);
int sn_dbg_ref_block_f16(sn_handle *h, const float *in, int h_px, int w, const float *w1, const float *b1,
                         const float *w2, const float *b2, int dil, float *out);
int sn_dbg_ref_block_f16x3(sn_handle *h, const float *in, int h_px, int w, const float *w1, const float *b1,
                           const float *w2, const float *b2, int dil, int form, float *out);
int sn_dbg_ref_tail_f16(sn_handle *h, int n, const float *in, int hk, int wk, const float *w1, const float *b1,
                        const float *w2, const float *b2, const float *head_w, float head_b, const float *low, int ups,
                        float dnorm, int h_out, int w_out, int form, float *out_disp, int32_t *out_raw);
int sn_dbg_read(sn_handle *h, const char *what, float *dst, size_t cap, size_t *n);
int sn_depth_from_raw(sn_handle *h, int n, const int32_t *raw, float focal_px, float baseline_mm, float *depth_m,
                      float *disp_px, int mem, void *stream);

typedef struct sn_camera {
  float fx, fy, cx, cy;
  float baseline_mm;
  float z_min_m, z_max_m;
  int step;
} sn_camera;
enum { SN_PC_ORGANISED = 0, SN_PC_COMPACT = 1 };
int sn_pointcloud_from_raw(sn_handle *h, int n, const int32_t *raw, const uint8_t *nv12, int nv12_pitch,
                           const sn_camera *cam, int layout, float *points, uint32_t *counts, int mem, void *stream);

typedef struct sn_lrc_params {
  float tau_px;
  float tau_rel;
  int   right_mirrored;
} sn_lrc_params;
enum { SN_LRC_KEPT = 0, SN_LRC_INVALID_IN = 1, SN_LRC_OUT_OF_VIEW = 2, SN_LRC_NO_PARTNER = 4, SN_LRC_INCONSISTENT = 8 };
enum { SN_LRC_IN_TENSOR = 0, SN_LRC_IN_SBS_NV12 = 1 };
int sn_mirror_pair_i8(sn_handle *h, int n, const int8_t *in_nchw6, int8_t *out_nchw6, int mem, void *stream);
int sn_lr_check(sn_handle *h, int n, const int32_t *raw_left, const int32_t *raw_right, const sn_lrc_params *p,
                int32_t *out_raw, float *disp_inout, uint8_t *mask, uint32_t *kept, int mem, void *stream);
int sn_infer_lrc(sn_handle *h, int n, const void *in, int in_kind, int w2, int h_px, const sn_lrc_params *p,
                 int32_t *out_i32, float *out_disp, int32_t *out_right_i32, uint8_t *mask, uint32_t *kept,
                 int mem, void *stream);

typedef struct sn_conf_params { float min_conf; } sn_conf_params;
enum { SN_CONF_KEPT = 0, SN_CONF_INVALID_IN = 1, SN_CONF_LOW = 64 };
int sn_infer_conf(sn_handle *h, int n, const void *in, int in_kind, int w2, int h_px, const sn_conf_params *p,
                  int32_t *out_i32, float *out_disp, float *out_conf, uint8_t *mask, uint32_t *kept,
                  int mem, void *stream);
int sn_conf_mask(sn_handle *h, int n, const int32_t *raw, const float *conf, const sn_conf_params *p,
                 int32_t *out_raw, float *disp_inout, uint8_t *mask, uint32_t *kept, int mem, void *stream);

typedef struct sn_filter_params {
  int   speckle_max_px;
  float speckle_diff_px;
  int   fill_max_px;
} sn_filter_params;
enum { SN_FLT_INVALID_IN = 1, SN_FLT_SPECKLE = 16, SN_FLT_FILLED = 32 };
int sn_filter_raw(sn_handle *h, int n, const int32_t *raw, const sn_filter_params *p, int32_t *out_raw,
                  float *disp_inout, uint8_t *mask, uint32_t *counts, int mem, void *stream);

typedef struct sn_smooth_params {
  int radius;
  int sigma_luma;
  int min_valid;
} sn_smooth_params;
enum { SN_SMOOTH_INVALID_IN = 1, SN_SMOOTH_CHANGED = 128 };
enum { SN_GUIDE_NV12 = 0, SN_GUIDE_TENSOR = 1 };
int sn_smooth_raw(sn_handle *h, int n, const int32_t *raw, const void *guide, int guide_kind, int guide_pitch,
                  const sn_smooth_params *p, int32_t *out_raw, float *disp_inout, uint8_t *mask, uint32_t *counts,
                  int mem, void *stream);

typedef struct sn_temporal_params {
  int   alpha;
  float delta_px;
  int   persist;
  int   luma_delta;
} sn_temporal_params;
enum { SN_TMP_INVALID_IN = 1, SN_TMP_BLENDED = 2, SN_TMP_HELD = 4, SN_TMP_MOVED = 8, SN_TMP_JUMP = 16 };
typedef struct sn_temporal sn_temporal;
int  sn_temporal_create(sn_handle *h, int streams, const sn_temporal_params *p, sn_temporal **out);
int  sn_temporal_reset(sn_temporal *t, int stream);
void sn_temporal_destroy(sn_temporal *t);
int  sn_temporal_push(sn_temporal *t, int n, const int *stream_of, const int32_t *raw, const void *guide, int guide_kind,
                      int guide_pitch, int32_t *out_raw, float *disp_inout, uint8_t *mask, uint32_t *counts, int mem,
                      void *stream);

typedef struct sn_eye_calib { double fx, fy, cx, cy; double d[5]; double R[9]; } sn_eye_calib;
typedef struct sn_stereo_calib {
  int src_w, src_h;
  sn_eye_calib left, right;
  double pfx, pfy, pcx, pcy;
  double baseline_mm;
} sn_stereo_calib;
typedef struct sn_rectify sn_rectify;
typedef struct sn_rectify_info { int src_w, src_h, w, h; uint32_t valid_left, valid_right; } sn_rectify_info;
int  sn_rectify_build_map(const sn_stereo_calib *c, int eye, int w, int h, int32_t *map_xy);
int  sn_rectify_create(sn_handle *h, const sn_stereo_calib *c, sn_rectify **out);
void sn_rectify_destroy(sn_rectify *r);
int  sn_rectify_get_info(const sn_rectify *r, sn_rectify_info *info);
int  sn_rectify_get_camera(const sn_rectify *r, sn_camera *cam);
int  sn_rectify_get_map(sn_rectify *r, int eye, int32_t *map_xy_host);
int  sn_rectify_nv12(sn_rectify *r, int n, const uint8_t *left, const uint8_t *right, int src_pitch, size_t src_frame,
                     uint8_t *out_sbs_nv12, int8_t *out_nchw6, int mem, void *stream);

typedef struct sn_jpeg_params { int quality; int rows_per_slice; } sn_jpeg_params;
size_t sn_jpeg_bound(int w, int h_px);
int  sn_jpeg_encode_nv12(sn_handle *h, int n, const uint8_t *nv12, int w, int h_px, int pitch, size_t frame,
                         const sn_jpeg_params *p, uint8_t *out, size_t out_stride, uint32_t *sizes, int mem, void *stream);
int  sn_dbg_jpeg_dct(sn_handle *h, const uint8_t *nv12, int w, int h_px, int pitch, float *out);

int sn_dbg_copy_limited(void *dst, const void *src, size_t bytes, int workgroups, void *stream);

#ifdef __cplusplus
}
#endif
#endif
```

Baseline: 3068.

## Coalesce async submissions into batched group launches via dispatcher queue

Adds an async queue with a dispatcher thread that gathers ready submitted pairs and issues them as one batched forward on dedicated group lanes, with up to two groups in flight. Per-pair launches are replaced by grouped launches so per-call launch and graph overhead is amortised and larger batches fill the GPU. It also moves the AUTO-mode statistics settling to per-group records and adds a rerun lane. The price is an extra thread, more synchronisation, added latency while a group is assembled, and more complex error and ticket handling.

```diff
diff --git a/hobot_stereonet_amd/csrc/sn_async_queue.hpp b/hobot_stereonet_amd/csrc/sn_async_queue.hpp
--- /dev/null
+++ b/hobot_stereonet_amd/csrc/sn_async_queue.hpp
@@ -0,0 +1,312 @@
+#pragma once
+
+#include <algorithm>
+#include <chrono>
+#include <condition_variable>
+#include <cstdint>
+#include <mutex>
+#include <thread>
+#include <vector>
+
+namespace sn_async {
+
+constexpr int kMaxInFlight = 2;
+constexpr int kMaxGroup = 64;
+constexpr int kBusy = -1000001;
+
+enum SlotState { kFree = 0, kStaging, kReady, kIssuing, kIssued, kFailed };
+
+struct Launch {
+  uint64_t id = 0;
+  int rec = -1;
+  int k = 0;
+  int lane = -1;
+  int others = 0;
+  int slot[kMaxGroup] = {};
+};
+
+struct Backend {
+  virtual ~Backend() {}
+  virtual void thread_begin() {}
+  virtual int issue(const Launch& l) = 0;
+  virtual void wait_done(const Launch& l) = 0;
+  virtual bool done(const Launch& l) = 0;
+};
+
+class Queue {
+ public:
+  Queue(int nslots, Backend* be, int max_group)
+      : be_(be), slots_(nslots), recs_(nslots + kMaxInFlight), hist_(nslots + 1, 0),
+        max_group_(max_group < 1 ? 1 : (max_group > kMaxGroup ? kMaxGroup : max_group)) {}
+  ~Queue() { stop(); }
+  Queue(const Queue&) = delete;
+  Queue& operator=(const Queue&) = delete;
+
+  int nslots() const { return (int)slots_.size(); }
+  int nrecs() const { return (int)recs_.size(); }
+
+  void start(bool threaded) {
+    threaded_ = threaded;
+    if (threaded) thread_ = std::thread([this] { run(); });
+  }
+  void stop() {
+    {
+      std::lock_guard<std::mutex> lk(mu_);
+      stop_ = true;
+    }
+    cv_disp_.notify_all();
+    cv_user_.notify_all();
+    if (thread_.joinable()) thread_.join();
+  }
+
+  int claim(int timeout_ms, int* slot, uint64_t* ticket) {
+    std::unique_lock<std::mutex> lk(mu_);
+    int found = -1;
+    auto find_free = [&] {
+      for (int i = 0; i < (int)slots_.size(); ++i)
+        if (slots_[i].state == kFree) {
+          found = i;
+          return true;
+        }
+      return false;
+    };
+    if (timeout_ms < 0) {
+      cv_user_.wait(lk, find_free);
+    } else if (!find_free()) {
+      if (timeout_ms == 0 ||
+          !cv_user_.wait_until(lk, std::chrono::system_clock::now() + std::chrono::milliseconds(timeout_ms), find_free))
+        return kBusy;
+    }
+    S& s = slots_[found];
+    s.state = kStaging;
+    s.ticket = next_ticket_++;
+    s.rec = -1;
+    s.rc = 0;
+    *slot = found;
+    *ticket = s.ticket;
+    return 0;
+  }
+  void ready(int slot) {
+    {
+      std::lock_guard<std::mutex> lk(mu_);
+      slots_[slot].state = kReady;
+    }
+    cv_disp_.notify_one();
+  }
+  void abandon(int slot) {
+    {
+      std::lock_guard<std::mutex> lk(mu_);
+      slots_[slot] = S();
+    }
+    cv_disp_.notify_one();
+    cv_user_.notify_all();
+  }
+  int issue_direct(int slot) {
+    std::lock_guard<std::mutex> issue_lk(issue_mu_);
+    Launch l;
+    {
+      std::lock_guard<std::mutex> lk(mu_);
+      slots_[slot].state = kIssuing;
+      const int one[1] = {slot};
+      make_launch(one, 1, &l);
+    }
+    const int rc = be_->issue(l);
+    {
+      std::lock_guard<std::mutex> lk(mu_);
+      finish_issue(l, rc);
+      recs_[l.rec].retired = true;
+      reap(l.rec);
+    }
+    cv_user_.notify_all();
+    return rc;
+  }
+
+  int find(uint64_t ticket) {
+    std::lock_guard<std::mutex> lk(mu_);
+    for (int i = 0; i < (int)slots_.size(); ++i)
+      if (slots_[i].state != kFree && slots_[i].ticket == ticket) return i;
+    return -1;
+  }
+  int wait_issued(int slot, Launch* l) {
+    std::unique_lock<std::mutex> lk(mu_);
+    cv_user_.wait(lk, [&] { return slots_[slot].state == kIssued || slots_[slot].state == kFailed || stop_; });
+    const S& s = slots_[slot];
+    if (s.state == kFailed) return s.rc;
+    if (s.state != kIssued) return kBusy;
+    *l = recs_[s.rec].l;
+    return 0;
+  }
+  bool begin_settle(int rec, int* rc) {
+    std::unique_lock<std::mutex> lk(mu_);
+    R& r = recs_[rec];
+    if (r.settle == 0) {
+      r.settle = 1;
+      return true;
+    }
+    cv_user_.wait(lk, [&] { return r.settle == 2; });
+    *rc = r.verdict;
+    return false;
+  }
+  void end_settle(int rec, int rc) {
+    {
+      std::lock_guard<std::mutex> lk(mu_);
+      recs_[rec].settle = 2;
+      recs_[rec].verdict = rc;
+    }
+    cv_user_.notify_all();
+  }
+  void release(int slot) {
+    {
+      std::lock_guard<std::mutex> lk(mu_);
+      const int rec = slots_[slot].rec;
+      slots_[slot] = S();
+      if (rec >= 0) {
+        --recs_[rec].refs;
+        reap(rec);
+      }
+    }
+    cv_disp_.notify_one();
+    cv_user_.notify_all();
+  }
+
+  void drain() {
+    std::unique_lock<std::mutex> lk(mu_);
+    cv_user_.wait(lk, [&] {
+      if (stop_) return true;
+      for (const S& s : slots_)
+        if (s.state == kStaging || s.state == kIssuing || (s.state == kReady && threaded_)) return false;
+      return true;
+    });
+  }
+  int launches_by_size(uint64_t* out, int cap) {
+    std::lock_guard<std::mutex> lk(mu_);
+    for (int i = 0; i < cap; ++i) out[i] = i + 1 < (int)hist_.size() ? hist_[i + 1] : 0;
+    return (int)slots_.size();
+  }
+
+ private:
+  struct S {
+    int state = kFree;
+    uint64_t ticket = 0;
+    int rec = -1;
+    int rc = 0;
+  };
+  struct R {
+    Launch l;
+    bool used = false, retired = false;
+    int refs = 0;
+    int settle = 0;
+    int verdict = 0;
+  };
+
+  void make_launch(const int* slot, int k, Launch* l) {
+    int rec = 0;
+    while (recs_[rec].used) ++rec;
+    R& r = recs_[rec];
+    r = R();
+    r.used = true;
+    r.refs = k;
+    l->id = next_launch_++;
+    l->rec = rec;
+    l->k = k;
+    l->lane = -1;
+    if (k >= 2) {
+      bool taken[kMaxInFlight] = {};
+      for (int f : flight_)
+        if (recs_[f].l.lane >= 0) taken[recs_[f].l.lane] = true;
+      for (int i = kMaxInFlight - 1; i >= 0; --i)
+        if (!taken[i]) l->lane = i;
+    }
+    l->others = 0;
+    for (const S& s : slots_)
+      if (s.state != kFree) ++l->others;
+    l->others -= k;
+    for (int i = 0; i < k; ++i) {
+      l->slot[i] = slot[i];
+      slots_[slot[i]].rec = rec;
+    }
+    r.l = *l;
+    ++hist_[k];
+  }
+  void finish_issue(const Launch& l, int rc) {
+    for (int i = 0; i < l.k; ++i) {
+      S& s = slots_[l.slot[i]];
+      s.state = rc ? kFailed : kIssued;
+      s.rc = rc;
+    }
+  }
+  int groups_in_flight() const {
+    int n = 0;
+    for (int f : flight_)
+      if (recs_[f].l.lane >= 0) ++n;
+    return n;
+  }
+  void retire_front() {
+    const int rec = flight_.front();
+    flight_.erase(flight_.begin());
+    recs_[rec].retired = true;
+    reap(rec);
+  }
+  void reap(int rec) {
+    R& r = recs_[rec];
+    if (r.used && r.retired && r.refs <= 0) r.used = false;
+  }
+
+  void run() {
+    be_->thread_begin();
+    std::unique_lock<std::mutex> lk(mu_);
+    while (!stop_) {
+      while (!flight_.empty() && be_->done(recs_[flight_.front()].l)) retire_front();
+      uint64_t fence = UINT64_MAX;
+      for (const S& s : slots_)
+        if (s.state == kStaging && s.ticket < fence) fence = s.ticket;
+      int take[kMaxGroup], k = 0;
+      std::vector<int> cand;
+      for (int i = 0; i < (int)slots_.size(); ++i)
+        if (slots_[i].state == kReady && slots_[i].ticket < fence) cand.push_back(i);
+      if (cand.empty()) {
+        cv_disp_.wait(lk);
+        continue;
+      }
+      if (cand.size() >= 2 && max_group_ >= 2 && groups_in_flight() >= kMaxInFlight) {
+        const Launch l = recs_[flight_.front()].l;
+        lk.unlock();
+        be_->wait_done(l);
+        lk.lock();
+        retire_front();
+        continue;
+      }
+      std::sort(cand.begin(), cand.end(), [&](int a, int b) { return slots_[a].ticket < slots_[b].ticket; });
+      for (int i : cand)
+        if (k < max_group_) take[k++] = i;
+      for (int i = 0; i < k; ++i) slots_[take[i]].state = kIssuing;
+      Launch l;
+      make_launch(take, k, &l);
+      flight_.push_back(l.rec);
+      lk.unlock();
+      const int rc = be_->issue(l);
+      lk.lock();
+      finish_issue(l, rc);
+      if (rc) {
+        flight_.erase(std::find(flight_.begin(), flight_.end(), l.rec));
+        recs_[l.rec].retired = true;
+        reap(l.rec);
+      }
+      cv_user_.notify_all();
+    }
+  }
+
+  Backend* be_;
+  std::mutex mu_, issue_mu_;
+  std::condition_variable cv_user_, cv_disp_;
+  std::vector<S> slots_;
+  std::vector<R> recs_;
+  std::vector<int> flight_;
+  std::vector<uint64_t> hist_;
+  uint64_t next_ticket_ = 1, next_launch_ = 1;
+  const int max_group_;
+  bool threaded_ = false, stop_ = false;
+  std::thread thread_;
+};
+
+}
diff --git a/hobot_stereonet_amd/csrc/sn_dbg_hooks.hpp b/hobot_stereonet_amd/csrc/sn_dbg_hooks.hpp
--- a/hobot_stereonet_amd/csrc/sn_dbg_hooks.hpp
+++ b/hobot_stereonet_amd/csrc/sn_dbg_hooks.hpp
@@ -625,6 +625,18 @@
   return hipGetLastError() == hipSuccess ? SN_OK : SN_ERR_DEVICE;
 }
 
+int sn_dbg_async_launches(sn_handle* h, uint64_t* by_size, int cap) {
+  if (!h || !by_size || cap <= 0) return SN_ERR_ARG;
+  sn_async::Queue* q;
+  {
+    std::lock_guard<std::mutex> lk(h->mu);
+    q = h->aq.get();
+  }
+  for (int i = 0; i < cap; ++i) by_size[i] = 0;
+  if (q) q->launches_by_size(by_size, cap);
+  return SN_OK;
+}
+
 int sn_dbg_read(sn_handle* h, const char* what, float* dst, size_t cap, size_t* n) {
   if (!h || !what || !n) return SN_ERR_ARG;
   int rc = check_device(h);
diff --git a/hobot_stereonet_amd/csrc/sn_engine.hpp b/hobot_stereonet_amd/csrc/sn_engine.hpp
--- a/hobot_stereonet_amd/csrc/sn_engine.hpp
+++ b/hobot_stereonet_amd/csrc/sn_engine.hpp
@@ -147,14 +147,13 @@
 
 struct Slot {
   hipStream_t stream = nullptr;
-  hipEvent_t ev0 = nullptr, ev1 = nullptr;
   Workspace ws;
   int8_t* pin_in = nullptr;
   int32_t* pin_raw = nullptr;
   float* pin_disp = nullptr;
   int32_t* user_raw = nullptr;
   float* user_disp = nullptr;
-  uint64_t ticket = 0;
+  int kind = 0;
   hipGraphExec_t gexec[2][4][4] = {};
   int uses[2][4][4] = {};
   int mode_run = 0;
@@ -163,6 +162,21 @@
 struct RangeCount {
   unsigned long long level[4] = {}, low = 0;
   bool any() const { return (level[0] | level[1] | level[2] | level[3] | low) != 0; }
+};
+
+struct GroupLane {
+  Workspace ws;
+  hipStream_t stream = nullptr;
+  uint8_t* nv12 = nullptr;
+};
+constexpr int kGroupLanes = sn_async::kMaxInFlight + 1;
+
+struct AsyncRec {
+  hipEvent_t ev0 = nullptr, ev1 = nullptr;
+  int mode = 0;
+  bool snap = false;
+  std::vector<unsigned long long> stats;
+  RangeCount range;
 };
 
 struct AutoCtl {
@@ -214,8 +228,13 @@
   Workspace ws;
   std::vector<Slot> slots;
   std::mutex mu;
-  std::condition_variable cv;
-  uint64_t next_ticket = 1;
+  bool coalesce = true;
+  int group_rb = 1, group_rb_x3 = 1;
+  std::unique_ptr<sn_async::Backend> abe;
+  std::unique_ptr<sn_async::Queue> aq;
+  std::vector<AsyncRec> arec;
+  GroupLane glane[kGroupLanes];
+  std::mutex mu_snap, mu_repeat;
   bool profiling = false;
   hipEvent_t ev[8] = {};
   hipEvent_t ev_dom[2 * 6] = {};
diff --git a/hobot_stereonet_amd/csrc/sn_forward.hpp b/hobot_stereonet_amd/csrc/sn_forward.hpp
--- a/hobot_stereonet_amd/csrc/sn_forward.hpp
+++ b/hobot_stereonet_amd/csrc/sn_forward.hpp
@@ -484,10 +484,10 @@
 }
 
 int forward(sn_handle* h, Workspace& ws, hipStream_t st, int n, const int8_t* in6, float* out_disp,
-            int32_t* out_raw, bool want_cost, int mode = 0, bool want_conf = false) {
+            int32_t* out_raw, bool want_cost, int mode = 0, bool want_conf = false, bool no_prof = false) {
   if (mode == 0) mode = h->precision == SN_PREC_AUTO ? h->actl.st.mode : h->precision;
   const int rb = chunk_pairs(h, ws, mode);
-  const bool prof = h->profiling && (&ws == &h->ws);
+  const bool prof = !no_prof && h->profiling && (&ws == &h->ws);
   const bool piped = !prof && (&ws == &h->ws) && h->overlap && n > rb;
   int rc;
   int ctr_block = 0;
@@ -650,14 +650,11 @@
     std::lock_guard<std::mutex> lk(h->mu);
     if (h->actl.calibrated) return SN_OK;
   }
-  const bool prof = h->profiling;
-  h->profiling = false;
   double lvl[kMaxLevels], res = 0.0;
   RangeCount range_x3, range;
-  int rc = forward(h, ws, st, 1, in6_pair, h->chk[1], nullptr, false, SN_PREC_F16X3);
+  int rc = forward(h, ws, st, 1, in6_pair, h->chk[1], nullptr, false, SN_PREC_F16X3, false, true);
   if (!rc && hipStreamSynchronize(st) == hipSuccess) read_stats(h, ws, 1, lvl, &res, &range_x3);
-  if (!rc) rc = forward(h, ws, st, 1, in6_pair, h->chk[0], nullptr, false, SN_PREC_F16);
-  h->profiling = prof;
+  if (!rc) rc = forward(h, ws, st, 1, in6_pair, h->chk[0], nullptr, false, SN_PREC_F16, false, true);
   if (rc) return rc;
   const size_t HW = (size_t)h->H * h->W;
   HIP_TRY(h, hipMemsetAsync(ws.stats + 4 * kStatWordStride, 0, kStatWordStride * sizeof(unsigned long long), st));
diff --git a/hobot_stereonet_amd/csrc/sn_switches.hpp b/hobot_stereonet_amd/csrc/sn_switches.hpp
--- a/hobot_stereonet_amd/csrc/sn_switches.hpp
+++ b/hobot_stereonet_amd/csrc/sn_switches.hpp
@@ -42,6 +42,7 @@
   int stream_priority = kSwitchUnset;
   bool no_overlap = false;
   bool no_graph = false;
+  bool async_coalesce = true;
   bool tail_fuse = true;
   int mgpu_gather = 0;
   bool mgpu_allow_dup = false;
@@ -119,6 +120,7 @@
   s->stream_priority = equals("SN_STREAM_PRIORITY", "") ? kSwitchUnset : int_or("SN_STREAM_PRIORITY", kSwitchUnset);
   s->no_overlap = present("SN_NO_OVERLAP");
   s->no_graph = present("SN_NO_GRAPH");
+  s->async_coalesce = on_unless_zero("SN_ASYNC_COALESCE");
   s->tail_fuse = on_unless_zero("SN_TAIL_FUSE");
   s->mgpu_gather = equals("SN_MGPU_GATHER", "peer") ? 1 : equals("SN_MGPU_GATHER", "rccl") ? 2 : 0;
   s->mgpu_allow_dup = int_or("SN_MGPU_ALLOW_DUP", 0) == 1;
diff --git a/hobot_stereonet_amd/csrc/stereonet_hip.hip b/hobot_stereonet_amd/csrc/stereonet_hip.hip
--- a/hobot_stereonet_amd/csrc/stereonet_hip.hip
+++ b/hobot_stereonet_amd/csrc/stereonet_hip.hip
@@ -18,6 +18,7 @@
 #include "../../include/stereonet_hip.h"
 #include "sn_internal.h"
 #include "sn_switches.hpp"
+#include "sn_async_queue.hpp"
 #include "sn_kernels.hpp"
 #include "sn_pointcloud.hpp"
 #include "sn_lrcheck.hpp"
@@ -49,6 +50,19 @@
     case SN_ERR_RANGE: return "activations left the range of fp16 (65504): the maps are not valid; use SN_PREC_FP32 for this model";
     default: return "unknown error";
   }
+}
+
+static bool tensors_fit32(const sn_handle* h, int nb, int rb) {
+  const int pb = piece_pairs(h, nb, rb);
+  const double low_elems = 2.0 * pb * kC * (h->Hp / 2.0) * (h->Wp / 2.0);
+  const double vol_elems = (double)pb * h->Dl * kC * h->hl * h->wl;
+  double ref_bytes = 0;
+  for (int lv = 0; lv < h->levels; ++lv) {
+    const RefGeom& rg = h->tw[lv].rg;
+    const double b = ((double)level_chunk_pairs(rb, pb, lv) * 4.0 * rg.Hs * rg.Ws + (double)ref_slack(rg) + (double)ref_front(rg)) * 16.0;
+    if (b > ref_bytes) ref_bytes = b;
+  }
+  return low_elems < 4.0e9 && ref_bytes < 4.0e9 && vol_elems < 4.0e9;
 }
 
 static thread_local std::string g_create_err;
@@ -174,24 +188,21 @@
     h->refine_chunk = rc_auto < 1 ? 1 : (rc_auto > 8 ? 8 : rc_auto);
   }
   h->num_cu = prop.multiProcessorCount > 0 ? prop.multiProcessorCount : 256;
+  h->group_rb = h->refine_chunk;
+  h->group_rb_x3 = h->refine_chunk_x3;
   if (h->refine_chunk > h->max_batch) h->refine_chunk = h->max_batch;
   if (h->refine_chunk_x3 > h->refine_chunk) h->refine_chunk_x3 = h->refine_chunk;
 
-  {
-    const int pb = piece_pairs(h, h->max_batch, h->refine_chunk);
-    const double low_elems = 2.0 * pb * kC * (h->Hp / 2.0) * (h->Wp / 2.0);
-    const double vol_elems = (double)pb * h->Dl * kC * h->hl * h->wl;
-    double ref_bytes = 0;
-    for (int lv = 0; lv < h->levels; ++lv) {
-      const RefGeom& rg = h->tw[lv].rg;
-      const double b = ((double)level_chunk_pairs(h->refine_chunk, pb, lv) * 4.0 * rg.Hs * rg.Ws + (double)ref_slack(rg) + (double)ref_front(rg)) * 16.0;
-      if (b > ref_bytes) ref_bytes = b;
-    }
-    if (low_elems >= 4.0e9 || ref_bytes >= 4.0e9 || vol_elems >= 4.0e9) {
-      delete h;
-      return SN_ERR_ARG;
-    }
-  }
+  if (!tensors_fit32(h, h->max_batch, h->refine_chunk)) {
+    delete h;
+    return SN_ERR_ARG;
+  }
+  if (h->group_rb > h->task_num) h->group_rb = h->task_num;
+  if (h->group_rb_x3 > h->group_rb) h->group_rb_x3 = h->group_rb;
+  while (h->group_rb > 1 && !tensors_fit32(h, h->task_num, h->group_rb)) --h->group_rb;
+  if (!tensors_fit32(h, h->task_num, h->group_rb)) h->group_rb = 0;
+  if (h->group_rb_x3 > h->group_rb) h->group_rb_x3 = h->group_rb;
+  h->coalesce = sw.async_coalesce;
   int rc = check_device(h);
   auto fail = [&](int code) {
     create_fail(code, h->err.empty() ? "engine set-up" : h->err.c_str());
@@ -314,6 +325,7 @@
     return SN_ERR_BUSY;
   }
   hipSetDevice(h->device);
+  if (h->aq) h->aq->stop();
   hipDeviceSynchronize();
   auto free_conv = [](ConvLayer& l) {
     hipFree(l.wx3);
@@ -366,9 +378,16 @@
       for (auto& gm : gk)
         for (auto& g : gm)
           if (g) hipGraphExecDestroy(g);
-    if (s.ev0) hipEventDestroy(s.ev0);
-    if (s.ev1) hipEventDestroy(s.ev1);
     if (s.stream) hipStreamDestroy(s.stream);
+  }
+  for (auto& r : h->arec) {
+    if (r.ev0) hipEventDestroy(r.ev0);
+    if (r.ev1) hipEventDestroy(r.ev1);
+  }
+  for (auto& g : h->glane) {
+    free_ws(&g.ws);
+    hipFree(g.nv12);
+    if (g.stream) hipStreamDestroy(g.stream);
   }
   for (auto& e : h->ev)
     if (e) hipEventDestroy(e);
@@ -616,86 +635,105 @@
   return SN_OK;
 }
 
+static int issue_one(sn_handle* h, const sn_async::Launch& l);
+static int issue_group(sn_handle* h, const sn_async::Launch& l);
+static void snapshot_stats(sn_handle* h, const sn_async::Launch& l);
+
+namespace {
+struct AsyncBackend : sn_async::Backend {
+  sn_handle* h;
+  explicit AsyncBackend(sn_handle* h_) : h(h_) {}
+  void thread_begin() override { (void)hipSetDevice(h->device); }
+  int issue(const sn_async::Launch& l) override { return l.k == 1 ? issue_one(h, l) : issue_group(h, l); }
+  void wait_done(const sn_async::Launch& l) override {
+    (void)hipEventSynchronize(h->arec[l.rec].ev1);
+    snapshot_stats(h, l);
+  }
+  bool done(const sn_async::Launch& l) override {
+    if (hipEventQuery(h->arec[l.rec].ev1) == hipErrorNotReady) {
+      (void)hipGetLastError();
+      return false;
+    }
+    (void)hipGetLastError();
+    snapshot_stats(h, l);
+    return true;
+  }
+};
+}
+
 static int ensure_slots(sn_handle* h) {
-  if (!h->slots.empty()) return SN_OK;
+  if (h->aq) return SN_OK;
   const size_t HW = (size_t)h->H * h->W;
-  h->slots.resize(h->task_num);
-  for (auto& s : h->slots) {
-    HIP_TRY(h, hipStreamCreateWithFlags(&s.stream, hipStreamNonBlocking));
-    HIP_TRY(h, hipEventCreate(&s.ev0));
-    HIP_TRY(h, hipEventCreate(&s.ev1));
-    int rc = alloc_ws(h, &s.ws, 1, 1, 1, 1);
-    if (rc) return rc;
-    HIP_TRY(h, hipHostMalloc(reinterpret_cast<void**>(&s.pin_in), 6 * HW, hipHostMallocDefault));
-    HIP_TRY(h, hipHostMalloc(reinterpret_cast<void**>(&s.pin_raw), 4 * HW, hipHostMallocDefault));
-    HIP_TRY(h, hipHostMalloc(reinterpret_cast<void**>(&s.pin_disp), 4 * HW, hipHostMallocDefault));
-  }
+  if (h->slots.empty()) {
+    h->slots.resize(h->task_num);
+    for (auto& s : h->slots) {
+      HIP_TRY(h, hipStreamCreateWithFlags(&s.stream, hipStreamNonBlocking));
+      int rc = alloc_ws(h, &s.ws, 1, 1, 1, 1);
+      if (rc) return rc;
+      HIP_TRY(h, hipHostMalloc(reinterpret_cast<void**>(&s.pin_in), 6 * HW, hipHostMallocDefault));
+      HIP_TRY(h, hipHostMalloc(reinterpret_cast<void**>(&s.pin_raw), 4 * HW, hipHostMallocDefault));
+      HIP_TRY(h, hipHostMalloc(reinterpret_cast<void**>(&s.pin_disp), 4 * HW, hipHostMallocDefault));
+    }
+  }
+  const int max_group = (h->coalesce && h->group_rb > 0) ? h->task_num : 1;
+  auto be = std::make_unique<AsyncBackend>(h);
+  auto q = std::make_unique<sn_async::Queue>(h->task_num, be.get(), max_group);
+  h->arec.resize(q->nrecs());
+  for (auto& r : h->arec) {
+    if (!r.ev0) HIP_TRY(h, hipEventCreate(&r.ev0));
+    if (!r.ev1) HIP_TRY(h, hipEventCreate(&r.ev1));
+    r.stats.assign(kStatU64, 0);
+  }
+  h->abe = std::move(be);
+  h->aq = std::move(q);
+  h->aq->start(h->coalesce);
   return SN_OK;
 }
 
 struct SlotGuard {
   sn_handle* h;
-  Slot* s;
-  bool take_mu;
+  int slot;
   bool armed = true;
   ~SlotGuard() {
-    if (!armed) return;
-    if (take_mu) h->mu.lock();
-    s->ticket = 0;
-    if (take_mu) h->mu.unlock();
-    h->cv.notify_one();
+    if (armed) h->aq->release(slot);
   }
 };
 
-static int submit_common(sn_handle* h, const void* in, int kind, int32_t* out_i32, float* out_disp, int timeout_ms,
-                         uint64_t* ticket) {
-  if (!h || !in || (!out_i32 && !out_disp) || !ticket) return SN_ERR_ARG;
-  std::unique_lock<std::mutex> lk(h->mu);
-  int rc = check_device(h);
-  if (rc) return rc;
-  if ((rc = ensure_slots(h))) return rc;
-  Slot* s = nullptr;
-  auto find_free = [&]() {
-    for (auto& c : h->slots)
-      if (c.ticket == 0) {
-        s = &c;
-        return true;
-      }
-    return false;
-  };
-  if (timeout_ms < 0) {
-    h->cv.wait(lk, find_free);
-  } else if (!h->cv.wait_for(lk, std::chrono::milliseconds(timeout_ms), find_free)) {
-    return SN_ERR_BUSY;
-  }
+static int stage_input(sn_handle* h, const Slot& s, hipStream_t st, uint8_t* nv12, int8_t* in6) {
   const size_t HW = (size_t)h->H * h->W;
-  s->ticket = h->next_ticket++;
-  s->user_raw = out_i32;
-  s->user_disp = out_disp;
-  SlotGuard guard{h, s, false};
-  memcpy(s->pin_in, in, (kind == 1 ? 3 : 6) * HW);
+  if (s.kind == 1) {
+    HIP_TRY(h, hipMemcpyAsync(nv12, s.pin_in, 3 * HW, hipMemcpyHostToDevice, st));
+    launch_pre_nv12(st, nv12, nv12 + h->W, 2 * h->W, h->W, h->H, in6);
+    HIP_TRY(h, hipGetLastError());
+  } else {
+    HIP_TRY(h, hipMemcpyAsync(in6, s.pin_in, 6 * HW, hipMemcpyHostToDevice, st));
+  }
+  return SN_OK;
+}
+
+static int issue_one(sn_handle* h, const sn_async::Launch& l) {
+  Slot* const s = &h->slots[l.slot[0]];
+  AsyncRec& R = h->arec[l.rec];
+  const size_t HW = (size_t)h->H * h->W;
+  const int kind = s->kind;
+  int32_t* const out_i32 = s->user_raw;
+  float* const out_disp = s->user_disp;
   const int mask = (out_i32 ? 1 : 0) | (out_disp ? 2 : 0);
-  const int mode = h->precision == SN_PREC_AUTO ? h->actl.st.mode : h->precision;
-  int others = 0;
-  for (auto& c : h->slots)
-    if (&c != s && c.ticket != 0) ++others;
-  const int shared = (others > 0 && switches().async_share) ? 1 : 0;
+  int mode;
+  {
+    std::lock_guard<std::mutex> lk(h->mu);
+    mode = h->precision == SN_PREC_AUTO ? h->actl.st.mode : h->precision;
+  }
+  const int shared = (l.others > 0 && switches().async_share) ? 1 : 0;
   s->ws.tower_cu = shared ? h->num_cu * 7 / 8 : 0;
   const int mi = (mode == SN_PREC_F16X3 ? 0 : 2) + shared;
   s->mode_run = mode;
+  R.mode = mode;
+  R.snap = false;
   auto enqueue = [&]() -> int {
-    if (kind == 1) {
-      HIP_TRY(h, hipMemcpyAsync(s->ws.nv12, s->pin_in, 3 * HW, hipMemcpyHostToDevice, s->stream));
-      launch_pre_nv12(s->stream, s->ws.nv12, s->ws.nv12 + h->W, 2 * h->W, h->W, h->H, s->ws.in6);
-      HIP_TRY(h, hipGetLastError());
-    } else {
-      HIP_TRY(h, hipMemcpyAsync(s->ws.in6, s->pin_in, 6 * HW, hipMemcpyHostToDevice, s->stream));
-    }
-    const bool prof = h->profiling;
-    h->profiling = false;
+    if (const int r = stage_input(h, *s, s->stream, s->ws.nv12, s->ws.in6)) return r;
     const int r = forward(h, s->ws, s->stream, 1, s->ws.in6, out_disp ? s->ws.out_disp : nullptr,
-                          out_i32 ? s->ws.out_raw : nullptr, false, mode);
-    h->profiling = prof;
+                          out_i32 ? s->ws.out_raw : nullptr, false, mode, false, true);
     if (r) return r;
     if (out_i32) HIP_TRY(h, hipMemcpyAsync(s->pin_raw, s->ws.out_raw, 4 * HW, hipMemcpyDeviceToHost, s->stream));
     if (out_disp) HIP_TRY(h, hipMemcpyAsync(s->pin_disp, s->ws.out_disp, 4 * HW, hipMemcpyDeviceToHost, s->stream));
@@ -716,17 +754,149 @@
       h->use_graphs = false;
     }
   }
-  HIP_TRY(h, hipEventRecord(s->ev0, s->stream));
+  HIP_TRY(h, hipEventRecord(R.ev0, s->stream));
   if (s->gexec[kind][mask][mi]) {
     HIP_TRY(h, hipGraphLaunch(s->gexec[kind][mask][mi], s->stream));
   } else {
-    rc = enqueue();
+    if (const int rc = enqueue()) return rc;
+    ++s->uses[kind][mask][mi];
+  }
+  HIP_TRY(h, hipEventRecord(R.ev1, s->stream));
+  return SN_OK;
+}
+
+static int ensure_lane(sn_handle* h, GroupLane* g) {
+  if (g->stream) return SN_OK;
+  const size_t HW = (size_t)h->H * h->W;
+  hipStream_t st = nullptr;
+  HIP_TRY(h, hipStreamCreateWithFlags(&st, hipStreamNonBlocking));
+  hipError_t e = dalloc(&g->nv12, (size_t)h->task_num * 3 * HW);
+  int rc = e == hipSuccess ? alloc_ws(h, &g->ws, h->task_num, h->group_rb, 1, h->group_rb_x3) : SN_ERR_NOMEM;
+  if (rc) {
+    set_err(h, "group workspace: " + std::string(sn_last_error(h)));
+    free_ws(&g->ws);
+    hipFree(g->nv12);
+    g->nv12 = nullptr;
+    hipStreamDestroy(st);
+    return rc == SN_ERR_DEVICE ? SN_ERR_NOMEM : rc;
+  }
+  g->stream = st;
+  return SN_OK;
+}
+
+static int enqueue_group(sn_handle* h, const sn_async::Launch& l, GroupLane& g, int mode) {
+  const size_t HW = (size_t)h->H * h->W;
+  bool any_raw = false, any_disp = false;
+  for (int i = 0; i < l.k; ++i) {
+    const Slot& s = h->slots[l.slot[i]];
+    if (const int rc = stage_input(h, s, g.stream, g.nv12 + (size_t)i * 3 * HW, g.ws.in6 + (size_t)i * 6 * HW)) return rc;
+    any_raw = any_raw || s.user_raw;
+    any_disp = any_disp || s.user_disp;
+  }
+  if (const int rc = forward(h, g.ws, g.stream, l.k, g.ws.in6, any_disp ? g.ws.out_disp : nullptr, any_raw ? g.ws.out_raw : nullptr,
+                             false, mode, false, true))
+    return rc;
+  for (int i = 0; i < l.k; ++i) {
+    const Slot& s = h->slots[l.slot[i]];
+    if (s.user_raw) HIP_TRY(h, hipMemcpyAsync(s.pin_raw, g.ws.out_raw + (size_t)i * HW, 4 * HW, hipMemcpyDeviceToHost, g.stream));
+    if (s.user_disp) HIP_TRY(h, hipMemcpyAsync(s.pin_disp, g.ws.out_disp + (size_t)i * HW, 4 * HW, hipMemcpyDeviceToHost, g.stream));
+  }
+  return SN_OK;
+}
+
+static int issue_group(sn_handle* h, const sn_async::Launch& l) {
+  if (l.lane < 0 || l.lane >= sn_async::kMaxInFlight || l.k > h->task_num) {
+    set_err(h, "internal: group launch without a lane");
+    return SN_ERR_DEVICE;
+  }
+  GroupLane& g = h->glane[l.lane];
+  AsyncRec& R = h->arec[l.rec];
+  if (const int rc = ensure_lane(h, &g)) return rc;
+  {
+    std::lock_guard<std::mutex> lk(h->mu);
+    R.mode = h->precision == SN_PREC_AUTO ? h->actl.st.mode : h->precision;
+  }
+  {
+    std::lock_guard<std::mutex> lk(h->mu_snap);
+    R.snap = false;
+  }
+  HIP_TRY(h, hipEventRecord(R.ev0, g.stream));
+  if (const int rc = enqueue_group(h, l, g, R.mode)) return rc;
+  HIP_TRY(h, hipEventRecord(R.ev1, g.stream));
+  return SN_OK;
+}
+
+static void snapshot_stats(sn_handle* h, const sn_async::Launch& l) {
+  if (l.k < 2) return;
+  std::lock_guard<std::mutex> lk(h->mu_snap);
+  AsyncRec& R = h->arec[l.rec];
+  if (R.snap) return;
+  const Workspace& ws = h->glane[l.lane].ws;
+  R.stats.assign(ws.stats_host, ws.stats_host + kStatU64);
+  R.snap = true;
+}
+
+static int settle_group(sn_handle* h, const sn_async::Launch& l, AsyncRec& R) {
+  Workspace snap;
+  snap.stats_host = R.stats.data();
+  double lvl[kMaxLevels], res = 0.0;
+  int rc;
+  read_stats(h, snap, l.k, lvl, &res, &R.range);
+  const bool is_auto = h->precision == SN_PREC_AUTO;
+  if (is_auto && R.mode == SN_PREC_F16 && !R.range.any()) {
+    bool calibrated;
+    {
+      std::lock_guard<std::mutex> lk(h->mu);
+      calibrated = h->actl.calibrated;
+    }
+    if (!calibrated) {
+      Slot& s0 = h->slots[l.slot[0]];
+      if ((rc = stage_input(h, s0, s0.stream, s0.ws.nv12, s0.ws.in6))) return rc;
+      if ((rc = auto_selfcheck(h, s0.ws, s0.stream, s0.ws.in6))) return rc;
+    }
+  }
+  for (int i = 0; i < l.k; ++i) count_call(h, 1);
+  const int next = fold_stats(h, lvl, res, R.range, l.k, R.mode);
+  if (is_auto && R.mode == SN_PREC_F16 && next == SN_PREC_F16X3) {
+    std::lock_guard<std::mutex> lk(h->mu_repeat);
+    GroupLane& g = h->glane[kGroupLanes - 1];
+    if ((rc = ensure_lane(h, &g))) return rc;
+    if ((rc = enqueue_group(h, l, g, SN_PREC_F16X3))) return rc;
+    HIP_TRY(h, hipStreamSynchronize(g.stream));
+    read_stats(h, g.ws, l.k, lvl, &res, &R.range);
+    fold_stats(h, lvl, res, R.range, l.k, SN_PREC_F16X3, false);
+  }
+  return SN_OK;
+}
+
+static int submit_common(sn_handle* h, const void* in, int kind, int32_t* out_i32, float* out_disp, int timeout_ms,
+                         uint64_t* ticket) {
+  if (!h || !in || (!out_i32 && !out_disp) || !ticket) return SN_ERR_ARG;
+  {
+    std::lock_guard<std::mutex> lk(h->mu);
+    int rc = check_device(h);
     if (rc) return rc;
-    ++s->uses[kind][mask][mi];
-  }
-  HIP_TRY(h, hipEventRecord(s->ev1, s->stream));
+    if ((rc = ensure_slots(h))) return rc;
+  }
+  int slot = -1;
+  uint64_t t = 0;
+  if (h->aq->claim(timeout_ms, &slot, &t) != 0) return SN_ERR_BUSY;
+  SlotGuard guard{h, slot};
+  Slot* const s = &h->slots[slot];
+  const size_t HW = (size_t)h->H * h->W;
+  s->user_raw = out_i32;
+  s->user_disp = out_disp;
+  s->kind = kind;
+  memcpy(s->pin_in, in, (kind == 1 ? 3 : 6) * HW);
+  if (h->coalesce) {
+    guard.armed = false;
+    *ticket = t;
+    h->aq->ready(slot);
+    return SN_OK;
+  }
+  if (const int rc = h->aq->issue_direct(slot)) return rc;
   guard.armed = false;
-  *ticket = s->ticket;
+  *ticket = t;
   return SN_OK;
 }
 
@@ -747,32 +917,47 @@
 
 int sn_wait(sn_handle* h, uint64_t ticket, float* infer_ms) {
   if (!h || ticket == 0) return SN_ERR_ARG;
-  Slot* s = nullptr;
+  sn_async::Queue* q;
   {
     std::lock_guard<std::mutex> lk(h->mu);
-    for (auto& c : h->slots)
-      if (c.ticket == ticket) s = &c;
-  }
-  if (!s) return SN_ERR_TICKET;
-  SlotGuard guard{h, s, true};
+    q = h->aq.get();
+  }
+  const int slot = q ? q->find(ticket) : -1;
+  if (slot < 0) return SN_ERR_TICKET;
+  Slot* const s = &h->slots[slot];
+  SlotGuard guard{h, slot};
+  sn_async::Launch l;
+  if (const int rc = q->wait_issued(slot, &l)) return rc == sn_async::kBusy ? SN_ERR_TICKET : rc;
+  AsyncRec& R = h->arec[l.rec];
   hipSetDevice(h->device);
-  HIP_TRY(h, hipEventSynchronize(s->ev1));
+  HIP_TRY(h, hipEventSynchronize(R.ev1));
   const size_t HW = (size_t)h->H * h->W;
-  auto rerun = [&]() -> int {
-    const int r = forward(h, s->ws, s->stream, 1, s->ws.in6, s->user_disp ? s->ws.out_disp : nullptr,
-                          s->user_raw ? s->ws.out_raw : nullptr, false, SN_PREC_F16X3);
-    if (r) return r;
-    if (s->user_raw) HIP_TRY(h, hipMemcpyAsync(s->pin_raw, s->ws.out_raw, 4 * HW, hipMemcpyDeviceToHost, s->stream));
-    if (s->user_disp) HIP_TRY(h, hipMemcpyAsync(s->pin_disp, s->ws.out_disp, 4 * HW, hipMemcpyDeviceToHost, s->stream));
-    HIP_TRY(h, hipEventRecord(s->ev1, s->stream));
-    HIP_TRY(h, hipEventSynchronize(s->ev1));
-    return SN_OK;
-  };
-  const bool check = h->precision == SN_PREC_AUTO && s->mode_run == SN_PREC_F16;
   RangeCount range;
-  if (const int rc = settle(h, s->ws, s->stream, 1, s->ws.in6, s->mode_run, check, true, rerun, &range)) return rc;
+  if (l.k == 1) {
+    auto rerun = [&]() -> int {
+      const int r = forward(h, s->ws, s->stream, 1, s->ws.in6, s->user_disp ? s->ws.out_disp : nullptr,
+                            s->user_raw ? s->ws.out_raw : nullptr, false, SN_PREC_F16X3, false, true);
+      if (r) return r;
+      if (s->user_raw) HIP_TRY(h, hipMemcpyAsync(s->pin_raw, s->ws.out_raw, 4 * HW, hipMemcpyDeviceToHost, s->stream));
+      if (s->user_disp) HIP_TRY(h, hipMemcpyAsync(s->pin_disp, s->ws.out_disp, 4 * HW, hipMemcpyDeviceToHost, s->stream));
+      HIP_TRY(h, hipEventRecord(R.ev1, s->stream));
+      HIP_TRY(h, hipEventSynchronize(R.ev1));
+      return SN_OK;
+    };
+    const bool check = h->precision == SN_PREC_AUTO && s->mode_run == SN_PREC_F16;
+    if (const int rc = settle(h, s->ws, s->stream, 1, s->ws.in6, s->mode_run, check, true, rerun, &range)) return rc;
+  } else {
+    snapshot_stats(h, l);
+    int rc = SN_OK;
+    if (q->begin_settle(l.rec, &rc)) {
+      rc = settle_group(h, l, R);
+      q->end_settle(l.rec, rc);
+    }
+    if (rc) return rc;
+    range = R.range;
+  }
   float ms = 0.f;
-  if (infer_ms) HIP_TRY(h, hipEventElapsedTime(&ms, s->ev0, s->ev1));
+  if (infer_ms) HIP_TRY(h, hipEventElapsedTime(&ms, R.ev0, R.ev1));
   if (infer_ms) *infer_ms = ms;
   if (s->user_raw) memcpy(s->user_raw, s->pin_raw, 4 * HW);
   if (s->user_disp) memcpy(s->user_disp, s->pin_disp, 4 * HW);
@@ -783,8 +968,16 @@
   if (!h) return SN_ERR_ARG;
   int rc = check_device(h);
   if (rc) return rc;
+  sn_async::Queue* q;
+  {
+    std::lock_guard<std::mutex> lk(h->mu);
+    q = h->aq.get();
+  }
+  if (q) q->drain();
   HIP_TRY(h, hipStreamSynchronize(h->stream));
   for (auto& s : h->slots) HIP_TRY(h, hipStreamSynchronize(s.stream));
+  for (auto& g : h->glane)
+    if (g.stream) HIP_TRY(h, hipStreamSynchronize(g.stream));
   return SN_OK;
 }
 
diff --git a/include/stereonet_hip.h b/include/stereonet_hip.h
--- a/include/stereonet_hip.h
+++ b/include/stereonet_hip.h
@@ -186,6 +186,7 @@
                         const float *w2, const float *b2, const float *head_w, float head_b, const float *low, int ups,
                         float dnorm, int h_out, int w_out, int form, float *out_disp, int32_t *out_raw);
 int sn_dbg_read(sn_handle *h, const char *what, float *dst, size_t cap, size_t *n);
+int sn_dbg_async_launches(sn_handle *h, uint64_t *by_size, int cap);
 int sn_depth_from_raw(sn_handle *h, int n, const int32_t *raw, float focal_px, float baseline_mm, float *depth_m,
                       float *disp_px, int mem, void *stream);
 
```

Result: no change. 3067, median of 2 (-0.0%).
